# mohammadasim98/mv-ldm

Hardware: AMD Instinct MI355X
Metric: denoised views/sec @ 256x256, 4 views, 50 DDIM steps (higher is better)
Workload: dtype bf16

## Files before the change

### include/mvldm.h

```cpp
#ifndef MVLDM_H
#define MVLDM_H

#include <stddef.h>
#include <stdint.h>

#ifdef __cplusplus
extern "C" {
#endif

#define MVLDM_ABI_VERSION 7

typedef void* mvldm_stream_t;

enum { MVLDM_F32 = 0, MVLDM_BF16 = 1, MVLDM_F16 = 2 };
enum { MVLDM_OK = 0, MVLDM_ERR_ARG = -1, MVLDM_ERR_HIP = -2, MVLDM_ERR_UNSUPPORTED = -3 };

enum { MVLDM_EPI_NONE = 0, MVLDM_EPI_SILU = 1, MVLDM_EPI_GEGLU = 2, MVLDM_EPI_GELU = 3  };
enum { MVLDM_ELT_COPY = 0, MVLDM_ELT_SILU = 1, MVLDM_ELT_GELU = 2 };

int mvldm_abi_version(void);
int mvldm_build_flags(void);
const char* mvldm_last_error(void);
int mvldm_device_info(int* cu_count, size_t* hbm_bytes, char* arch, int arch_len);

typedef struct mvldm_igemm_desc {
    const void* src0;
    const void* src1;
    const void* weight;
    const float* bias;
    const float* row_bias;
    const void* residual;
    void* dst;
    float* workspace;
    int32_t c0, c1;
    int32_t n_img, h_in, w_in, h_out, w_out;
    int32_t ksize, stride, pad, upsample;
    int32_t n_out, n_pad, k_pad;
    int32_t row_bias_ld;
    int32_t epilogue;
    int32_t act_dtype;
    int32_t dst_dtype;
    int32_t splitk;
    int32_t tile;
    int32_t k_order;
    int32_t dst_ld;
    float out_scale;
    size_t workspace_bytes;
} mvldm_igemm_desc;
int mvldm_igemm_fwd(const mvldm_igemm_desc* d, mvldm_stream_t stream);
size_t mvldm_igemm_workspace_bytes(const mvldm_igemm_desc* d);

int mvldm_pack_weight(const float* src, void* dst, int n_out, int c_in, int ksize, int c_pad, int n_pad,
                      int k_pad, int geglu, int k_order, int dst_dtype, int transpose, int c_off, int n_rows,
                      mvldm_stream_t stream);

int mvldm_pack_skinny(const void* packed, void* dst, int n_pad, int k_pad, int geglu, int dtype, mvldm_stream_t stream);
int mvldm_igemm_skinny_config(const mvldm_igemm_desc* d);

typedef struct mvldm_pack_job {
    const float* src; void* dst;
    int n_out, c_in, ksize, c_pad, n_pad, k_pad, geglu, k_order, transpose, c_off, n_rows;
    int kind;
    int blocks;
    int block0;
} mvldm_pack_job;
int mvldm_pack_job_prepare(mvldm_pack_job* job , int dst_dtype);
int mvldm_pack_weight_batch(const mvldm_pack_job* jobs , int n_jobs, const int32_t* block_job, int total_blocks,
                            int dst_dtype, mvldm_stream_t stream);

#define MVLDM_GN_MAX_CHUNKS 32
int mvldm_groupnorm_fwd(const void* x0, const void* x1, void* y, const float* gamma, const float* beta, int n_img,
                        int hw, int c0, int c1, int groups, float eps, int silu, int dtype, void* stats_ws,
                        float* stats_out, mvldm_stream_t stream);
int mvldm_groupnorm_passes(int n_img, int hw, int c, int groups, int dtype);

int mvldm_layernorm_fwd(const void* x, void* y, const float* gamma, const float* beta, int rows, int c, float eps,
                        int dtype, mvldm_stream_t stream);

int mvldm_attention_fwd(const void* q, const void* k, const void* v, void* out, int ld_q, int ld_k, int ld_v,
                        int ld_o, int heads, int head_dim, const int32_t* seg, int n_seg, int max_q_len,
                        float scale, int dtype, float* lse, int lse_ld, mvldm_stream_t stream);

int mvldm_timestep_embed_fwd(const int64_t* timesteps, const float* freqs, void* out, int n, int dim,
                             int flip_sin_to_cos, int dst_dtype, mvldm_stream_t stream);

int mvldm_eltwise_fwd(const void* x, void* y, size_t n, int op, int src_dtype, int dst_dtype, mvldm_stream_t stream);

int mvldm_ddim_cfg_step(const float* eps, const float* x_t, float* x_next, const int32_t* cond_img,
                        const int32_t* uncond_img, int n_tgt, int hw, int c, float cfg_scale, const float* coef,
                        const int32_t* step_ptr, void* unet_in, int unet_in_c, int unet_in_dtype, int n_steps,
                        float clip_range, mvldm_stream_t stream);
int mvldm_ddpm_cfg_step(const float* eps_c, const float* eps_u, const float* x_t, const float* noise, float* x_next, size_t n,
                        float cfg_scale, const float* coef, float clip_range, mvldm_stream_t stream);
int mvldm_ddim_advance(int32_t* step_ptr, const int64_t* t_table, int n_steps, int64_t* timesteps,
                       const int32_t* tgt_rows, int n_rows, mvldm_stream_t stream);

int mvldm_nchw_to_nhwc(const float* src, void* dst, int n_img, int c, int hw, int dst_c, int dst_c_off,
                       int dst_dtype, float scale, float shift, const int32_t* img_map, mvldm_stream_t stream);
int mvldm_nhwc_to_nchw(const void* src, float* dst, int n_img, int c, int hw, int src_c, int src_c_off,
                       int src_dtype, float scale, float shift, int clamp01, mvldm_stream_t stream);

enum { MVLDM_RAYS_RAW = 0, MVLDM_RAYS_POSITIONAL = 1, MVLDM_RAYS_SRT = 2 };
int mvldm_ray_channels(int mode, int n_origin_octaves, int n_dir_octaves);
int mvldm_ray_encode(const float* extrinsics, const float* intrinsics, int n_cam, int h, int w, float* out_nchw,
                     void* out_nhwc, int nhwc_c, int nhwc_c_off, int nhwc_dtype, const int32_t* img_map, int mode,
                     int n_origin_octaves, int n_dir_octaves, int plucker, mvldm_stream_t stream);

int mvldm_posterior_sample(const float* moments, const float* noise, float* out, int n, int c, int hw, float scale,
                           mvldm_stream_t stream);


typedef struct mvldm_wgrad_desc {
    const void* src0; const void* src1; const void* dy;
    float* grad;
    float* workspace; size_t workspace_bytes;
    int32_t c0, c1, c_in;
    int32_t n_img, h_in, w_in, h_out, w_out;
    int32_t ksize, stride, pad, upsample;
    int32_t n_out, dy_ld;
    int32_t act_dtype;
    int32_t accumulate;
} mvldm_wgrad_desc;
int mvldm_igemm_wgrad(const mvldm_wgrad_desc* d, mvldm_stream_t stream);

int mvldm_colsum(const void* x, float* dst, float* workspace, size_t workspace_bytes, int n_seg, int rows_per_seg, int n,
                 int ld, int ld_dst, int per_seg, int accumulate, int dtype, mvldm_stream_t stream);

#define MVLDM_NORM_BWD_STORE 0x100
int mvldm_groupnorm_bwd(const void* x0, const void* x1, const void* dy, void* dx0, void* dx1, const float* gamma,
                        const float* beta, const float* stats, float* dgamma, float* dbeta, int n_img, int hw, int c0,
                        int c1, int groups, int silu, int dtype, float* workspace, size_t workspace_bytes,
                        mvldm_stream_t stream);
int mvldm_layernorm_bwd(const void* x, const void* dy, void* dx, const float* gamma, float* dgamma, float* dbeta,
// ... 233 lines not shown
```

### mv_ldm_amd/_lib.py

```python
from __future__ import annotations

import ctypes as C
from pathlib import Path

LIB_PATH = Path(__file__).resolve().parent / "csrc" / "libmvldm_hip.so"

ABI_VERSION = 7
F32, BF16, F16 = 0, 1, 2
EPI_NONE, EPI_SILU, EPI_GEGLU, EPI_GELU = 0, 1, 2, 3
RAYS_RAW, RAYS_POSITIONAL, RAYS_SRT = 0, 1, 2
ELT_COPY, ELT_SILU, ELT_GELU = 0, 1, 2
NORM_BWD_STORE = 0x100
GN_MAX_CHUNKS = 32
JPEG_GRAY, JPEG_444, JPEG_422, JPEG_420 = 0, 1, 2, 3
JPEG_REASONS = ("ok", "not a JPEG", "truncated", "corrupt", "progressive", "frame type", "precision", "components", "sampling", "colour space",
                "scans", "size", "range guard", "restart intervals")
JPEG_RANGE = 12
JPEG_RESTART = 13
JPEG_HUFF_TABLE_BYTES, JPEG_TABLE_BYTES = 1424, 8928

(OP_IGEMM, OP_GROUPNORM, OP_LAYERNORM, OP_ATTENTION, OP_TIMESTEP_EMBED, OP_ELTWISE, OP_DDIM_STEP, OP_DDIM_ADVANCE,
 OP_NCHW_TO_NHWC, OP_NHWC_TO_NCHW, OP_MEMCPY, OP_RAY_ENCODE, OP_POSTERIOR_SAMPLE,
 OP_WGRAD, OP_ATTENTION_BWD, OP_GROUPNORM_BWD, OP_LAYERNORM_BWD, OP_COLSUM, OP_TRAIN_ELTWISE, OP_POOL2X2, OP_ZERO_INSERT,
 OP_ADD_NOISE, OP_MSE_LOSS, OP_FILL_ZERO, OP_PAR_BEGIN, OP_PAR_NEXT, OP_PAR_END, OP_GATHER_ROWS, OP_ATTN_MERGE) = range(1, 30)
TE_SILU_BWD, TE_ADD, TE_GEGLU_FWD, TE_GEGLU_BWD, TE_GELU_BWD = 0, 1, 2, 3, 4

vp, i32, f32, sz = C.c_void_p, C.c_int32, C.c_float, C.c_size_t


class IgemmDesc(C.Structure):
    _fields_ = [("src0", vp), ("src1", vp), ("weight", vp), ("bias", vp), ("row_bias", vp), ("residual", vp),
                ("dst", vp), ("workspace", vp),
                ("c0", i32), ("c1", i32),
                ("n_img", i32), ("h_in", i32), ("w_in", i32), ("h_out", i32), ("w_out", i32),
                ("ksize", i32), ("stride", i32), ("pad", i32), ("upsample", i32),
                ("n_out", i32), ("n_pad", i32), ("k_pad", i32),
                ("row_bias_ld", i32), ("epilogue", i32), ("act_dtype", i32), ("dst_dtype", i32),
                ("splitk", i32), ("tile", i32), ("k_order", i32), ("dst_ld", i32), ("out_scale", f32), ("workspace_bytes", sz)]


class _GroupNorm(C.Structure):
    _fields_ = [("x", vp), ("x1", vp), ("y", vp), ("gamma", vp), ("beta", vp), ("stats_ws", vp),
                ("n_img", i32), ("hw", i32), ("c0", i32), ("c1", i32), ("groups", i32), ("silu", i32), ("dtype", i32),
                ("eps", f32), ("stats_out", vp)]


class _LayerNorm(C.Structure):
    _fields_ = [("x", vp), ("y", vp), ("gamma", vp), ("beta", vp), ("rows", i32), ("c", i32), ("dtype", i32), ("eps", f32)]


class _Attention(C.Structure):
    _fields_ = [("q", vp), ("k", vp), ("v", vp), ("out", vp), ("seg", vp),
                ("ld_q", i32), ("ld_k", i32), ("ld_v", i32), ("ld_o", i32), ("heads", i32), ("head_dim", i32),
                ("n_seg", i32), ("max_q_len", i32), ("dtype", i32), ("scale", f32), ("lse", vp), ("lse_ld", i32)]


class _Temb(C.Structure):
    _fields_ = [("timesteps", vp), ("freqs", vp), ("out", vp), ("n", i32), ("dim", i32), ("flip", i32), ("dst_dtype", i32)]


class _Eltwise(C.Structure):
    _fields_ = [("x", vp), ("y", vp), ("n", sz), ("op", i32), ("src_dtype", i32), ("dst_dtype", i32)]


class _Ddim(C.Structure):
    _fields_ = [("eps", vp), ("x_t", vp), ("x_next", vp), ("cond_img", vp), ("uncond_img", vp), ("coef", vp),
                ("step_ptr", vp), ("unet_in", vp),
                ("n_tgt", i32), ("hw", i32), ("c", i32), ("unet_in_c", i32), ("unet_in_dtype", i32), ("cfg_scale", f32),
                ("n_steps", i32), ("clip_range", f32)]


class _Advance(C.Structure):
    _fields_ = [("step_ptr", vp), ("t_table", vp), ("timesteps", vp), ("tgt_rows", vp), ("n_steps", i32), ("n_rows", i32)]


class _Layout(C.Structure):
    _fields_ = [("src", vp), ("dst", vp), ("n_img", i32), ("c", i32), ("hw", i32), ("other_c", i32),
                ("other_c_off", i32), ("dtype", i32), ("clamp01", i32), ("scale", f32), ("shift", f32), ("img_map", vp)]


class _Rays(C.Structure):
    _fields_ = [("extrinsics", vp), ("intrinsics", vp), ("out_nchw", vp), ("out_nhwc", vp), ("img_map", vp),
                ("n_cam", i32), ("h", i32), ("w", i32), ("nhwc_c", i32), ("nhwc_c_off", i32), ("nhwc_dtype", i32),
                ("mode", i32), ("n_origin_octaves", i32), ("n_dir_octaves", i32), ("plucker", i32)]


class _Posterior(C.Structure):
    _fields_ = [("moments", vp), ("noise", vp), ("out", vp), ("n", i32), ("c", i32), ("hw", i32), ("scale", f32)]


class _Memcpy(C.Structure):
    _fields_ = [("src", vp), ("dst", vp), ("bytes", sz)]


class _AttnMerge(C.Structure):
    _fields_ = [("oa", vp), ("ob", vp), ("out", vp), ("lse_a", vp), ("lse_b", vp), ("a_img", vp), ("b_img", vp), ("out_img", vp),
                ("n_img", i32), ("tokens", i32), ("heads", i32), ("head_dim", i32), ("ld_a", i32), ("ld_b", i32), ("ld_o", i32),
                ("lse_ld_a", i32), ("lse_ld_b", i32), ("dtype", i32)]


class _Gather(C.Structure):
    _fields_ = [("src", vp), ("dst", vp), ("src_index", vp), ("dst_index", vp), ("row_bytes", sz), ("n_rows", i32)]


class PackJob(C.Structure):
    _fields_ = [("src", vp), ("dst", vp), ("n_out", i32), ("c_in", i32), ("ksize", i32), ("c_pad", i32), ("n_pad", i32), ("k_pad", i32),
                ("geglu", i32), ("k_order", i32), ("transpose", i32), ("c_off", i32), ("n_rows", i32), ("kind", i32), ("blocks", i32),
                ("block0", i32)]


class WgradDesc(C.Structure):
    _fields_ = [("src0", vp), ("src1", vp), ("dy", vp), ("grad", vp), ("workspace", vp), ("workspace_bytes", sz),
                ("c0", i32), ("c1", i32), ("c_in", i32),
                ("n_img", i32), ("h_in", i32), ("w_in", i32), ("h_out", i32), ("w_out", i32),
                ("ksize", i32), ("stride", i32), ("pad", i32), ("upsample", i32),
                ("n_out", i32), ("dy_ld", i32), ("act_dtype", i32), ("accumulate", i32)]


class AttnBwdDesc(C.Structure):
    _fields_ = [("q", vp), ("k", vp), ("v", vp), ("out", vp), ("dout", vp), ("dq", vp), ("dk", vp), ("dv", vp),
                ("lse", vp), ("delta", vp), ("seg", vp),
                ("ld_q", i32), ("ld_k", i32), ("ld_v", i32), ("ld_o", i32), ("ld_do", i32), ("ld_dq", i32), ("ld_dk", i32), ("ld_dv", i32),
                ("heads", i32), ("head_dim", i32), ("n_seg", i32), ("max_q_len", i32), ("max_kv_len", i32), ("total_q_rows", i32),
                ("stat_ld", i32), ("dtype", i32), ("scale", f32)]


class _GroupNormBwd(C.Structure):
    _fields_ = [("x0", vp), ("x1", vp), ("dy", vp), ("dx0", vp), ("dx1", vp), ("gamma", vp), ("beta", vp), ("stats", vp),
                ("dgamma", vp), ("dbeta", vp), ("workspace", vp), ("workspace_bytes", sz),
                ("n_img", i32), ("hw", i32), ("c0", i32), ("c1", i32), ("groups", i32), ("silu", i32), ("dtype", i32)]


class _LayerNormBwd(C.Structure):
    _fields_ = [("x", vp), ("dy", vp), ("dx", vp), ("gamma", vp), ("dgamma", vp), ("dbeta", vp), ("workspace", vp),
                ("workspace_bytes", sz), ("rows", i32), ("c", i32), ("dtype", i32), ("eps", f32)]


class _Colsum(C.Structure):
    _fields_ = [("x", vp), ("dst", vp), ("workspace", vp), ("workspace_bytes", sz),
                ("n_seg", i32), ("rows_per_seg", i32), ("n", i32), ("ld", i32), ("ld_dst", i32), ("per_seg", i32),
                ("accumulate", i32), ("dtype", i32)]


class _TrainEltwise(C.Structure):
    _fields_ = [("a", vp), ("b", vp), ("out", vp), ("rows", sz), ("op", i32), ("d", i32), ("a_dtype", i32), ("dtype", i32)]


class _Resample(C.Structure):
    _fields_ = [("src", vp), ("dst", vp), ("n_img", i32), ("h", i32), ("w", i32), ("c", i32), ("dtype", i32)]


class _AddNoise(C.Structure):
    _fields_ = [("x0", vp), ("noise", vp), ("coef", vp), ("dst", vp), ("img_map", vp),
                ("n", i32), ("c", i32), ("hw", i32), ("dst_c", i32), ("dst_c_off", i32), ("dst_dtype", i32)]


class _Mse(C.Structure):
    _fields_ = [("pred", vp), ("noise", vp), ("tgt_img", vp), ("loss", vp), ("dpred", vp), ("workspace", vp),
                ("n_tgt", i32), ("hw", i32), ("c", i32), ("accumulate", i32), ("dpred_c", i32), ("dpred_dtype", i32),
                ("loss_scale", f32), ("grad_scale", f32), ("amp_scale", vp)]


class AmpState(C.Structure):
    _fields_ = [("scale", f32), ("growth_tracker", i32), ("adam_step", i32), ("found_inf", i32), ("skipped", i32), ("reserved", i32 * 3)]


class _Fill(C.Structure):
    _fields_ = [("dst", vp), ("bytes", sz)]


class _OpUnion(C.Union):
    _fields_ = [("igemm", IgemmDesc), ("groupnorm", _GroupNorm), ("layernorm", _LayerNorm), ("attention", _Attention),
                ("temb", _Temb), ("eltwise", _Eltwise), ("ddim", _Ddim), ("advance", _Advance), ("layout", _Layout),
                ("memcpy_", _Memcpy), ("gather", _Gather), ("attn_merge", _AttnMerge), ("rays", _Rays), ("posterior", _Posterior),
                ("wgrad", WgradDesc), ("attention_bwd", AttnBwdDesc), ("groupnorm_bwd", _GroupNormBwd),
                ("layernorm_bwd", _LayerNormBwd), ("colsum", _Colsum), ("train_eltwise", _TrainEltwise), ("resample", _Resample),
                ("add_noise", _AddNoise), ("mse", _Mse), ("fill", _Fill)]


class Op(C.Structure):
    _fields_ = [("kind", i32), ("tag", i32), ("u", _OpUnion)]


SIGNATURES = {
    "mvldm_abi_version": (C.c_int, []),
    "mvldm_build_flags": (C.c_int, []),
    "mvldm_last_error": (C.c_char_p, []),
    "mvldm_device_info": (C.c_int, [C.POINTER(C.c_int), C.POINTER(sz), C.c_char_p, C.c_int]),
    "mvldm_igemm_fwd": (C.c_int, [C.POINTER(IgemmDesc), vp]),
    "mvldm_igemm_workspace_bytes": (sz, [C.POINTER(IgemmDesc)]),
    "mvldm_pack_weight": (C.c_int, [vp, vp] + [C.c_int] * 12 + [vp]),
    "mvldm_pack_skinny": (C.c_int, [vp, vp, C.c_int, C.c_int, C.c_int, C.c_int, vp]),
    "mvldm_igemm_skinny_config": (C.c_int, [C.POINTER(IgemmDesc)]),
    "mvldm_pack_job_prepare": (C.c_int, [C.POINTER(PackJob), C.c_int]),
    "mvldm_pack_weight_batch": (C.c_int, [vp, C.c_int, vp, C.c_int, C.c_int, vp]),
    "mvldm_groupnorm_fwd": (C.c_int, [vp, vp, vp, vp, vp, C.c_int, C.c_int, C.c_int, C.c_int, C.c_int, f32, C.c_int, C.c_int, vp, vp, vp]),
    "mvldm_groupnorm_passes": (C.c_int, [C.c_int] * 5),
    "mvldm_layernorm_fwd": (C.c_int, [vp, vp, vp, vp, C.c_int, C.c_int, f32, C.c_int, vp]),
    "mvldm_attention_fwd": (C.c_int, [vp, vp, vp, vp] + [C.c_int] * 6 + [vp, C.c_int, C.c_int, f32, C.c_int, vp, C.c_int, vp]),
    "mvldm_igemm_wgrad": (C.c_int, [C.POINTER(WgradDesc), vp]),
    "mvldm_colsum": (C.c_int, [vp, vp, vp, sz] + [C.c_int] * 8 + [vp]),
    "mvldm_groupnorm_bwd": (C.c_int, [vp] * 10 + [C.c_int] * 7 + [vp, sz, vp]),
    "mvldm_layernorm_bwd": (C.c_int, [vp] * 6 + [C.c_int, C.c_int, f32, C.c_int, vp, sz, vp]),
    "mvldm_attention_bwd": (C.c_int, [C.POINTER(AttnBwdDesc), vp]),
    "mvldm_train_eltwise": (C.c_int, [C.c_int, vp, vp, vp, sz, C.c_int, C.c_int, C.c_int, vp]),
    "mvldm_pool2x2_sum": (C.c_int, [vp, vp] + [C.c_int] * 5 + [vp]),
    "mvldm_zero_insert2x": (C.c_int, [vp, vp] + [C.c_int] * 5 + [vp]),
    "mvldm_add_noise": (C.c_int, [vp, vp, vp, vp] + [C.c_int] * 6 + [vp, vp]),
    "mvldm_mse_loss": (C.c_int, [vp, vp, vp, C.c_int, C.c_int, C.c_int, vp, C.c_int, f32, vp, C.c_int, C.c_int, f32, vp, vp]),
    "mvldm_grad_norm": (C.c_int, [vp, sz, vp, f32, vp, vp, vp]),
    "mvldm_adamw_step": (C.c_int, [vp, vp, vp, vp, sz, f32, f32, f32, f32, f32, C.c_int, f32, vp, vp]),
    "mvldm_mse_loss_amp": (C.c_int, [vp, vp, vp, C.c_int, C.c_int, C.c_int, vp, C.c_int, f32, vp, C.c_int, C.c_int, f32, vp, vp, vp]),
    "mvldm_grad_norm_amp": (C.c_int, [vp, sz, vp, f32, vp, vp, vp, vp]),
    "mvldm_adamw_step_amp": (C.c_int, [vp, vp, vp, vp, sz, f32, f32, f32, f32, f32, f32, vp, vp, vp]),
    "mvldm_amp_update": (C.c_int, [vp, f32, f32, C.c_int, vp]),
    "mvldm_timestep_embed_fwd": (C.c_int, [vp, vp, vp, C.c_int, C.c_int, C.c_int, C.c_int, vp]),
    "mvldm_eltwise_fwd": (C.c_int, [vp, vp, sz, C.c_int, C.c_int, C.c_int, vp]),
    "mvldm_ddim_cfg_step": (C.c_int, [vp, vp, vp, vp, vp, C.c_int, C.c_int, C.c_int, f32, vp, vp, vp, C.c_int, C.c_int, C.c_int, f32, vp]),
    "mvldm_ddim_advance": (C.c_int, [vp, vp, C.c_int, vp, vp, C.c_int, vp]),
    "mvldm_gather_rows": (C.c_int, [vp, vp, vp, vp, C.c_int, sz, vp]),
    "mvldm_attention_merge": (C.c_int, [vp] * 8 + [C.c_int] * 10 + [vp]),
    "mvldm_ddpm_cfg_step": (C.c_int, [vp, vp, vp, vp, vp, sz, f32, vp, f32, vp]),
    "mvldm_ema_update": (C.c_int, [vp, vp, sz, f32, vp]),
    "mvldm_image_metrics_workspace_bytes": (sz, [C.c_int] * 4),
    "mvldm_image_metrics": (C.c_int, [vp, vp] + [C.c_int] * 5 + [vp, vp, vp, sz, vp]),
    "mvldm_lpips_workspace_bytes": (sz, [C.c_int] * 3),
    "mvldm_lpips_tap_slots": (C.c_int, [C.c_int] * 3),
    "mvldm_lpips_prep": (C.c_int, [vp, vp, vp] + [C.c_int] * 6 + [vp]),
    "mvldm_lpips_relu": (C.c_int, [vp, sz, C.c_int, vp]),
    "mvldm_lpips_tap": (C.c_int, [vp, vp, vp] + [C.c_int] * 5 + [vp, sz, C.c_int, C.c_int, vp]),
    "mvldm_lpips_fold": (C.c_int, [vp, sz, C.c_int, C.c_int, C.c_int, vp, vp]),
    "mvldm_dists_workspace_bytes": (sz, [C.c_int] * 3),
    "mvldm_dists_stat_slots": (C.c_int, [C.c_int] * 3),
    "mvldm_dists_prep": (C.c_int, [vp, vp, vp] + [C.c_int] * 5 + [vp]),
    "mvldm_dists_stats": (C.c_int, [vp, vp] + [C.c_int] * 5 + [vp, sz, C.c_int, C.c_int, vp]),
    "mvldm_dists_l2pool": (C.c_int, [vp, vp] + [C.c_int] * 5 + [vp]),
    "mvldm_dists_fold": (C.c_int, [vp, sz, C.c_int, C.c_int, C.c_int, vp, vp, vp, vp]),
    "mvldm_fid_workspace_bytes": (sz, [C.c_int] * 4),
    "mvldm_fid_pool_slots": (C.c_int, [C.c_int] * 3),
    "mvldm_fid_prep": (C.c_int, [vp, C.c_int, vp] + [C.c_int] * 7 + [vp]),
    "mvldm_fid_pool": (C.c_int, [vp] + [C.c_int] * 5 + [vp, sz, vp]),
    "mvldm_fid_accumulate": (C.c_int, [vp, sz] + [C.c_int] * 4 + [vp, vp, vp]),
    "mvldm_fid_compute": (C.c_int, [vp, vp, C.c_int, vp, vp, vp]),
    "mvldm_inception_workspace_bytes": (sz, [C.c_int] * 3),
    "mvldm_inception_prep": (C.c_int, [vp, C.c_int, vp] + [C.c_int] * 7 + [vp, sz, vp]),
    "mvldm_inception_unfold": (C.c_int, [vp, vp] + [C.c_int] * 9 + [vp]),
    "mvldm_inception_maxpool": (C.c_int, [vp, vp] + [C.c_int] * 9 + [vp]),
    "mvldm_inception_avgpool": (C.c_int, [vp, vp] + [C.c_int] * 7 + [vp]),
    "mvldm_inception_concat": (C.c_int, [vp, vp, sz] + [C.c_int] * 5 + [vp]),
    "mvldm_inception_features": (C.c_int, [vp] + [C.c_int] * 5 + [vp, vp]),
    "mvldm_frechet_accumulate": (C.c_int, [vp, C.c_int, C.c_int, vp, vp]),
    "mvldm_frechet_workspace_bytes": (sz, [C.c_int]),
    "mvldm_frechet_compute": (C.c_int, [vp, vp, C.c_int, vp, sz, vp, vp, vp]),
    "mvldm_kid_workspace_bytes": (sz, [C.c_int, C.c_int]),
    "mvldm_kid_compute": (C.c_int, [vp, C.c_int, vp, C.c_int, C.c_int, vp, vp, C.c_int, C.c_int, vp, sz, vp, vp, vp, vp]),
    "mvldm_crop_shim_workspace_bytes": (sz, [C.c_int] * 5),
    "mvldm_crop_shim": (C.c_int, [vp, C.c_int, vp] + [C.c_int] * 5 + [vp, sz, C.POINTER(C.c_int), vp]),
    "mvldm_crop_shim_flip": (C.c_int, [vp, C.c_int, vp] + [C.c_int] * 5 + [vp, vp, sz, C.POINTER(C.c_int), vp]),
    "mvldm_crop_shim_axis": (C.c_int, [C.c_int] * 4 + [C.POINTER(i32), C.POINTER(i32), C.c_int]),
    "mvldm_jpeg_probe": (C.c_int, [vp, sz, C.POINTER(i32)]),
    "mvldm_jpeg_coef_count": (sz, [C.c_int] * 3),
    "mvldm_jpeg_entropy": (C.c_int, [vp, sz, vp, sz, vp, C.POINTER(i32)]),
    "mvldm_jpeg_workspace_bytes": (sz, [C.c_int] * 4),
    "mvldm_jpeg_decode": (C.c_int, [vp, vp, vp] + [C.c_int] * 4 + [vp, sz, vp]),
    "mvldm_jpeg_idct_host": (C.c_int, [vp, vp, vp, C.c_int, C.c_int, C.c_int]),
    "mvldm_jpeg_scan_room": (sz, [sz]),
    "mvldm_jpeg_scan_prepare": (C.c_int, [vp, sz, vp, sz, sz, vp, vp, vp]),
    "mvldm_jpeg_entropy_chunk_subseqs": (C.c_int, []),
    "mvldm_jpeg_entropy_device": (C.c_int, [vp, sz, vp, vp] + [C.c_int] * 4 + [vp, vp, vp, C.c_int, vp]),
    "mvldm_jpeg_entropy_emul_host": (C.c_int, [vp, sz, vp, vp] + [C.c_int] * 4 + [vp, vp, vp, C.c_int, C.c_int]),
    "mvldm_nchw_to_nhwc": (C.c_int, [vp, vp] + [C.c_int] * 6 + [f32, f32, vp, vp]),
    "mvldm_ray_channels": (C.c_int, [C.c_int, C.c_int, C.c_int]),
    "mvldm_ray_encode": (C.c_int, [vp, vp, C.c_int, C.c_int, C.c_int, vp, vp, C.c_int, C.c_int, C.c_int, vp] + [C.c_int] * 4 + [vp]),
# ... 56 lines not shown
```

### mv_ldm_amd/csrc/igemm.hip

```cpp
#include <algorithm>
#include <cstdio>
#include <cstdlib>

#include "igemm_common.h"

namespace mvldm {

template <typename T> __global__ __launch_bounds__(256) void igemm_splitk_reduce(const IgemmParams p) {
    const bool geglu = p.epilogue == MVLDM_EPI_GEGLU;
    const size_t total = (size_t)p.M * p.n_dst;
    const size_t slab = (size_t)p.M * p.n_pad;
    for (size_t idx = (size_t)blockIdx.x * 256 + threadIdx.x; idx < total; idx += (size_t)gridDim.x * 256) {
        const int m = (int)(idx / p.n_dst), col = (int)(idx - (size_t)m * p.n_dst);
        float v;
        if (geglu) {
            const int nv = (col >> 5) * 64 + (col & 31), ng = nv + 32;
            float a = 0.f, g = 0.f;
            for (int s = 0; s < p.splitk; ++s) {
                a += p.ws[s * slab + (size_t)m * p.n_pad + nv];
                g += p.ws[s * slab + (size_t)m * p.n_pad + ng];
            }
            if (p.bias) { a += p.bias[col]; g += p.bias[p.n_dst + col]; }
            v = a * gelu_erf_fast(g);
        } else {
// ... 65 lines not shown
                const float* rb = p.row_bias + (size_t)(m / p.hw_out) * p.row_bias_ld + col;
#pragma unroll
                for (int e = 0; e < 8; ++e) a[e] += rb[e];
            }
            if (p.epilogue == MVLDM_EPI_SILU) {
#pragma unroll
                for (int e = 0; e < 8; ++e) a[e] = silu_f(a[e]);
            } else if (p.epilogue == MVLDM_EPI_GELU) {
#pragma unroll
                for (int e = 0; e < 8; ++e) a[e] = gelu_erf_fast(a[e]);
            }
        }
#pragma unroll
        for (int e = 0; e < 8; ++e) a[e] *= p.out_scale;
        if (p.residual) {
            const Chunk<T> rc = load_chunk<T>(reinterpret_cast<const T*>(p.residual) + (size_t)m * p.n_dst + col);
#pragma unroll
            for (int e = 0; e < 8; ++e) a[e] += rc.get(e);
        }
        size_t drow = (size_t)m;
        if (p.scatter) {
            const int img = m / p.hw_out, rem = m - img * p.hw_out;
            const int i = rem / p.w_out, j = rem - i * p.w_out;
            drow = ((size_t)img * (2 * p.h_out) + 2 * i + p.ph_y) * (size_t)(2 * p.w_out) + 2 * j + p.ph_x;
        }
        Chunk<T> oc;
#pragma unroll
        for (int e = 0; e < 8; ++e) oc.set(e, a[e]);
        store_chunk<T>(reinterpret_cast<T*>(p.dst) + drow * p.dst_ld + col, oc);
    }
}

static int env_int(const char* name, int dflt) { return knob_int(name, dflt); }
static const int kEnvTarget = env_int("MVLDM_IGEMM_TARGET", 0);
static const int kEnvSync = env_int("MVLDM_IGEMM_SYNC", 0);
static const int kEnvPx = env_int("MVLDM_IGEMM_PX", 0);
static const int kEnvNoStage = env_int("MVLDM_IGEMM_NOSTAGE", 0);
#ifdef MVLDM_EXPERIMENTS
static const int kEnvFake = env_int("MVLDM_IGEMM_FAKE", 0);
#else
static constexpr int kEnvFake = 0;
#endif

static thread_local int t_force_sync = 0;

static int launch_igemm(const IgemmParams& p, int tile, int act_dtype, hipStream_t s) {
    if (tile >= 1 && tile <= 5) return igemm_launch_small(p, tile, act_dtype, s);
    if (tile >= 6 && tile <= 8) return igemm_launch_large(p, tile, act_dtype, s);
    if (tile == 9 || tile == 10 || tile == 18) return igemm_launch_xl(p, tile, act_dtype, s);
    if (tile == 11 || tile == 17) return igemm_launch_halo(p, tile, act_dtype, s);
    return set_error(MVLDM_ERR_ARG, "igemm: bad tile %d", tile);
}


static void choose_config(const mvldm_igemm_desc& d, int M, int k_tiles, int& tile, int& splitk, size_t ws_bytes) {
    const int target = kEnvTarget ? kEnvTarget : 512;
    if (tile == 0) {
        const bool can10 = d.act_dtype != MVLDM_F32 && d.k_order == 1 && d.dst_dtype != MVLDM_F32 && d.n_pad % 320 == 0 &&
                           d.epilogue != MVLDM_EPI_GEGLU && d.upsample != 1 && d.n_out % 8 == 0 && (d.dst_ld <= 0 || d.dst_ld % 8 == 0) &&
                           !(d.ksize == 3 && d.src1);
        const int wgs10 = cdiv(M, 256) * (d.n_pad / 320);
        const double eff10 = (double)wgs10 / (256.0 * cdiv(wgs10, 256));
        if (can10 && (wgs10 >= 1024 || (wgs10 >= 512 && (eff10 >= 0.9 || d.ksize == 1)))) tile = 10;
        else if (M <= 32) tile = 5;
        else if (M <= 64) tile = 4;
        else if (d.ksize >= 2) tile = cdiv(M, 256) * cdiv(d.n_pad, 128) >= 300 ? 7 : 2;
        else if (d.n_pad >= 768 && d.act_dtype != MVLDM_F32 && d.k_order == 1 && d.dst_dtype != MVLDM_F32 &&
                 cdiv(M, 256) * cdiv(d.n_pad, 256) >= 1024)
            tile = 9;
        else if (d.k_pad >= 1024 && d.n_pad >= 1024 && cdiv(M, 128) * cdiv(d.n_pad, 256) >= 300) tile = 8;
        else tile = d.n_pad < 640 ? 2 : 3;
    }
    const int tm = cdiv(M, kTiles[tile].bm), tn = cdiv(d.n_pad, kTiles[tile].bn);
    if (splitk == 0) {
        splitk = 1;
        const int wgs = tm * tn;
        if (wgs < target) splitk = std::min(std::max(k_tiles / 4, 1), cdiv(target, wgs));
        if (d.workspace == nullptr) splitk = 1;
        while (splitk > 1 && (size_t)splitk * M * d.n_pad * sizeof(float) > ws_bytes) --splitk;
    }
    splitk = std::max(1, std::min(splitk, k_tiles));
}

static int fill_params(const mvldm_igemm_desc& d, IgemmParams& p, int& tile) {
    const int epc = d.act_dtype == MVLDM_F32 ? 4 : 8;
    const int bk = d.act_dtype == MVLDM_F32 ? 32 : 64;
    MVLDM_REQUIRE(d.src0 && d.weight && d.dst, "igemm: null pointer");
    const bool phase = d.upsample >= 2;
    MVLDM_REQUIRE(d.upsample >= 0 && d.upsample <= 5, "igemm: upsample %d", d.upsample);
    MVLDM_REQUIRE(phase ? (d.ksize == 2 && d.stride == 1 && d.h_out == d.h_in && d.w_out == d.w_in && !d.src1 && !d.residual &&
                           !d.row_bias && d.act_dtype != MVLDM_F32 && d.dst_dtype == d.act_dtype && d.k_order == 1)
                        : (d.ksize == 1 || d.ksize == 3),
                  "igemm: ksize %d / upsample %d", d.ksize, d.upsample);
    MVLDM_REQUIRE(d.stride == 1 || d.stride == 2, "igemm: stride %d", d.stride);
    MVLDM_REQUIRE(d.c0 % epc == 0 && d.c1 % epc == 0 && d.c0 > 0, "igemm: channels (%d,%d) must be multiples of %d", d.c0, d.c1, epc);
    MVLDM_REQUIRE((d.c1 == 0) == (d.src1 == nullptr), "igemm: src1/c1 mismatch");
    MVLDM_REQUIRE(d.k_pad % bk == 0 && d.k_pad >= d.ksize * d.ksize * (d.c0 + d.c1), "igemm: k_pad %d", d.k_pad);
    MVLDM_REQUIRE(d.n_pad % 64 == 0 && d.n_pad >= d.n_out, "igemm: n_pad %d (n_out %d)", d.n_pad, d.n_out);
    MVLDM_REQUIRE(d.dst_dtype == d.act_dtype || d.dst_dtype == MVLDM_F32, "igemm: dst dtype");
    if (d.epilogue == MVLDM_EPI_GEGLU)
        MVLDM_REQUIRE(d.n_out % 64 == 0 && !d.row_bias, "igemm: GEGLU needs n_out %% 64 == 0");
    p.src0 = d.src0; p.src1 = d.src1; p.weight = d.weight; p.bias = d.bias; p.row_bias = d.row_bias;
    p.residual = d.residual; p.dst = d.dst; p.ws = d.workspace;
    p.c0 = d.c0; p.c1 = d.c1; p.ctot = d.c0 + d.c1;
    p.n_img = d.n_img; p.h_in = d.h_in; p.w_in = d.w_in; p.h_out = d.h_out; p.w_out = d.w_out;
    p.hw_out = d.h_out * d.w_out;
    p.ksize = d.ksize; p.stride = d.stride; p.pad = d.pad; p.upsample = phase ? 0 : d.upsample; p.taps = d.ksize * d.ksize;
    p.scatter = phase; p.ph_y = phase ? (d.upsample - 2) >> 1 : 0; p.ph_x = phase ? (d.upsample - 2) & 1 : 0;
    p.ty0 = phase ? p.ph_y - 1 : -d.pad; p.tx0 = phase ? p.ph_x - 1 : -d.pad;
    p.cy = phase ? 1 - p.ph_y : d.ksize / 2; p.cx = phase ? 1 - p.ph_x : d.ksize / 2;
    p.M = d.n_img * p.hw_out; p.n_out = d.n_out; p.n_pad = d.n_pad; p.k_pad = d.k_pad;
    p.n_dst = d.epilogue == MVLDM_EPI_GEGLU ? d.n_out / 2 : d.n_out;
    p.rb_vec = d.row_bias && ((uintptr_t)d.row_bias % 16 == 0) && d.row_bias_ld % 4 == 0;
    p.bias_vec = d.bias && ((uintptr_t)d.bias % 16 == 0);
    p.row_bias_ld = d.row_bias_ld; p.epilogue = d.epilogue; p.dst_f32 = d.dst_dtype == MVLDM_F32;
    p.out_scale = d.out_scale;
    p.dst_ld = d.dst_ld > 0 ? d.dst_ld : p.n_dst;
    MVLDM_REQUIRE(p.dst_ld >= p.n_dst, "igemm: dst_ld %d < n_dst %d", p.dst_ld, p.n_dst);
    p.k_tiles = d.k_pad / bk;
    tile = d.tile & 63;
    t_force_sync = (d.tile >> 12) & 1;
    const int force_px = (d.tile >> 8) & 15;
    int splitk = d.splitk;
    MVLDM_REQUIRE(((tile >= 0 && tile <= kNumTiles) || tile == 17 || deep_tile(tile)) && splitk >= 0, "igemm: tile/splitk");
    choose_config(d, p.M, p.k_tiles, tile, splitk, d.workspace_bytes);
    if (splitk > 1)
        MVLDM_REQUIRE(d.workspace && (size_t)splitk * p.M * d.n_pad * sizeof(float) <= d.workspace_bytes,
                      "igemm: split-K workspace too small");
    const double es = 2.0;
    const double b0 = (double)d.n_img * d.h_in * d.w_in * d.c0 * es, b1 = (double)d.n_img * d.h_in * d.w_in * d.c1 * es;
    const double bw = (double)d.n_pad * d.k_pad * es;
    p.use_bl = d.act_dtype != MVLDM_F32 && d.k_order == 1 && !t_force_sync && !kEnvSync &&
               b0 < 4.0e9 && b1 < 4.0e9 && bw < 4.0e9;
    if (d.act_dtype != MVLDM_F32 && d.k_order == 1 && !t_force_sync && !kEnvSync && !p.use_bl) {
        static bool warned = false;
        if (!warned) {
            warned = true;
            fprintf(stderr, "[mvldm] igemm: operand of %.2f GB exceeds the 4 GB range of the fast 16-bit loop; using the slower "
                            "64-bit-address loop (split the batch to avoid this)\n", std::max(std::max(b0, b1), bw) / 1e9);
        }
    }
    p.src0_bytes = (unsigned)b0; p.src1_bytes = (unsigned)b1; p.w_bytes = (unsigned)bw;
    p.fake = kEnvFake;
    p.nt_store = stream_stores((size_t)p.M * (size_t)p.n_dst * (p.dst_f32 || d.act_dtype == MVLDM_F32 ? 4 : 2));
    if (kEnvFake & 1) p.src0_bytes = p.src1_bytes = 0;
    if (kEnvFake & 2) p.w_bytes = 0;
    if (tile >= 6 && !p.use_bl) tile = 2;
    if (deep_tile(tile) && d.upsample) tile = 2;
    p.splitk = splitk;
    if (p.use_bl) {
        const int cbs = p.k_tiles / p.taps;
        const int per = cdiv(cbs, std::min(splitk, cbs));
        p.k_tiles_per_split = per * p.taps;
        p.splitk = cdiv(cbs, per);
    } else {
        p.k_tiles_per_split = cdiv(p.k_tiles, splitk);
        p.splitk = cdiv(p.k_tiles, p.k_tiles_per_split);
    }
    p.stage_epi = d.act_dtype != MVLDM_F32 && !kEnvNoStage && (p.splitk > 1 || (!p.dst_f32 && p.n_dst % 8 == 0 && p.dst_ld % 8 == 0));
    if (tile >= 9 && tile <= 10 && (!p.stage_epi || (tile == 10 && d.epilogue == MVLDM_EPI_GEGLU))) tile = 7;
    if (tile == 11 && !(p.use_bl && p.stage_epi && p.splitk == 1 && d.ksize == 3 && d.stride == 1 && d.pad == 1 && !d.upsample &&
                        d.h_out == d.h_in && d.w_out == d.w_in && halo_rows_for(d.w_in) <= 384 && halo_smem(d.w_in) <= 160 * 1024))
        tile = 7;
    if (tile == 17 && !(p.use_bl && p.stage_epi && p.splitk == 1 && d.ksize == 3 && d.stride == 1 && d.pad == 1 && !d.upsample && d.c1 == 0 &&
                        d.h_out == d.h_in && d.w_out == d.w_in && d.epilogue != MVLDM_EPI_GEGLU && halow_smem(d.w_in) <= 160 * 1024))
        tile = 7;
    if (phase) {
        MVLDM_REQUIRE(p.use_bl && p.stage_epi, "igemm: 2x2 phase conv needs the lean 16-bit loop and an 8-aligned 16-bit output");
        if (tile != 7 && tile != 10) tile = 2;
    }
    if (p.use_bl && d.upsample == 1 && tile != 7) tile = 2;
    if (p.use_bl && d.upsample != 1) {
        const int hc = (d.h_out - 1) * d.stride + p.ty0 + p.cy, wc = (d.w_out - 1) * d.stride + p.tx0 + p.cx;
        MVLDM_REQUIRE(p.ty0 + p.cy >= 0 && p.tx0 + p.cx >= 0 && hc < d.h_in && wc < d.w_in,
                      "igemm: conv geometry (pad %d, stride %d) not supported", d.pad, d.stride);
    }
    p.tiles_m = cdiv(p.M, kTiles[tile].bm);
    p.tiles_n = cdiv(d.n_pad, kTiles[tile].bn);
    p.korder = d.k_order;
    if (d.k_order)
        MVLDM_REQUIRE(d.k_order == 1 && p.ctot % bk == 0 && d.c0 % bk == 0 && d.k_pad == p.taps * p.ctot,
                      "igemm: k_order 1 needs channel counts (%d,%d) multiples of %d", d.c0, d.c1, bk);
    {
        const double a_bytes = (double)d.n_img * d.h_in * d.w_in * p.ctot, w_bytes = (double)d.n_pad * d.k_pad;
        double best = 1e300;
        for (int px = 1; px <= 8; px *= 2) {
            const int py = 8 / px;
            const int sm = cdiv(p.tiles_m, px), sn = cdiv(p.tiles_n, py);
            const double waste = (double)(8 * sm * sn) / ((double)p.tiles_m * p.tiles_n);
            const double cost = (py * a_bytes + px * w_bytes) * waste * waste;
            if (cost < best) { best = cost; p.px = px; p.sub_m = sm; p.sub_n = sn; }
        }
        p.m_fast = w_bytes >= a_bytes;
        const int fpx = force_px ? force_px : kEnvPx;
        if (fpx > 0 && fpx <= 8 && (8 % fpx) == 0) {
            p.px = fpx; p.sub_m = cdiv(p.tiles_m, p.px); p.sub_n = cdiv(p.tiles_n, 8 / p.px);
        }
        p.grp_m = p.grp_n = 1;
        static const int kGroup = knob_int("MVLDM_IGEMM_GROUP", -1);
        if (kGroup != 0 && ((tile >= 7 && tile <= 10) || tile == 17) && p.sub_m * p.sub_n > 32) {
            const double ax = a_bytes / p.px, wx = w_bytes / (8 / p.px);
            double bestc = 1e300;
            for (int gm = 1; gm <= 32; gm *= 2) {
                if (kGroup > 0 && gm != kGroup) continue;
                const int gme = std::min(gm, p.sub_m), gne = std::min(32 / gm, p.sub_n);
                const double c = ax * cdiv(p.sub_n, gne) + wx * cdiv(p.sub_m, gme);
                if (c < bestc) { bestc = c; p.grp_m = gme; p.grp_n = gne; }
            }
        }
    }
    return MVLDM_OK;
}

int linear_pp_run(const mvldm_igemm_desc& d, hipStream_t s);
int linear_pw_run(const mvldm_igemm_desc& d, hipStream_t s);
int linear_ws_run(const mvldm_igemm_desc& d, hipStream_t s);
int skinny_run(const mvldm_igemm_desc& d, hipStream_t s);
int linear_rs_run(const mvldm_igemm_desc& d, hipStream_t s);

int igemm_run(const mvldm_igemm_desc& d, hipStream_t s) {
    IgemmParams p;
    int tile = 0;
    if (d.n_img == 0 || d.h_out == 0 || d.w_out == 0) return MVLDM_OK;
    const int req = d.tile & 63;
    if (req == 15) return skinny_run(d, s);
    if (req == 12 || req == 13 || req == 14 || req == 19) {
        MVLDM_REQUIRE(d.src0 && d.weight && d.dst, "igemm: null pointer");
        return req == 12 ? linear_pp_run(d, s) : req == 13 ? linear_pw_run(d, s) : req == 14 ? linear_ws_run(d, s) : linear_rs_run(d, s);
    }
    MVLDM_REQUIRE(d.k_order != 2, "igemm: the fragment-order pack (k_order 2) is read by tile 15 only");
    int rc = fill_params(d, p, tile);
    if (rc) return rc;
    if (p.M == 0) return MVLDM_OK;
    rc = dispatch_dtype(d.act_dtype, [&](auto t) {
        using T = decltype(t);
        int r = launch_igemm(p, tile, Elt<T>::DT, s);
        if (r) return r;
        if (p.splitk > 1) {
            if constexpr (sizeof(T) == 2) {
                if (!p.dst_f32 && p.n_dst % 8 == 0 && p.dst_ld % 8 == 0 && ((uintptr_t)p.ws % 16) == 0 &&
                    (!p.residual || ((uintptr_t)p.residual % 16) == 0) && ((uintptr_t)p.dst % 16) == 0) {
                    const size_t chunks = (size_t)p.M * (p.n_dst / 8);
                    hipLaunchKernelGGL(igemm_splitk_reduce_vec<T>, dim3((unsigned)std::min<size_t>((chunks + 255) / 256, 4096)), dim3(256), 0, s, p);
                    return check_launch();
                }
            }
            const size_t total = (size_t)p.M * p.n_dst;
            const int blocks = (int)std::min<size_t>((total + 255) / 256, 4096);
            hipLaunchKernelGGL(igemm_splitk_reduce<T>, dim3(blocks), dim3(256), 0, s, p);
            return check_launch();
        }
        return (int)MVLDM_OK;
    });
    return rc;
}

}

using namespace mvldm;

extern "C" int mvldm_igemm_fwd(const mvldm_igemm_desc* d, mvldm_stream_t stream) {
    MVLDM_REQUIRE(d != nullptr, "igemm: null desc");
    return igemm_run(*d, (hipStream_t)stream);
}

extern "C" size_t mvldm_igemm_workspace_bytes(const mvldm_igemm_desc* d) {
    if (!d) return 0;
    const size_t M = (size_t)d->n_img * d->h_out * d->w_out;
    return (size_t)16 * M * d->n_pad * sizeof(float);
}
```

### mv_ldm_amd/csrc/igemm_bl.h

```cpp
#pragma once
#include "igemm_common.h"

namespace mvldm {

template <typename T, int BM, int BN, int WM, int WN>
__global__ __launch_bounds__(WM* WN * 64) void igemm_kernel(const IgemmParams p) {
    using M_ = Mma<T>;
    constexpr int NT = WM * WN * 64;
    constexpr int EPC = Elt<T>::EPC;
    constexpr int BK = M_::BK;
    constexpr int TM = BM / WM / 32, TN = BN / WN / 32;
    constexpr int A_BYTES = BM * M_::PITCH, B_BYTES = BN * M_::PITCH;
    constexpr int A_IT = BM * 8 / NT, B_IT = BN * 8 / NT;
    static_assert(A_IT >= 1 && B_IT >= 1 && TM >= 1 && TN >= 1, "bad tile");
    extern __shared__ __attribute__((aligned(16))) char smem[];

    const int tid = threadIdx.x, lane = tid & 63, wave = tid >> 6;
    const int wm = wave / WN, wn = wave % WN;
    const int hi = lane >> 5, l31 = lane & 31;

    int split, tm, tn;
    if (!map_block(p, split, tm, tn)) return;
    const int kt0 = split * p.k_tiles_per_split;
    const int kt1 = min(kt0 + p.k_tiles_per_split, p.k_tiles);
// ... 36 lines not shown
        const int cs = from0 ? p.c0 : p.c1;
#pragma unroll
        for (int it = 0; it < A_IT; ++it) {
            int iy = a_y[it] + ky, ix = a_x[it] + kx;
            const bool ok = tap_ok && a_img[it] >= 0 && iy >= 0 && iy < hs && ix >= 0 && ix < wsz;
            if (p.upsample) { iy >>= 1; ix >>= 1; }
            if (ok) {
                const size_t off = ((size_t)(a_img[it] * p.h_in + iy) * p.w_in + ix) * cs;
                areg[it] = *reinterpret_cast<const u32x4*>(sbase + off);
            } else {
                areg[it] = u32x4{0u, 0u, 0u, 0u};
            }
        }
#pragma unroll
        for (int it = 0; it < B_IT; ++it) {
            const int n = tn * BN + r0 + it * (NT / 8);
            if (n < p.n_pad)
                breg[it] = *reinterpret_cast<const u32x4*>(wbase + (size_t)it * (NT / 8) * p.k_pad + (size_t)kt * BK);
            else
                breg[it] = u32x4{0u, 0u, 0u, 0u};
        }
    };
    auto store_tile = [&](int stage) {
        char* at = smem + stage * (A_BYTES + B_BYTES);
        char* bt = at + A_BYTES;
#pragma unroll
        for (int it = 0; it < A_IT; ++it) M_::store(at, r0 + it * (NT / 8), kc, areg[it]);
#pragma unroll
        for (int it = 0; it < B_IT; ++it) M_::store(bt, r0 + it * (NT / 8), kc, breg[it]);
    };

    f32x16 acc[TM][TN];
#pragma unroll
    for (int i = 0; i < TM; ++i)
#pragma unroll
        for (int j = 0; j < TN; ++j)
#pragma unroll
            for (int r = 0; r < 16; ++r) acc[i][j][r] = 0.f;

    if (kt0 < kt1) {
        load_tile(kt0);
        store_tile(0);
    }
    __syncthreads();
    int cur = 0;
    for (int kt = kt0; kt < kt1; ++kt) {
        const bool more = kt + 1 < kt1;
        if (more) load_tile(kt + 1);
        const char* at = smem + cur * (A_BYTES + B_BYTES);
        const char* bt = at + A_BYTES;
#pragma unroll
        for (int kk = 0; kk < BK / M_::KI; ++kk) {
            typename M_::Frag a[TM], b[TN];
#pragma unroll
            for (int i = 0; i < TM; ++i) a[i] = M_::load(at, wm * (BM / WM) + i * 32 + l31, kk, hi);
#pragma unroll
            for (int j = 0; j < TN; ++j) b[j] = M_::load(bt, wn * (BN / WN) + j * 32 + l31, kk, hi);
#pragma unroll
            for (int i = 0; i < TM; ++i)
#pragma unroll
                for (int j = 0; j < TN; ++j) acc[i][j] = M_::mma(a[i], b[j], acc[i][j]);
        }
        if (more) store_tile(cur ^ 1);
        __syncthreads();
        cur ^= 1;
    }

    if constexpr (sizeof(T) == 2) {
        if (p.stage_epi) {
            igemm_epilogue_staged<T, BM, BN, WM, WN>(p, acc, tm, tn, split, wm, wn, wave, lane, smem);
            return;
        }
    }
    igemm_epilogue<T, BM, BN, WM, WN>(p, acc, tm, tn, split, wm, wn, hi, l31);
}


template <int TAPS, int A_IT, bool DUAL, bool UPS> struct BlAddr {
    unsigned a0[UPS ? TAPS : 1][A_IT];
    unsigned a1[DUAL ? (UPS ? TAPS : 1) : 1][DUAL ? A_IT : 1];
    unsigned mask[UPS ? 1 : A_IT];
};

template <typename T, int BM, int BN, int NW, int KS, bool DUAL, int A_IT, int B_IT, int STAGES, bool UPS, int t, int LO = 0, int HI = 1 << 20>
__device__ __forceinline__ void bl_issue(const IgemmParams& p, char* stage_base, int wave, int cb,
                                         const BlAddr<KS * KS, A_IT, DUAL, UPS>& ad, const unsigned (&vb)[B_IT]) {
    constexpr int BK = 64, TAPS = KS * KS;
    const int lead = (!UPS && KS > 1) ? p.w_in + 1 : 0;
    const int disp = UPS ? 0 : (t / KS - p.cy) * p.w_in + (t % KS - p.cx) + lead;
    const unsigned lead0 = (unsigned)lead * (unsigned)p.c0 * 2u, lead1 = (unsigned)lead * (unsigned)p.c1 * 2u;
    const __amdgpu_buffer_rsrc_t r0 = __builtin_amdgcn_make_buffer_rsrc(
        const_cast<char*>(reinterpret_cast<const char*>(p.src0)) - lead0, 0, p.src0_bytes + lead0, 0x00020000);
    const __amdgpu_buffer_rsrc_t r1 = __builtin_amdgcn_make_buffer_rsrc(
        const_cast<char*>(reinterpret_cast<const char*>(DUAL ? p.src1 : p.src0)) - (DUAL ? lead1 : lead0), 0,
        DUAL ? p.src1_bytes + lead1 : p.src0_bytes + lead0, 0x00020000);
    const __amdgpu_buffer_rsrc_t rw = __builtin_amdgcn_make_buffer_rsrc(const_cast<void*>(p.weight), 0, p.w_bytes, 0x00020000);
    char* at = stage_base;
    char* bt = at + BM * 128;
    const int c = cb * BK;
    const bool from0 = !DUAL || c < p.c0;
    const int soff = ((from0 ? c : c - p.c0) + disp * (from0 ? p.c0 : p.c1)) * 2;
#pragma unroll
    for (int it = (LO > 0 ? LO : 0); it < (HI < A_IT ? HI : A_IT); ++it) {
        __attribute__((address_space(3))) void* dst = (__attribute__((address_space(3))) void*)(at + (wave + NW * it) * 1024);
        unsigned v0, v1;
        if constexpr (UPS) {
            v0 = ad.a0[t][it];
            v1 = ad.a1[DUAL ? t : 0][DUAL ? it : 0];
        } else {
            const bool ok = (ad.mask[it] >> t) & 1u;
            v0 = ok ? ad.a0[0][it] : kBufOob;
            v1 = ok ? ad.a1[0][DUAL ? it : 0] : kBufOob;
        }
        if (from0) __builtin_amdgcn_raw_ptr_buffer_load_lds(r0, dst, 16, v0, soff, 0, 0);
        else __builtin_amdgcn_raw_ptr_buffer_load_lds(r1, dst, 16, v1, soff, 0, 0);
    }
    const int koff = (cb * TAPS + t) * (BK * 2);
#pragma unroll
    for (int it = (LO > A_IT ? LO - A_IT : 0); it < (HI - A_IT < B_IT ? HI - A_IT : B_IT); ++it)
        __builtin_amdgcn_raw_ptr_buffer_load_lds(rw, (__attribute__((address_space(3))) void*)(bt + (wave + NW * it) * 1024), 16,
                                                 vb[it], koff, 0, 0);
}

template <typename T, int BM, int BN, int WM, int WN>
__device__ __forceinline__ void bl_compute(const char* stage_base, f32x16 (&acc)[BM / WM / 32][BN / WN / 32], int wm, int wn,
                                           int hi, int l31) {
    constexpr int TM = BM / WM / 32, TN = BN / WN / 32;
#pragma unroll
    for (int kk = 0; kk < 64 / Mma<T>::KI; ++kk) {
        BlFrags<T, TM, TN> f;
        bl_load<T, BM, BN, WM, WN>(stage_base, f, kk, wm, wn, hi, l31);
        bl_mma<T, TM, TN>(f, acc);
    }
}

template <int LPT, int MAXY>
__device__ __forceinline__ void bl_wait_young(int young) {
    if constexpr (MAXY >= 1) {
        if (young >= MAXY) {
            asm volatile("s_waitcnt vmcnt(%0) lgkmcnt(0)" ::"n"(MAXY * LPT) : "memory");
            return;
        }
        bl_wait_young<LPT, MAXY - 1>(young);
    } else {
        asm volatile("s_waitcnt vmcnt(0) lgkmcnt(0)" ::: "memory");
    }
}

template <typename T, int BM, int BN, int WM, int WN, int KS, bool DUAL, int STAGES, bool UPS>
__global__ __launch_bounds__(WM* WN * 64) void igemm_bl_kernel(const IgemmParams p) {
    using M_ = Mma<T>;
    static_assert(sizeof(T) == 2, "16-bit activation types only");
    constexpr int NW = WM * WN, TAPS = KS * KS;
    constexpr int BK = 64, EPC = 8;
    constexpr int TM = BM / WM / 32, TN = BN / WN / 32;
    constexpr int A_BYTES = BM * 128, B_BYTES = BN * 128, STAGE_BYTES = A_BYTES + B_BYTES;
    constexpr int A_IT = BM / 8 / NW, B_IT = BN / 8 / NW, LPT = A_IT + B_IT;
    static_assert(A_IT >= 1 && B_IT >= 1 && (BM / 8) % NW == 0 && (BN / 8) % NW == 0, "bad tile");
    static_assert(STAGES >= 2 && STAGES <= 8, "ring depth");
    extern __shared__ __attribute__((aligned(16))) char smem[];

    const auto [lane, wave, wm, wn, hi, l31] = wave_lane<WN>();
    int split, tm, tn;
    if (!map_block(p, split, tm, tn)) return;
    const int cb0 = split * (p.k_tiles_per_split / TAPS);
    const int cb1 = min(cb0 + p.k_tiles_per_split / TAPS, p.k_tiles / TAPS);

    const int slot = lane & 7, rsub = lane >> 3;
    BlAddr<TAPS, A_IT, DUAL, UPS> ad;
#pragma unroll
    for (int it = 0; it < A_IT; ++it) {
        const int row = (wave + NW * it) * 8 + rsub;
        const int m = tm * BM + row;
        const unsigned chunk = (unsigned)((slot ^ ((row >> 1) & 7)) * EPC);
        const bool live = m < p.M;
        const int img = live ? m / p.hw_out : 0, rem = live ? m - img * p.hw_out : 0;
        const int oy = rem / p.w_out, ox = rem - oy * p.w_out;
        if constexpr (UPS) {
            const unsigned hs = 2 * p.h_in, wsz = 2 * p.w_in;
            const int y0 = live ? oy * p.stride - p.pad : -(1 << 20), x0 = ox * p.stride - p.pad;
#pragma unroll
            for (int t = 0; t < TAPS; ++t) {
                const int iy = y0 + t / KS, ix = x0 + t % KS;
                const bool ok = (unsigned)iy < hs && (unsigned)ix < wsz;
                const unsigned pix = (unsigned)(img * p.h_in + (iy >> 1)) * (unsigned)p.w_in + (unsigned)(ix >> 1);
                ad.a0[t][it] = ok ? (pix * (unsigned)p.c0 + chunk) * 2u : kBufOob;
                if constexpr (DUAL) ad.a1[t][it] = ok ? (pix * (unsigned)p.c1 + chunk) * 2u : kBufOob;
            }
        } else {
            const int yc = oy * p.stride + p.ty0 + p.cy, xc = ox * p.stride + p.tx0 + p.cx;
            const unsigned pix = (unsigned)(img * p.h_in + yc) * (unsigned)p.w_in + (unsigned)xc;
            unsigned msk = 0;
#pragma unroll
            for (int t = 0; t < TAPS; ++t) {
                const int iy = yc + t / KS - p.cy, ix = xc + t % KS - p.cx;
                msk |= (live && (unsigned)iy < (unsigned)p.h_in && (unsigned)ix < (unsigned)p.w_in) ? (1u << t) : 0u;
            }
            ad.a0[0][it] = (pix * (unsigned)p.c0 + chunk) * 2u;
            if constexpr (DUAL) ad.a1[0][it] = (pix * (unsigned)p.c1 + chunk) * 2u;
            ad.mask[it] = msk;
        }
    }
    unsigned vb[B_IT];
#pragma unroll
    for (int it = 0; it < B_IT; ++it) {
        const int row = (wave + NW * it) * 8 + rsub;
        const int n = tn * BN + row;
        const unsigned chunk = (unsigned)((slot ^ ((row >> 1) & 7)) * EPC);
        vb[it] = n < p.n_pad ? ((unsigned)n * (unsigned)p.k_pad + chunk) * 2u : kBufOob;
    }

    f32x16 acc[TM][TN];
#pragma unroll
    for (int i = 0; i < TM; ++i)
#pragma unroll
        for (int j = 0; j < TN; ++j)
#pragma unroll
            for (int r = 0; r < 16; ++r) acc[i][j][r] = 0.f;

#define MVLDM_BL_ISSUE(stage_, cb_, t_) \
    bl_issue<T, BM, BN, NW, KS, DUAL, A_IT, B_IT, STAGES, UPS, t_>(p, smem + (stage_) * STAGE_BYTES, wave, cb_, ad, vb)
#define MVLDM_BL_ISSUE_R(stage_, cb_, t_, lo_, hi_) \
    bl_issue<T, BM, BN, NW, KS, DUAL, A_IT, B_IT, STAGES, UPS, t_, lo_, hi_>(p, smem + (stage_) * STAGE_BYTES, wave, cb_, ad, vb)
#define MVLDM_BL_NEXT(t_, d_) (((t_) + (d_)) % TAPS)
#define MVLDM_BL_LOAD(f_, slot_, kk_) bl_load<T, BM, BN, WM, WN>(smem + (slot_) * STAGE_BYTES, f_, kk_, wm, wn, hi, l31)
#define MVLDM_BL_MMA(f_)                  \
    __builtin_amdgcn_sched_barrier(0);    \
    bl_mma<T, TM, TN>(f_, acc);           \
    __builtin_amdgcn_sched_barrier(0);
#define MVLDM_BL_STEP(t_)                                                                                         \
    {                                                                                                             \
        static_assert(64 / M_::KI == 4, "four k-sub-steps per K-tile");                                          \
        MVLDM_BL_LOAD(f1, slot_c, 1);                                                                             \
        MVLDM_BL_MMA(f0)                                                                                          \
        MVLDM_BL_LOAD(f0, slot_c, 2);                                                                             \
        MVLDM_BL_MMA(f1)                                                                                          \
        MVLDM_BL_LOAD(f1, slot_c, 3);                                                                             \
        MVLDM_BL_MMA(f0)                                                                                          \
            \
                             \
        if (STAGES == 3 && cb + ((t_) + 2) / TAPS < cb1) asm volatile("s_waitcnt vmcnt(%0) lgkmcnt(0)" ::"n"(LPT) : "memory"); \
        else asm volatile("s_waitcnt vmcnt(0) lgkmcnt(0)" ::: "memory");                                          \
        __builtin_amdgcn_s_barrier();                                                                             \
        {                                                                                                         \
                   \
            const int cbn_ = cb + ((t_) + STAGES) / TAPS;                                                         \
            if (cbn_ < cb1) { MVLDM_BL_ISSUE(slot_c, cbn_, MVLDM_BL_NEXT(t_, STAGES)); }                          \
        }                                                                                                         \
        slot_c = slot_c + 1 == STAGES ? 0 : slot_c + 1;                                                           \
        MVLDM_BL_LOAD(f0, slot_c, 0);                                                                             \
        MVLDM_BL_MMA(f1)                                                                                          \
    }
#ifdef MVLDM_BL_BURST
    constexpr bool SPREAD_S = false;
#elif defined(MVLDM_BL_SPREAD_ALL)
    constexpr bool SPREAD_S = true;
#else
    constexpr bool SPREAD_S = NW == 8;
#endif
#define MVLDM_BL_STEP_SIMPLE(t_)                                                                                  \
    {                                                                                                             \
        asm volatile("s_waitcnt vmcnt(0) lgkmcnt(0)" ::: "memory");                                               \
        __builtin_amdgcn_s_barrier();                                                                             \
        if constexpr (!SPREAD_S) {                                                                                \
            const int cbn_ = cb + ((t_) + 1) / TAPS;                                                              \
            if (cbn_ < cb1) { MVLDM_BL_ISSUE(slot_c ^ 1, cbn_, MVLDM_BL_NEXT(t_, 1)); }                           \
            bl_compute<T, BM, BN, WM, WN>(smem + slot_c * STAGE_BYTES, acc, wm, wn, hi, l31);                     \
        } else {                                                                                                  \
            constexpr int Q0_ = (4 * LPT + 8) / 9, Q1_ = Q0_ + (LPT - Q0_ + 1) / 2;                              \
            const int cbn_ = cb + ((t_) + 1) / TAPS;                                                              \
            const bool more_ = cbn_ < cb1;                                                                        \
            if (more_) { MVLDM_BL_ISSUE_R(slot_c ^ 1, cbn_, MVLDM_BL_NEXT(t_, 1), 0, Q0_); }                      \
            {                                                                                                     \
                BlFrags<T, TM, TN> fs_;                                                                           \
                MVLDM_BL_LOAD(fs_, slot_c, 0);                                                                    \
                bl_mma<T, TM, TN>(fs_, acc);                                                                      \
            }                                                                                                     \
            if (more_) { MVLDM_BL_ISSUE_R(slot_c ^ 1, cbn_, MVLDM_BL_NEXT(t_, 1), Q0_, Q1_); }                    \
            {                                                                                                     \
                BlFrags<T, TM, TN> fs_;                                                                           \
                MVLDM_BL_LOAD(fs_, slot_c, 1);                                                                    \
                bl_mma<T, TM, TN>(fs_, acc);                                                                      \
            }                                                                                                     \
            if (more_) { MVLDM_BL_ISSUE_R(slot_c ^ 1, cbn_, MVLDM_BL_NEXT(t_, 1), Q1_, LPT); }                    \
            {                                                                                                     \
                BlFrags<T, TM, TN> fs_;                                                                           \
                MVLDM_BL_LOAD(fs_, slot_c, 2);                                                                    \
                bl_mma<T, TM, TN>(fs_, acc);                                                                      \
                MVLDM_BL_LOAD(fs_, slot_c, 3);                                                                    \
                bl_mma<T, TM, TN>(fs_, acc);                                                                      \
            }                                                                                                     \
        }                                                                                                         \
        slot_c ^= 1;                                                                                              \
    }
#define MVLDM_BL_STEP_DEEP(t_)                                                                                    \
    {                                                                                                             \
        bl_wait_young<LPT, STAGES - 2>((cb1 - cb) * TAPS - (t_) - 1);       \
        __builtin_amdgcn_s_barrier();                                       \
        {                                                                                                         \
            const int cbn_ = cb + ((t_) + STAGES - 1) / TAPS;                                                     \
            if (cbn_ < cb1) { MVLDM_BL_ISSUE(slot_c == 0 ? STAGES - 1 : slot_c - 1, cbn_, MVLDM_BL_NEXT(t_, STAGES - 1)); } \
        }                                                                                                         \
        bl_compute<T, BM, BN, WM, WN>(smem + slot_c * STAGE_BYTES, acc, wm, wn, hi, l31);                         \
        slot_c = slot_c + 1 == STAGES ? 0 : slot_c + 1;                                                           \
    }
#define MVLDM_BL_PRO(j_)                                                                                          \
    if constexpr (STAGES - 1 > (j_)) {                                                                            \
        if (cb0 + (j_) / TAPS < cb1) { MVLDM_BL_ISSUE((j_), cb0 + (j_) / TAPS, ((j_) % TAPS)); }                  \
    }
    constexpr bool PIPE = NW == 8 && TM * TN <= 8 && STAGES <= 3;
    if constexpr (STAGES > 3) {
        static_assert((STAGES - 2) * LPT <= 63, "vmcnt is a 6-bit counter");
        if (cb0 < cb1) {
            MVLDM_BL_ISSUE(0, cb0, 0);
            MVLDM_BL_PRO(1) MVLDM_BL_PRO(2) MVLDM_BL_PRO(3) MVLDM_BL_PRO(4) MVLDM_BL_PRO(5) MVLDM_BL_PRO(6)
            int slot_c = 0;
            for (int cb = cb0; cb < cb1; ++cb) {
                MVLDM_BL_STEP_DEEP(0)
                if constexpr (TAPS == 4) { MVLDM_BL_STEP_DEEP(1) MVLDM_BL_STEP_DEEP(2) MVLDM_BL_STEP_DEEP(3) }
                if constexpr (TAPS == 9) {
                    MVLDM_BL_STEP_DEEP(1) MVLDM_BL_STEP_DEEP(2) MVLDM_BL_STEP_DEEP(3) MVLDM_BL_STEP_DEEP(4)
                    MVLDM_BL_STEP_DEEP(5) MVLDM_BL_STEP_DEEP(6) MVLDM_BL_STEP_DEEP(7) MVLDM_BL_STEP_DEEP(8)
                }
            }
        }
    } else if constexpr (!PIPE) {
        static_assert(STAGES == 2, "the plain loop uses the 2-slot ring");
        if (cb0 < cb1) {
            MVLDM_BL_ISSUE(0, cb0, 0);
            int slot_c = 0;
            for (int cb = cb0; cb < cb1; ++cb) {
                MVLDM_BL_STEP_SIMPLE(0)
                if constexpr (TAPS == 4) { MVLDM_BL_STEP_SIMPLE(1) MVLDM_BL_STEP_SIMPLE(2) MVLDM_BL_STEP_SIMPLE(3) }
                if constexpr (TAPS == 9) {
                    MVLDM_BL_STEP_SIMPLE(1) MVLDM_BL_STEP_SIMPLE(2) MVLDM_BL_STEP_SIMPLE(3) MVLDM_BL_STEP_SIMPLE(4)
                    MVLDM_BL_STEP_SIMPLE(5) MVLDM_BL_STEP_SIMPLE(6) MVLDM_BL_STEP_SIMPLE(7) MVLDM_BL_STEP_SIMPLE(8)
                }
            }
        }
    } else if (cb0 < cb1) {
        MVLDM_BL_ISSUE(0, cb0, 0);
        const bool has1 = cb0 + 1 / TAPS < cb1, has2 = STAGES == 3 && cb0 + 2 / TAPS < cb1;
        if (has1) { MVLDM_BL_ISSUE(1, cb0 + 1 / TAPS, (1 % TAPS)); }
        if constexpr (STAGES == 3) {
            if (has2) { MVLDM_BL_ISSUE(2, cb0 + 2 / TAPS, (2 % TAPS)); }
        }
        if (has2) asm volatile("s_waitcnt vmcnt(%0)" ::"n"(2 * LPT) : "memory");
        else if (has1) asm volatile("s_waitcnt vmcnt(%0)" ::"n"(LPT) : "memory");
        else asm volatile("s_waitcnt vmcnt(0)" ::: "memory");
        __builtin_amdgcn_s_barrier();
        int slot_c = 0;
        BlFrags<T, TM, TN> f0, f1;
        MVLDM_BL_LOAD(f0, 0, 0);
        for (int cb = cb0; cb < cb1; ++cb) {
            MVLDM_BL_STEP(0)
            if constexpr (TAPS == 4) { MVLDM_BL_STEP(1) MVLDM_BL_STEP(2) MVLDM_BL_STEP(3) }
            if constexpr (TAPS == 9) {
                MVLDM_BL_STEP(1) MVLDM_BL_STEP(2) MVLDM_BL_STEP(3) MVLDM_BL_STEP(4)
                MVLDM_BL_STEP(5) MVLDM_BL_STEP(6) MVLDM_BL_STEP(7) MVLDM_BL_STEP(8)
            }
        }
    }
#undef MVLDM_BL_STEP_SIMPLE
#undef MVLDM_BL_STEP_DEEP
#undef MVLDM_BL_PRO
#undef MVLDM_BL_LOAD
#undef MVLDM_BL_MMA
#undef MVLDM_BL_NEXT
#undef MVLDM_BL_STEP
#undef MVLDM_BL_ISSUE
#undef MVLDM_BL_ISSUE_R
    asm volatile("s_waitcnt vmcnt(0)" ::: "memory");
    if constexpr (TM * TN > 4) {
        igemm_epilogue_staged<T, BM, BN, WM, WN>(p, acc, tm, tn, split, wm, wn, wave, lane, smem);
    } else {
        if (p.stage_epi) igemm_epilogue_staged<T, BM, BN, WM, WN>(p, acc, tm, tn, split, wm, wn, wave, lane, smem);
        else igemm_epilogue<T, BM, BN, WM, WN>(p, acc, tm, tn, split, wm, wn, hi, l31);
    }
}

template <typename T, int BM, int BN, int WM, int WN> static int launch_sync(const IgemmParams& p, hipStream_t s) {
    static std::atomic<uint64_t> done{0};
    constexpr int ring = 2 * (BM + BN) * Mma<T>::PITCH, park = WM * WN * 32 * (park_blocks(BN / WN / 32) * 32 + 4) * 4;
    return launch_kernel(igemm_kernel<T, BM, BN, WM, WN>, done, (sizeof(T) == 2 && park > ring) ? park : ring,
                         8 * p.sub_m * p.sub_n * p.splitk, WM * WN * 64, p, s);
}

template <typename T, int BM, int BN, int WM, int WN, int KS, bool DUAL, int STAGES, bool UPS>
static int launch_bl_s(const IgemmParams& p, hipStream_t s) {
    static std::atomic<uint64_t> done{0};
    constexpr int ring = STAGES * (BM + BN) * 128, park = WM * WN * 32 * (park_blocks(BN / WN / 32) * 32 + 4) * 4;
    return launch_kernel(igemm_bl_kernel<T, BM, BN, WM, WN, KS, DUAL, STAGES, UPS>, done, ring > park ? ring : park,
                         8 * p.sub_m * p.sub_n * p.splitk, WM * WN * 64, p, s);
}
template <typename T, int BM, int BN, int WM, int WN, int KS, bool DUAL, int DEPTH = 0>
static int launch_bl(const IgemmParams& p, hipStream_t s) {
    constexpr int STAGES = DEPTH ? DEPTH : ((WM * WN == 8 && 3 * (BM + BN) * 128 <= 160 * 1024) ? 3 : 2);
    if (p.upsample) {
        if constexpr (KS == 3 && !DUAL && ((BM == 128 && BN == 64) || (BM == 256 && BN == 128)))
            return launch_bl_s<T, BM, BN, WM, WN, KS, DUAL, STAGES, true>(p, s);
        else
            return set_error(MVLDM_ERR_ARG, "igemm: upsampling 3x3 conv needs tile 2 or 7 on the 16-bit path");
    }
    return launch_bl_s<T, BM, BN, WM, WN, KS, DUAL, STAGES, false>(p, s);
}
template <typename T, int BM, int BN, int WM, int WN, int DEPTH> static int launch_bl_deep(const IgemmParams& p, hipStream_t s) {
    const bool dual = p.c1 > 0;
    if (p.ksize == 3) return dual ? launch_bl<T, BM, BN, WM, WN, 3, true, DEPTH>(p, s) : launch_bl<T, BM, BN, WM, WN, 3, false, DEPTH>(p, s);
    if (p.ksize == 1) return dual ? launch_bl<T, BM, BN, WM, WN, 1, true, DEPTH>(p, s) : launch_bl<T, BM, BN, WM, WN, 1, false, DEPTH>(p, s);
    return set_error(MVLDM_ERR_ARG, "igemm: the deep-ring tiles take 1x1 and 3x3 convs");
}

template <typename T, int BM, int BN, int WM, int WN> static int launch_bl_any(const IgemmParams& p, hipStream_t s) {
    const bool dual = p.c1 > 0;
    if (p.ksize == 2) {
        if constexpr ((BM == 128 && BN == 64) || (BM == 256 && BN == 128) || (BM == 256 && BN == 320))
            return launch_bl<T, BM, BN, WM, WN, 2, false>(p, s);
        else
            return set_error(MVLDM_ERR_ARG, "igemm: 2x2 phase conv needs tile 2, 7 or 10");
    }
    if (p.ksize == 3) {
        if (!dual) return launch_bl<T, BM, BN, WM, WN, 3, false>(p, s);
        if constexpr (BM == 256 && BN >= 256)
            return set_error(MVLDM_ERR_UNSUPPORTED, "igemm: tiles 9 / 10 do not take a two-source 3x3 conv (use tile 7 or 11)");
        else
            return launch_bl<T, BM, BN, WM, WN, 3, true>(p, s);
    }
    return dual ? launch_bl<T, BM, BN, WM, WN, 1, true>(p, s) : launch_bl<T, BM, BN, WM, WN, 1, false>(p, s);
}

template <typename T, int BM, int BN, int WM, int WN> static int launch_tile(const IgemmParams& p, hipStream_t s) {
    if constexpr (sizeof(T) == 2) {
        if (p.use_bl) return launch_bl_any<T, BM, BN, WM, WN>(p, s);
    }
    return launch_sync<T, BM, BN, WM, WN>(p, s);
}

}
```

### mv_ldm_amd/csrc/igemm_common.h

```cpp
#pragma once
#include <algorithm>

#include "common.h"

namespace mvldm {

struct IgemmParams {
    const void* src0; const void* src1; const void* weight;
    const float* bias; const float* row_bias; const void* residual; void* dst; float* ws;
    int c0, c1, ctot;
    int n_img, h_in, w_in, h_out, w_out, hw_out;
    int ksize, stride, pad, upsample;
    int M, n_out, n_pad, n_dst, k_pad, taps;
    int row_bias_ld, epilogue, dst_f32, dst_ld;
    float out_scale;
    int splitk, k_tiles, k_tiles_per_split;
    int tiles_m, tiles_n;
    int korder;
    int px, sub_m, sub_n, m_fast;
    int grp_m, grp_n;
    int rb_vec;
    int bias_vec;
    int ty0, tx0, cy, cx;
    int scatter, ph_y, ph_x;
    int fake;
    unsigned src0_bytes, src1_bytes, w_bytes;
    int use_bl, stage_epi;
    int nt_store;
};

template <typename T> struct Mma;

template <typename T16> struct Mma16 : Mfma16<T16> {
    static constexpr int KI = 16;
    static constexpr int BK = 64;
    static constexpr int PITCH = 128;
    using Frag = typename Mfma16<T16>::Frag;
    static __device__ __forceinline__ void store(char* tile, int r, int kc, u32x4 v) {
        *reinterpret_cast<u32x4*>(tile + r * PITCH + ((kc ^ ((r >> 1) & 7)) << 4)) = v;
    }
    static __device__ __forceinline__ Frag load(const char* tile, int r, int kk, int hi) {
        const int kc = kk * 2 + hi;
        return *reinterpret_cast<const Frag*>(tile + r * PITCH + ((kc ^ ((r >> 1) & 7)) << 4));
    }
};
template <> struct Mma<bf16_t> : Mma16<bf16_t> {};
template <> struct Mma<f16_t> : Mma16<f16_t> {};
template <> struct Mma<float> {
    static constexpr int KI = 2;
    static constexpr int BK = 32;
    static constexpr int PITCH = 33 * 4;
    using Frag = float;
    static __device__ __forceinline__ void store(char* tile, int r, int kc, u32x4 v) {
        uint32_t* p = reinterpret_cast<uint32_t*>(tile + r * PITCH + kc * 16);
        p[0] = v[0]; p[1] = v[1]; p[2] = v[2]; p[3] = v[3];
    }
    static __device__ __forceinline__ Frag load(const char* tile, int r, int kk, int hi) {
        return *reinterpret_cast<const float*>(tile + r * PITCH + (kk * 2 + hi) * 4);
    }
    static __device__ __forceinline__ f32x16 mma(Frag a, Frag b, f32x16 c) {
        return __builtin_amdgcn_mfma_f32_32x32x2f32(a, b, c, 0, 0, 0);
    }
};

__device__ __forceinline__ int orig_col(int n_packed, int n_out, bool geglu) {
    if (!geglu) return n_packed;
    const int blk = n_packed >> 5, w = n_packed & 31;
    return (blk & 1) ? (n_out >> 1) + (blk >> 1) * 32 + w : (blk >> 1) * 32 + w;
}

template <typename T, bool SCATTER = false>
__device__ __forceinline__ void epilogue_store(const IgemmParams& p, int m, int n_dst_col, float v) {
    v *= p.out_scale;
    if (p.residual) v += to_f32<T>(reinterpret_cast<const T*>(p.residual)[(size_t)m * p.n_dst + n_dst_col]);
    size_t drow = (size_t)m;
    if (SCATTER && p.scatter) {
        const int img = m / p.hw_out, rem = m - img * p.hw_out;
        const int i = rem / p.w_out, j = rem - i * p.w_out;
        drow = ((size_t)img * (2 * p.h_out) + 2 * i + p.ph_y) * (size_t)(2 * p.w_out) + 2 * j + p.ph_x;
    }
    const size_t o = drow * p.dst_ld + n_dst_col;
    if (p.dst_f32) reinterpret_cast<float*>(p.dst)[o] = v;
    else reinterpret_cast<T*>(p.dst)[o] = from_f32<T>(v);
}

__device__ __forceinline__ bool map_block(const IgemmParams& p, int& split, int& tm, int& tn) {
    const int b = blockIdx.x, xcd = b & 7, idx = b >> 3;
    const int xm = xcd % p.px, xn = xcd / p.px;
    const int per = p.sub_m * p.sub_n;
    split = idx / per;
    const int r = idx - split * per;
    int tml, tnl;
    if (p.grp_m * p.grp_n > 1) {
        const int gm = p.grp_m, gn = p.grp_n;
        const int nfull = p.sub_m / gm, per_super = gm * p.sub_n;
        int mg, gm_eff, rr;
        if (r < nfull * per_super) { mg = r / per_super; rr = r - mg * per_super; gm_eff = gm; }
        else { mg = nfull; rr = r - nfull * per_super; gm_eff = p.sub_m - nfull * gm; }
        const int ng = rr / (gm_eff * gn), r2 = rr - ng * gm_eff * gn;
        tnl = ng * gn + r2 / gm_eff;
        tml = mg * gm + r2 % gm_eff;
    } else if (p.m_fast) { tnl = r / p.sub_m; tml = r - tnl * p.sub_m; }
    else { tml = r / p.sub_n; tnl = r - tml * p.sub_n; }
    tm = xm * p.sub_m + tml;
    tn = xn * p.sub_n + tnl;
    return tm < p.tiles_m && tn < p.tiles_n;
}

template <typename T, int BM, int BN, int WM, int WN>
__device__ __forceinline__ void igemm_epilogue(const IgemmParams& p, f32x16 (&acc)[BM / WM / 32][BN / WN / 32], int tm, int tn,
                                               int split, int wm, int wn, int hi, int l31) {
// ... 312 lines not shown
```

### mv_ldm_amd/csrc/skinny.hip

```cpp
#include <algorithm>
#include <cstdio>
#include <cstdlib>
#include <cstring>

#include "common.h"

namespace mvldm {

struct SkParams {
    const void* src0; const void* src1; const void* w;
    const float* bias; const float* row_bias; const void* residual; void* dst;
    int c0, c1;
    int n_img, h_in, w_in, hw_in, h_out, w_out, hw_out;
    int stride, ty0, tx0, ksize;
    int M, n_out, n_dst, dst_ld, row_bias_ld, rb_hw;
    int epilogue, dst_f32;
    float out_scale;
    int n_tiles;
    int n_groups, m_groups, G;
    int n_cbs, cb0;
    int n_stages;
    int ksteps;
    int scatter, ph_y, ph_x;
    int hw_sh, w_sh, rb_sh;
// ... 712 lines not shown
    for (int c : pref)
        if (c > 0 && c < kNumSkCfgs && sk_cfg_fits(kSkCfgs[c], d)) return c;
    for (int c = 1; c < kNumSkCfgs; ++c)
        if (sk_cfg_fits(kSkCfgs[c], d)) return c;
    return 0;
}

int skinny_run(const mvldm_igemm_desc& d, hipStream_t s) {
    MVLDM_REQUIRE(d.src0 && d.weight && d.dst, "igemm: null pointer");
    MVLDM_REQUIRE(skinny_applicable(d), "igemm: tile 15 (skinny weight-streaming GEMM) does not apply to this problem (needs the fragment-order "
                                        "pack, k_order 2, 16-bit activations, channels in multiples of 64, ksize 1 / 3 or a 2x2 phase conv)");
    int cfg = (d.tile >> 8) & 63;
    if (cfg == 0) cfg = sk_choose(d);
    MVLDM_REQUIRE(cfg > 0 && cfg < kNumSkCfgs && sk_cfg_fits(kSkCfgs[cfg], d), "igemm: tile 15: configuration %d does not compute this problem", cfg);
    const SkinnyCfgInfo& k = kSkCfgs[cfg];
    SkParams p;
    const bool phase = d.upsample >= 2;
    p.src0 = d.src0; p.src1 = d.src1; p.w = d.weight; p.bias = d.bias; p.row_bias = d.row_bias; p.residual = d.residual; p.dst = d.dst;
    p.c0 = d.c0; p.c1 = d.c1;
    const SkGeom g = sk_geom(d);
    p.n_img = g.n_img; p.h_in = g.h_in; p.w_in = g.w_in; p.hw_in = g.h_in * g.w_in; p.h_out = g.h_out; p.w_out = g.w_out; p.hw_out = g.h_out * g.w_out;
    p.rb_hw = d.h_out * d.w_out;
    auto lg2 = [](int v) { int sh = 0; while ((1 << sh) < v) ++sh; return (1 << sh) == v ? sh : -1; };
    p.hw_sh = lg2(p.hw_out); p.w_sh = lg2(p.w_out); p.rb_sh = lg2(p.rb_hw);
    p.stride = d.stride; p.ksize = d.ksize;
    p.scatter = phase; p.ph_y = phase ? (d.upsample - 2) >> 1 : 0; p.ph_x = phase ? (d.upsample - 2) & 1 : 0;
    p.ty0 = phase ? p.ph_y - 1 : -d.pad; p.tx0 = phase ? p.ph_x - 1 : -d.pad;
    p.M = p.n_img * p.hw_out; p.n_out = d.n_out;
    p.n_dst = d.epilogue == MVLDM_EPI_GEGLU ? d.n_out / 2 : d.n_out;
    p.dst_ld = d.dst_ld > 0 ? d.dst_ld : p.n_dst;
    p.row_bias_ld = d.row_bias_ld; p.epilogue = d.epilogue; p.dst_f32 = d.dst_dtype == MVLDM_F32; p.out_scale = d.out_scale;
    p.n_tiles = d.n_pad / 16;
    p.n_groups = (p.n_tiles + k.nt - 1) / k.nt;
    p.G = k.mt * 16 / p.hw_out;
    p.m_groups = (p.n_img + p.G - 1) / p.G;
    p.n_cbs = (d.c0 + d.c1) / 64; p.cb0 = d.c0 / 64;
    p.n_stages = k.sc ? (p.n_cbs + k.sc - 1) / k.sc : p.n_cbs;
    p.ksteps = p.n_cbs * k.taps * 2;
    const double px = (double)d.n_img * d.h_in * d.w_in;
    p.src0_bytes = (unsigned)(px * d.c0 * 2.0); p.src1_bytes = (unsigned)(px * d.c1 * 2.0);
    p.w_bytes = (unsigned)((double)d.n_pad * d.k_pad * 2.0);
    p.fake = kSkFake;
    p.trace = nullptr;
#ifdef MVLDM_SK_TRACE
    static unsigned long long* trace = nullptr;
    if (getenv("MVLDM_SK_TRACE")) {
        if (!trace) hipHostMalloc((void**)&trace, 16 * 40 * 8 * 8, hipHostMallocMapped);
        memset(trace, 0, 16 * 40 * 8 * 8);
        p.trace = trace;
    }
#endif
    if (kSkFake & 1) p.w_bytes = 0;
    if (kSkFake & 2) p.src0_bytes = p.src1_bytes = 0;
    if (kSkFake & 4) p.n_stages = 0;
    if (p.M == 0) return MVLDM_OK;
    const int grid = 8 * ((p.n_groups + 7) / 8) * p.m_groups;
    const int rc = dispatch_dtype(d.act_dtype, [&](auto t) -> int {
        using T = decltype(t);
        if constexpr (sizeof(T) == 2) return sk_dispatch<T>(cfg, p, grid, s);
        else return set_error(MVLDM_ERR_ARG, "igemm: tile 15 needs a 16-bit activation type");
    });
#ifdef MVLDM_SK_TRACE
    if (p.trace && getenv("MVLDM_SK_TRACE_DUMP")) {
        hipDeviceSynchronize();
        const unsigned long long t0 = p.trace[0];
        for (int w = 0; w < k.nw; ++w) {
            fprintf(stderr, "wave %d:", w);
            for (int st = 0; st < std::min(p.n_stages, 24); ++st) {
                const unsigned long long* e = p.trace + (w * 40 + st) * 8;
                fprintf(stderr, " [s%d +%llu w%llu b%llu c%llu i%llu]", st, e[0] - t0, e[1] - e[0], e[2] - e[1], e[3] - e[2], e[4] - e[3]);
            }
            fprintf(stderr, "\n");
        }
    }
#endif
    return rc;
}

}

using namespace mvldm;

extern "C" int mvldm_igemm_skinny_config(const mvldm_igemm_desc* d) {
    if (!d) return 0;
    mvldm_igemm_desc t = *d;
    t.k_order = 2;
    if (!t.weight) t.weight = t.src0;
    if (!skinny_applicable(t)) return 0;
    return sk_choose(t);
}

extern "C" int mvldm_pack_skinny(const void* packed, void* dst, int n_pad, int k_pad, int geglu, int dtype, mvldm_stream_t stream) {
    MVLDM_REQUIRE(packed && dst, "pack_skinny: null pointer");
    MVLDM_REQUIRE(dtype == MVLDM_BF16 || dtype == MVLDM_F16, "pack_skinny: 16-bit types only");
    MVLDM_REQUIRE(n_pad > 0 && n_pad % 64 == 0 && k_pad > 0 && k_pad % 64 == 0, "pack_skinny: n_pad %d / k_pad %d must be multiples of 64", n_pad, k_pad);
    const int n_tiles = n_pad / 16, ksteps = k_pad / 32;
    const size_t total = (size_t)n_tiles * ksteps * 64;
    const int blocks = (int)std::min<size_t>((total + 255) / 256, 8192);
    hipLaunchKernelGGL(pack_skinny_kernel, dim3(blocks), dim3(256), 0, (hipStream_t)stream, reinterpret_cast<const u32x4*>(packed),
                       reinterpret_cast<u32x4*>(dst), n_tiles, ksteps, geglu);
    return check_launch();
}
```

### mv_ldm_amd/modules.py

```python
from __future__ import annotations

import math
import os
from types import SimpleNamespace
from typing import List, Optional, Sequence

import torch
from torch import nn

from . import _lib as L
from . import ops
from .ops import PackedWeight
from .plan import Builder
from .runtime import from_nhwc, get_compute_dtype, require_gpu, to_nhwc


_EPOCH_COUNTER = [0]


def bump_weights_epoch(module=None) -> int:
    _EPOCH_COUNTER[0] += 1
    e = _EPOCH_COUNTER[0]
    if module is None:
        _GLOBAL_FLOOR[0] = e
# ... 57 lines not shown
        return b.conv(x, self.packed(b.dtype, c_tot, None if x2 is None else x.shape[-1]), self._f32("bias"), x2=x2,
                      stride=self.stride[0], pad=self.padding[0], **kw)

    def forward(self, x):
        b = eager_builder(x)
        return from_nhwc(self.emit(b, to_nhwc(x, b.dtype, ops.epc(b.dtype))))


class Linear(nn.Linear, _PackMixin):
    def packed(self, dtype, geglu=False) -> PackedWeight:
        require_gpu(self.weight)
        return self._cache(("w", dtype, geglu), [self.weight], lambda: ops.pack_weight(self.weight, dtype, geglu=geglu))

    def emit(self, b: Builder, x, **kw):
        return b.linear(x, self.packed(b.dtype), self._f32("bias"), **kw)

    def forward(self, x):
        b = eager_builder(x)
        lead = x.shape[:-1]
        x2 = x.reshape(-1, x.shape[-1])
        x2 = x2 if x2.dtype == b.dtype and x2.is_contiguous() else ops.convert(x2.contiguous(), b.dtype)
        return self.emit(b, x2).reshape(*lead, -1)


class GroupNorm(nn.GroupNorm, _PackMixin):
    def emit(self, b: Builder, x, silu=False, x2=None, name="groupnorm"):
        return b.groupnorm(x, self._f32("weight"), self._f32("bias"), self.num_groups, self.eps, silu, x2=x2, name=name)

    def forward(self, x):
        b = eager_builder(x)
        return from_nhwc(self.emit(b, to_nhwc(x, b.dtype)))


class LayerNorm(nn.LayerNorm, _PackMixin):
    def emit(self, b: Builder, x, name="layernorm"):
        return b.layernorm(x, self._f32("weight"), self._f32("bias"), self.eps, name=name)


class SiLU(nn.Module):
    def forward(self, x):
        require_gpu(x)
        if x.ndim == 4:
            return from_nhwc(ops.silu(to_nhwc(x, x.dtype if x.dtype != torch.float64 else torch.float32)))
        return ops.silu(x.contiguous())


class Timesteps(nn.Module):

    def __init__(self, num_channels: int, flip_sin_to_cos: bool = True, downscale_freq_shift: float = 0.0):
        super().__init__()
        self.num_channels, self.flip_sin_to_cos, self.downscale_freq_shift = num_channels, flip_sin_to_cos, downscale_freq_shift
        half = num_channels // 2
        exponent = -math.log(10000) * torch.arange(0, half, dtype=torch.float32) / (half - downscale_freq_shift)
        self.register_buffer("freqs", torch.exp(exponent), persistent=False)

    def emit(self, b: Builder, timesteps, dtype=torch.float32):
        return b.timestep_embed(timesteps, self.freqs, self.num_channels, self.flip_sin_to_cos, dtype)

    def forward(self, timesteps):
        require_gpu(timesteps)
        return ops.timestep_embed(timesteps.to(torch.int64).contiguous(), self.freqs, self.num_channels,
                                  self.flip_sin_to_cos, torch.float32)


class TimestepEmbedding(nn.Module):
    def __init__(self, in_channels: int, time_embed_dim: int):
        super().__init__()
        self.linear_1 = Linear(in_channels, time_embed_dim)
        self.act = nn.SiLU()
        self.linear_2 = Linear(time_embed_dim, time_embed_dim)

    def emit(self, b: Builder, t_emb, silu_out=False):
        h = self.linear_1.emit(b, t_emb, epilogue=L.EPI_SILU, name="time_embedding.linear_1")
        out = self.linear_2.emit(b, h, epilogue=L.EPI_SILU if silu_out else L.EPI_NONE, name="time_embedding.linear_2")
        b.free(h)
        return out

    def forward(self, sample):
        b = eager_builder(sample)
        x = sample if sample.dtype == b.dtype else ops.convert(sample.contiguous(), b.dtype)
        return self.emit(b, x)


class ResnetBlock2D(nn.Module):

    def __init__(self, in_channels, out_channels=None, temb_channels=512, groups=32, eps=1e-6):
        super().__init__()
        out_channels = in_channels if out_channels is None else out_channels
        self.in_channels, self.out_channels = in_channels, out_channels
        self.norm1 = GroupNorm(groups, in_channels, eps=eps)
        self.conv1 = Conv2d(in_channels, out_channels, 3, padding=1)
        self.time_emb_proj = Linear(temb_channels, out_channels) if temb_channels is not None else None
        self.norm2 = GroupNorm(groups, out_channels, eps=eps)
        self.dropout = nn.Dropout(0.0)
        self.conv2 = Conv2d(out_channels, out_channels, 3, padding=1)
        self.nonlinearity = nn.SiLU()
        self.conv_shortcut = Conv2d(in_channels, out_channels, 1) if in_channels != out_channels else None

    def emit(self, b: Builder, x, temb=None, x2=None, temb_proj=None, out=None):
        if self.time_emb_proj is not None and temb_proj is None:
            ta = b.eltwise(temb, L.ELT_SILU, name="temb_silu")
            temb_proj = self.time_emb_proj.emit(b, ta, out_dtype=torch.float32, name="time_emb_proj")
            b.free(ta)
        def main_chain():
            g1 = self.norm1.emit(b, x, silu=True, x2=x2, name="norm1+silu")
            h = self.conv1.emit(b, g1, row_bias=temb_proj, name="conv1")
            b.free(g1)
            g2 = self.norm2.emit(b, h, silu=True, name="norm2+silu")
            b.free(h)
            return g2

        if self.conv_shortcut is None:
            assert x2 is None
            g2, sc = main_chain(), x
        elif b.small_launch(x.shape[0] * x.shape[1] * x.shape[2], self.conv_shortcut.out_channels):
            with b.parallel() as par:
                par.lane()
                g2 = main_chain()
                par.lane()
                sc = self.conv_shortcut.emit(b, x, x2=x2, name="conv_shortcut")
        else:
            g2 = main_chain()
            sc = self.conv_shortcut.emit(b, x, x2=x2, name="conv_shortcut")
        out = self.conv2.emit(b, g2, residual=sc, name="conv2", **({} if out is None else {"out": out}))
        b.free(g2)
        if sc is not x:
            b.free(sc)
        return out

    def forward(self, input_tensor, temb=None):
        b = eager_builder(input_tensor)
        x = to_nhwc(input_tensor, b.dtype)
        if temb is not None and (temb.dtype != b.dtype or not temb.is_contiguous()):
            temb = ops.convert(temb.contiguous(), b.dtype)
        return from_nhwc(self.emit(b, x, temb))


class Attention(nn.Module, _PackMixin):

    def __init__(self, query_dim, cross_attention_dim=None, heads=8, dim_head=64, bias=False, out_bias=True):
        super().__init__()
        inner = heads * dim_head
        self.heads, self.dim_head, self.inner = heads, dim_head, inner
        kv = query_dim if cross_attention_dim is None else cross_attention_dim
        self.to_q = Linear(query_dim, inner, bias=bias)
        self.to_k = Linear(kv, inner, bias=bias)
        self.to_v = Linear(kv, inner, bias=bias)
        self.to_out = nn.ModuleList([Linear(inner, query_dim, bias=out_bias), nn.Dropout(0.0)])

    def _packed_cat(self, dtype, mods: Sequence[Linear]):
        ws = [m.weight for m in mods]
        return self._cache(("cat", dtype, len(mods)), ws, lambda: ops.pack_weight(torch.cat([w.detach() for w in ws], 0), dtype))

    def _bias_cat(self, mods: Sequence[Linear]):
        if mods[0].bias is None:
            return None
        bs = [m.bias for m in mods]
        return self._cache(("bcat", len(mods)), bs, lambda: torch.cat([x.detach().float() for x in bs], 0).contiguous())

    def out_bias(self, extra: Optional[torch.Tensor] = None):
        bo = self.to_out[0].bias
        if extra is None:
            return self.to_out[0]._f32("bias")
        return self._cache(("bsum",), [bo, extra], lambda: (bo.detach().float() + extra.detach().float()).contiguous())

    def emit_self(self, b: Builder, xn, residual, seg, lens, extra_bias=None, name="attn", kv_lens=None):
        C = self.inner
        qkv = b.linear(xn, self._packed_cat(b.dtype, [self.to_q, self.to_k, self.to_v]),
                       self._bias_cat([self.to_q, self.to_k, self.to_v]), name=name + ".to_qkv")
        a = b.attention(qkv[:, :C], qkv[:, C:2 * C], qkv[:, 2 * C:], self.heads, self.dim_head, seg, lens, lens if kv_lens is None else kv_lens,
                        name=name + ".sdpa")
        b.free(qkv)
        out = b.linear(a, self.to_out[0].packed(b.dtype), self.out_bias(extra_bias), residual=residual, name=name + ".to_out")
        b.free(a)
        return out

    def emit_cross(self, b: Builder, xn, ctx, residual, seg, q_lens, kv_lens, name="attn"):
        C = self.inner
        q = self.to_q.emit(b, xn, name=name + ".to_q")
        kv = b.linear(ctx, self._packed_cat(b.dtype, [self.to_k, self.to_v]), self._bias_cat([self.to_k, self.to_v]), name=name + ".to_kv")
        a = b.attention(q, kv[:, :C], kv[:, C:], self.heads, self.dim_head, seg, q_lens, kv_lens, name=name + ".sdpa")
        b.free(q)
        b.free(kv)
        out = b.linear(a, self.to_out[0].packed(b.dtype), self.out_bias(), residual=residual, name=name + ".to_out")
        b.free(a)
        return out


class GEGLU(nn.Module):
    def __init__(self, dim_in, dim_out):
        super().__init__()
        self.proj = Linear(dim_in, dim_out * 2)


class FeedForward(nn.Module):

    def __init__(self, dim, mult=4):
        super().__init__()
        self.net = nn.ModuleList([GEGLU(dim, dim * mult), nn.Dropout(0.0), Linear(dim * mult, dim)])

    def emit(self, b: Builder, xn, residual, name="ff"):
        p = self.net[0].proj
        g = b.linear(xn, p.packed(b.dtype, geglu=True), p._f32("bias"), epilogue=L.EPI_GEGLU, name=name + ".geglu")
        out = self.net[2].emit(b, g, residual=residual, name=name + ".out")
        b.free(g)
# ... 330 lines not shown
```

### mv_ldm_amd/ops.py

```python
from __future__ import annotations

import ctypes as C
import os
from dataclasses import dataclass
from typing import NamedTuple, Optional, Sequence

import math

import numpy as np
import torch

from . import _lib as L

_DT = {torch.float32: L.F32, torch.bfloat16: L.BF16, torch.float16: L.F16}


def dt(t) -> int:
    return _DT[t if isinstance(t, torch.dtype) else t.dtype]


def epc(dtype: torch.dtype) -> int:
    return 4 if dtype == torch.float32 else 8


def stream() -> int:
    return torch.cuda.current_stream().cuda_stream


def ptr(t: Optional[torch.Tensor]) -> Optional[int]:
    return None if t is None else t.data_ptr()


def _roundup(a: int, b: int) -> int:
    return (a + b - 1) // b * b


_WS: dict = {}


def workspace(nbytes: int, device, key: str = "splitk") -> torch.Tensor:
    k = (str(device), key)
    cur = _WS.get(k)
    if cur is None or cur.numel() < nbytes:
        cur = torch.empty(max(nbytes, 1 << 20), dtype=torch.uint8, device=device)
        _WS[k] = cur
    return cur


@dataclass
class PackedWeight:
    data: torch.Tensor
    n_out: int
    n_pad: int
    k_pad: int
    c_pad: int
    ksize: int
    geglu: bool = False
    k_order: int = 0
    _skinny: Optional[torch.Tensor] = None
    _skinny_pinned: bool = False

    def can_skinny(self) -> bool:
        return self.k_order == 1 and self.data.dtype != torch.float32 and self.c_pad % 64 == 0 and self.k_pad == self.ksize * self.ksize * self.c_pad \
            and self.ksize in (1, 2, 3) and self.n_out % 4 == 0

    def skinny(self) -> torch.Tensor:
        if self._skinny is None:
            assert self.can_skinny(), "tile 15 needs a 16-bit block-major pack with channels in multiples of 64"
            out = torch.empty_like(self.data)
            L.check(L.load().mvldm_pack_skinny(self.data.data_ptr(), out.data_ptr(), self.n_pad, self.k_pad, int(self.geglu), dt(self.data), stream()))
            self._skinny = out
        return self._skinny

    def drop_skinny(self):
        if not self._skinny_pinned:
            self._skinny = None


def block_k(dtype: torch.dtype) -> int:
    return 32 if dtype == torch.float32 else 64


def pack_weight_t(w: torch.Tensor, dtype: torch.dtype, c_off: int = 0, n_rows: Optional[int] = None,
                  out: Optional[torch.Tensor] = None) -> PackedWeight:
    assert w.is_cuda and w.dtype == torch.float32 and w.is_contiguous()
    n_out, c_in = w.shape[0], w.shape[1]
    ksize = w.shape[2] if w.ndim == 4 else 1
    n_rows = c_in - c_off if n_rows is None else n_rows
    c_pad = _roundup(n_out, epc(dtype))
    bk = block_k(dtype)
    k_pad = _roundup(ksize * ksize * c_pad, bk)
    n_pad = _roundup(n_rows, 64)
    k_order = int(c_pad % bk == 0)
    data = torch.zeros(n_pad, k_pad, dtype=dtype, device=w.device) if out is None else out
    L.check(L.load().mvldm_pack_weight(w.data_ptr(), data.data_ptr(), n_out, c_in, ksize, c_pad, n_pad, k_pad, 0, k_order, dt(dtype),
                                       1, c_off, n_rows, stream()))
    return PackedWeight(data, n_rows, n_pad, k_pad, c_pad, ksize, False, k_order)


def pack_weight(w: torch.Tensor, dtype: torch.dtype, c_pad: Optional[int] = None, geglu: bool = False,
                c_split: Optional[int] = None, out: Optional[torch.Tensor] = None) -> PackedWeight:
    assert w.is_cuda, "pack_weight needs a device tensor (no CPU path)"
    w = w.detach().to(torch.float32).contiguous()
    n_out, c_in = w.shape[0], w.shape[1]
    ksize = w.shape[2] if w.ndim == 4 else 1
    e = epc(dtype)
    c_pad = _roundup(c_in, e) if c_pad is None else c_pad
    bk = block_k(dtype)
    k_pad = _roundup(ksize * ksize * c_pad, bk)
    n_pad = _roundup(n_out, 64)
    k_order = int(c_pad % bk == 0 and (c_split is None or c_split % bk == 0))
    out = torch.empty(n_pad, k_pad, dtype=dtype, device=w.device) if out is None else out
    L.check(L.load().mvldm_pack_weight(w.data_ptr(), out.data_ptr(), n_out, c_in, ksize, c_pad, n_pad, k_pad,
                                       int(geglu), k_order, dt(dtype), 0, 0, n_out, stream()))
    return PackedWeight(out, n_out, n_pad, k_pad, c_pad, ksize, geglu, k_order)


def pack_job(w: torch.Tensor, pw: PackedWeight, *, transpose: bool = False, c_off: int = 0) -> "L.PackJob":
    assert w.is_cuda and w.dtype == torch.float32 and w.is_contiguous()
    j = L.PackJob()
    j.src, j.dst = w.data_ptr(), pw.data.data_ptr()
    j.n_out, j.c_in, j.ksize = w.shape[0], w.shape[1], pw.ksize
    j.c_pad, j.n_pad, j.k_pad, j.geglu, j.k_order = pw.c_pad, pw.n_pad, pw.k_pad, int(pw.geglu), pw.k_order
    j.transpose, j.c_off, j.n_rows = int(transpose), c_off, (pw.n_out if transpose else w.shape[0])
    L.check(L.load().mvldm_pack_job_prepare(C.byref(j), dt(pw.data.dtype)))
    return j


class PackBatch:

    def __init__(self, jobs: Sequence["L.PackJob"], dtype: torch.dtype, device):
        self.n, self.dtype = len(jobs), dtype
        arr = (L.PackJob * max(len(jobs), 1))()
        b0 = 0
        for i, j in enumerate(jobs):
            C.memmove(C.byref(arr[i]), C.byref(j), C.sizeof(L.PackJob))
            arr[i].block0 = b0
            b0 += j.blocks
        self.total_blocks = b0
        raw = torch.frombuffer(bytearray(bytes(arr)), dtype=torch.uint8).clone()
        self.table = raw.to(device)
        self.block_job = None
        if jobs:
            self.block_job = torch.repeat_interleave(torch.arange(len(jobs), dtype=torch.int32), torch.tensor([j.blocks for j in jobs])).to(device)
            assert self.block_job.numel() == b0

    def run(self):
        L.check(L.load().mvldm_pack_weight_batch(self.table.data_ptr(), self.n, None if self.block_job is None else self.block_job.data_ptr(),
                                                 self.total_blocks, dt(self.dtype), stream()))


def conv_out_hw(h: int, w: int, ksize: int, stride: int, pad: int, upsample) -> tuple:
    if int(upsample) >= 2:
        return h, w
    hs, ws = (2 * h, 2 * w) if upsample else (h, w)
    if ksize == 3 and stride == 2 and pad == 0:
        return (hs + 1 - 3) // 2 + 1, (ws + 1 - 3) // 2 + 1
    return (hs + 2 * pad - ksize) // stride + 1, (ws + 2 * pad - ksize) // stride + 1


def use_skinny(d, pw: PackedWeight) -> torch.Tensor:
    t = pw.skinny()
    d.weight, d.k_order = ptr(t), 2
    return t


def igemm_desc(src0, src1, pw: PackedWeight, dst, *, n_img, h_in, w_in, h_out, w_out, stride=1, pad=None, upsample=False,
               bias=None, row_bias=None, residual=None, epilogue=L.EPI_NONE, out_scale=1.0, ws=None, splitk=0,
               tile=0, into=None) -> L.IgemmDesc:
    d = L.IgemmDesc() if into is None else into
    c0 = src0.shape[-1]
    c1 = 0 if src1 is None else src1.shape[-1]
    assert c0 + c1 == pw.c_pad, f"weight packed for {pw.c_pad} channels, sources give {c0}+{c1}"
    assert not pw.k_order or c0 % block_k(src0.dtype) == 0, "weight packed block-major but the source split is unaligned"
    d.src0, d.src1, d.weight = ptr(src0), ptr(src1), ptr(pw.data)
    d.bias, d.row_bias, d.residual, d.dst = ptr(bias), ptr(row_bias), ptr(residual), ptr(dst)
    d.c0, d.c1 = c0, c1
    d.n_img, d.h_in, d.w_in, d.h_out, d.w_out = n_img, h_in, w_in, h_out, w_out
    d.ksize, d.stride, d.upsample = pw.ksize, stride, int(upsample)
    d.pad = (pw.ksize // 2) if pad is None else pad
    d.n_out, d.n_pad, d.k_pad = pw.n_out, pw.n_pad, pw.k_pad
    d.row_bias_ld = 0 if row_bias is None else row_bias.stride(0)
    d.epilogue, d.act_dtype, d.dst_dtype = epilogue, dt(src0), dt(dst)
    d.splitk, d.tile, d.out_scale = splitk, tile, out_scale
    n_dst = pw.n_out // 2 if epilogue == L.EPI_GEGLU else pw.n_out
    d.dst_ld = 0 if dst.shape[-1] == n_dst else dst.shape[-1]
    d.k_order = pw.k_order
    if (tile & 63) == 15:
        use_skinny(d, pw)
    if ws is not None:
        d.workspace, d.workspace_bytes = ws.data_ptr(), ws.numel() * ws.element_size()
    else:
        d.workspace, d.workspace_bytes = None, 0
        if splitk == 0:
            d.splitk = 1
    return d


def conv2d(x: torch.Tensor, pw: PackedWeight, bias=None, *, x2=None, stride=1, pad=None, upsample=False, row_bias=None,
           residual=None, epilogue=L.EPI_NONE, out_dtype=None, out_scale=1.0, splitk=0, tile=0, out=None, dst=None) -> torch.Tensor:
    assert x.is_cuda and x.is_contiguous() and (x2 is None or x2.is_contiguous())
    n, h, w, _ = x.shape
    pad = (pw.ksize // 2) if pad is None else pad
    ho, wo = conv_out_hw(h, w, pw.ksize, stride, pad, upsample)
    n_dst = pw.n_out // 2 if epilogue == L.EPI_GEGLU else pw.n_out
    if dst is not None:
        up = 2 if int(upsample) >= 2 else 1
        assert out is None and dst.is_contiguous() and dst.dtype == (out_dtype or x.dtype) and dst.shape[-1] > n_dst
        assert dst.numel() == n * up * ho * up * wo * dst.shape[-1]
        out = dst
    elif out is None:
        out = torch.empty(n, ho, wo, n_dst, dtype=out_dtype or x.dtype, device=x.device)
    else:
        assert out.is_contiguous() and out.numel() == n * ho * wo * n_dst and out.dtype == (out_dtype or x.dtype)
        out = out.view(n, ho, wo, n_dst)
    scratch = None
    if splitk != 1:
        scratch = workspace(min(16 * n * ho * wo * pw.n_pad * 4, 256 << 20), x.device)
    d = igemm_desc(x, x2, pw, out, n_img=n, h_in=h, w_in=w, h_out=ho, w_out=wo, stride=stride, pad=pad,
                   upsample=upsample, bias=bias, row_bias=row_bias, residual=residual, epilogue=epilogue,
                   out_scale=out_scale, ws=scratch, splitk=splitk, tile=tile)
    L.check(L.load().mvldm_igemm_fwd(C.byref(d), stream()))
    return out


def upsample_phase_weights(w: torch.Tensor) -> list:
    assert w.ndim == 4 and w.shape[2:] == (3, 3)
    w = w.detach().to(torch.float32)
    rows = {0: (w[:, :, 0], w[:, :, 1] + w[:, :, 2]), 1: (w[:, :, 0] + w[:, :, 1], w[:, :, 2])}
    out = []
    for py in (0, 1):
        for px in (0, 1):
            taps = []
            for r in rows[py]:
                cols = (r[:, :, 0], r[:, :, 1] + r[:, :, 2]) if px == 0 else (r[:, :, 0] + r[:, :, 1], r[:, :, 2])
                taps.append(torch.stack(cols, dim=-1))
            out.append(torch.stack(taps, dim=-2).contiguous())
    return out


def conv2d_upsample_phases(x: torch.Tensor, pws, bias=None, tile=0, splitk=0) -> torch.Tensor:
    n, h, w, _ = x.shape
    out = torch.empty(n, 2 * h, 2 * w, pws[0].n_out, dtype=x.dtype, device=x.device)
    scratch = workspace(min(16 * n * h * w * pws[0].n_pad * 4, 256 << 20), x.device)
    for phase, pw in enumerate(pws):
        d = igemm_desc(x, None, pw, out, n_img=n, h_in=h, w_in=w, h_out=h, w_out=w, stride=1, pad=0, upsample=2 + phase,
                       bias=bias, splitk=splitk, tile=tile, ws=scratch)
        L.check(L.load().mvldm_igemm_fwd(C.byref(d), stream()))
    return out


def linear(x: torch.Tensor, pw: PackedWeight, bias=None, *, residual=None, epilogue=L.EPI_NONE, out_dtype=None,
           splitk=0, tile=0, out=None, dst=None) -> torch.Tensor:
    rows, c = x.shape
    y = conv2d(x.view(rows, 1, 1, c), pw, bias, residual=None if residual is None else residual.view(rows, 1, 1, -1),
               epilogue=epilogue, out_dtype=out_dtype, splitk=splitk, tile=tile, out=out, dst=None if dst is None else dst.view(rows, 1, 1, -1))
    return y.view(rows, -1)


def groupnorm(x: torch.Tensor, gamma, beta, groups: int, eps: float, silu: bool, x2=None, stats_out=None, out=None) -> torch.Tensor:
    assert x.is_cuda and x.is_contiguous() and (x2 is None or x2.is_contiguous())
    n, c0 = x.shape[0], x.shape[-1]
    c1 = 0 if x2 is None else x2.shape[-1]
    hw = math.prod(x.shape[1:-1])
    if out is None:
        y = torch.empty(*x.shape[:-1], c0 + c1, dtype=x.dtype, device=x.device)
    else:
        assert out.is_contiguous() and out.dtype == x.dtype and out.numel() == n * hw * (c0 + c1)
        y = out.view(*x.shape[:-1], c0 + c1)
    ws = workspace(max(n, 1) * L.GN_MAX_CHUNKS * groups * 2 * 8, x.device, "gn")
    L.check(L.load().mvldm_groupnorm_fwd(x.data_ptr(), ptr(x2), y.data_ptr(), gamma.data_ptr(), beta.data_ptr(), n, hw, c0, c1,
                                         groups, eps, int(silu), dt(x), ws.data_ptr(), ptr(stats_out), stream()))
    return y


def layernorm(x: torch.Tensor, gamma, beta, eps: float = 1e-5, out=None) -> torch.Tensor:
    assert x.is_cuda and x.is_contiguous()
    c = x.shape[-1]
    rows = x.numel() // c
    if out is None:
        y = torch.empty_like(x)
    else:
        assert out.is_contiguous() and out.dtype == x.dtype and out.numel() == x.numel()
        y = out.view(x.shape)
    L.check(L.load().mvldm_layernorm_fwd(x.data_ptr(), y.data_ptr(), gamma.data_ptr(), beta.data_ptr(), rows, c, eps,
                                         dt(x), stream()))
    return y


def make_segments(q_lens, kv_lens=None, device="cuda") -> torch.Tensor:
    kv_lens = q_lens if kv_lens is None else kv_lens
    rows, q0, k0 = [], 0, 0
    for ql, kl in zip(q_lens, kv_lens):
        rows.append([q0, ql, k0, kl])
        q0, k0 = q0 + ql, k0 + kl
    return torch.tensor(rows, dtype=torch.int32, device=device)


def attention(q: torch.Tensor, k: torch.Tensor, v: torch.Tensor, heads: int, head_dim: int, seg: torch.Tensor,
              max_q_len: int, scale: Optional[float] = None, lse: Optional[torch.Tensor] = None, out=None) -> torch.Tensor:
    assert q.is_cuda and q.stride(1) == 1 and k.stride(1) == 1 and v.stride(1) == 1
    if out is None:
        out = torch.empty(q.shape[0], heads * head_dim, dtype=q.dtype, device=q.device)
    assert out.stride(1) == 1 and out.dtype == q.dtype and out.shape[1] == heads * head_dim
# ... 892 lines not shown
```

### mv_ldm_amd/plan.py

```python
from __future__ import annotations

import ctypes as C
import json
import os
import sys
from dataclasses import dataclass
from typing import List, Optional

import torch

from . import _lib as L
from .ops import PackedWeight, conv_out_hw, dt, igemm_desc, ptr, use_skinny


def _PIN_TILE() -> int:
    v = os.environ.get("MVLDM_IGEMM_TILE")
    return int(v) if v else 0


@dataclass
class OpMeta:
    name: str
    kind: int
    flops: float = 0.0
    bytes: float = 0.0


class Builder:
    def __init__(self, device, dtype: torch.dtype, record: bool = False, splitk_ws_bytes: int = 256 << 20):
        self.device, self.dtype, self.record = torch.device(device), dtype, record
        self.ops: List[L.Op] = []
        self.meta: List[OpMeta] = []
        self.keep: list = []
        self._pool: dict = {}
        self._ws = None
        self._ws_bytes = splitk_ws_bytes
        self._gn_ws = None
        self._scope: List[str] = []
        self._lane = 0
        self._lane_ws: dict = {}
        self._deferred: Optional[list] = None
        self.skinny = True
        self._skinny_pw: dict = {}

    def empty(self, *shape, dtype=None) -> torch.Tensor:
        dtype = dtype or self.dtype
        if self.record:
            nbytes = int(torch.Size(shape).numel()) * torch.empty(0, dtype=dtype).element_size()
            free = self._pool.get(nbytes)
            if free:
                base = free.pop()
                return base.view(dtype).view(*shape)
        t = torch.empty(*shape, dtype=dtype, device=self.device)
        if self.record:
            self.keep.append(t)
            self.__dict__.setdefault("_own_ptrs", set()).add(t.data_ptr())
        return t

    def free(self, t: Optional[torch.Tensor]):
        if t is None or not self.record:
            return
        base = t.reshape(-1).view(torch.uint8)
        if self._deferred is not None:
            self._deferred.append(base)
            return
        self._pool.setdefault(base.numel(), []).append(base)

    class _Parallel:

        def __init__(self, b):
            self.b, self.n = b, 0

        def __enter__(self):
            assert self.b._deferred is None, "parallel groups do not nest"
            self.b._marker(L.OP_PAR_BEGIN, "par_begin")
            self.b._deferred = []
            return self

        def lane(self):
            if self.n:
                self.b._marker(L.OP_PAR_NEXT, "par_next")
            self.b._lane = self.n
            self.n += 1

        def __exit__(self, *a):
            b = self.b
            b._marker(L.OP_PAR_END, "par_end")
            b._lane = 0
            deferred, b._deferred = b._deferred, None
            for base in deferred:
                b._pool.setdefault(base.numel(), []).append(base)

    def parallel(self):
        return Builder._Parallel(self)

    def _marker(self, kind: int, name: str):
        op = L.Op()
        op.kind = kind
        self._emit(op, name)

    def splitk_ws(self) -> torch.Tensor:
        if self._lane:
            ws = self._lane_ws.get(("splitk", self._lane))
            if ws is None:
                ws = torch.empty(min(self._ws_bytes, 64 << 20), dtype=torch.uint8, device=self.device)
                self._lane_ws[("splitk", self._lane)] = ws
                self.keep.append(ws)
            return ws
        if self._ws is None:
            self._ws = torch.empty(self._ws_bytes, dtype=torch.uint8, device=self.device)
            self.keep.append(self._ws)
        return self._ws

    def gn_ws(self, n_img: int, groups: int) -> torch.Tensor:
        need = n_img * L.GN_MAX_CHUNKS * groups * 16
        if self._lane:
            ws = self._lane_ws.get(("gn", self._lane))
            if ws is None or ws.numel() < need:
                ws = torch.empty(max(need, 1 << 16), dtype=torch.uint8, device=self.device)
                self._lane_ws[("gn", self._lane)] = ws
                self.keep.append(ws)
            return ws
        if self._gn_ws is None or self._gn_ws.numel() < need:
            self._gn_ws = torch.empty(max(need, 1 << 16), dtype=torch.uint8, device=self.device)
            self.keep.append(self._gn_ws)
        return self._gn_ws

    class _Scope:
        def __init__(self, b, name):
            self.b, self.name = b, name

        def __enter__(self):
            self.b._scope.append(self.name)

        def __exit__(self, *a):
            self.b._scope.pop()

    def scope(self, name: str):
        return Builder._Scope(self, name)

    def _emit(self, op: L.Op, name: str, flops=0.0, nbytes=0.0, refs=()):
        if self.record:
            op.tag = len(self.ops)
            self.ops.append(op)
            self.meta.append(OpMeta("/".join(self._scope + [name]), op.kind, flops, nbytes))
            self.keep.extend(r for r in refs if r is not None)
        else:
            L.check(L.load().mvldm_op_run(C.byref(op), torch.cuda.current_stream().cuda_stream))

    def conv(self, x, pw: PackedWeight, bias=None, *, x2=None, stride=1, pad=None, upsample=False, row_bias=None,
             residual=None, epilogue=L.EPI_NONE, out_dtype=None, out_scale=1.0, out=None, name="conv", splitk=0, tile=0):
        n, h, w, c0 = x.shape
        c1 = 0 if x2 is None else x2.shape[-1]
        pad = (pw.ksize // 2) if pad is None else pad
        ho, wo = conv_out_hw(h, w, pw.ksize, stride, pad, upsample)
        n_dst = pw.n_out // 2 if epilogue == L.EPI_GEGLU else pw.n_out
        if out is None:
            out = self.empty(n, ho, wo, n_dst, dtype=out_dtype or x.dtype)
        ws = self.splitk_ws() if splitk != 1 else None
        if tile == 0 and _PIN_TILE() and x.dtype != torch.float32 and pw.k_order == 1:
            tile, splitk = _PIN_TILE(), 1
        m = n * ho * wo
        k_real = pw.ksize * pw.ksize * (c0 + c1)
        es = x.element_size()
        nbytes = (pw.n_out * k_real + n * h * w * (c0 + c1)) * es + m * n_dst * out.element_size() \
            + (m * n_dst * es if residual is not None else 0)
        self._igemm(x, x2, pw, bias, row_bias, residual, out, ws, name, 2.0 * m * pw.n_out * k_real, nbytes, h_out=ho, w_out=wo,
                    stride=stride, pad=pad, upsample=upsample, epilogue=epilogue, out_scale=out_scale, splitk=splitk, tile=tile)
        return out

    def _igemm(self, x, x2, pw, bias, row_bias, residual, out, ws, name, flops, nbytes, *, h_out, w_out, tile=0, **desc):
        n, h, w, c0 = x.shape
        c1 = 0 if x2 is None else x2.shape[-1]
        op = L.Op()
        op.kind = L.OP_IGEMM
        d = igemm_desc(x, x2, pw, out, n_img=n, h_in=h, w_in=w, h_out=h_out, w_out=w_out, bias=bias, row_bias=row_bias,
                       residual=residual, ws=ws, tile=tile, into=op.u.igemm, **desc)
        m = n * h_out * w_out
        can_sk = tile == 0 and self.skinny and skinny_candidate(pw, m, c0, c1, d.upsample, x.dtype) \
            and x.is_cuda and L.load().mvldm_igemm_skinny_config(C.byref(d)) > 0
        if can_sk and skinny_rule(m, pw.n_pad):
            tile = d.tile = 15
            use_skinny(d, pw)
        elif can_sk and self.record:
            self._skinny_pw[len(self.ops)] = pw
        if self.record:
            own = self.__dict__.get("_own_ptrs", ())
            self.__dict__.setdefault("_tune_srcs", {})[len(self.ops)] = tuple(t if (t is not None and t.data_ptr() in own) else None
                                                                              for t in (x, x2))
        self._emit(op, name, flops, nbytes, (x, x2, pw.data, pw._skinny if (tile & 63) == 15 else None, bias, row_bias, residual, out))

    def small_launch(self, rows: int, n_out: int) -> bool:
        limit = int(os.environ.get("MVLDM_PAR_ROWS", "0"))
        return self.record and rows * max(n_out, 1) <= limit * 640 and limit > 0

    def conv_upsample_phases(self, x, pws, bias=None, name="upsample"):
        n, h, w, c0 = x.shape
        out = self.empty(n, 2 * h, 2 * w, pws[0].n_out, dtype=x.dtype)
        lanes = self.parallel() if self.small_launch(n * h * w, pws[0].n_out) else None
        if lanes is not None:
            lanes.__enter__()
        for phase, pw in enumerate(pws):
            if lanes is not None:
                lanes.lane()
            self._phase_conv(x, pw, bias, out, phase, name)
        if lanes is not None:
            lanes.__exit__(None, None, None)
        return out

    def _phase_conv(self, x, pw, bias, out, phase, name, tile=0, splitk=0):
        n, h, w, c0 = x.shape
        ws = self.splitk_ws()
        assert pw.ksize == 2 and pw.k_order == 1 and c0 == pw.c_pad
        m = n * h * w
        es = x.element_size()
        nbytes = (pw.n_out * 4 * c0 + (m * c0 if phase == 0 else 0)) * es + m * pw.n_out * es
        self._igemm(x, None, pw, bias, None, None, out, ws, f"{name}.p{phase}", 2.0 * m * pw.n_out * 4 * c0, nbytes, h_out=h, w_out=w,
                    stride=1, pad=0, upsample=2 + phase, splitk=splitk, tile=tile)

    def linear(self, x, pw: PackedWeight, bias=None, *, residual=None, epilogue=L.EPI_NONE, out_dtype=None, out=None,
               name="linear", row_bias=None):
        rows, c = x.shape
        y = self.conv(x.view(rows, 1, 1, c), pw, bias, residual=None if residual is None else residual.view(rows, 1, 1, -1),
                      epilogue=epilogue, out_dtype=out_dtype, out=None if out is None else out.view(rows, 1, 1, -1),
                      name=name, row_bias=row_bias)
        return y.view(rows, -1)

    def groupnorm(self, x, gamma, beta, groups, eps, silu, x2=None, name="groupnorm", stats_out=None):
        n, c0 = x.shape[0], x.shape[-1]
        c1 = 0 if x2 is None else x2.shape[-1]
        hw = x.numel() // (n * c0)
        y = self.empty(*x.shape[:-1], c0 + c1, dtype=x.dtype)
        op = L.Op()
        op.kind = L.OP_GROUPNORM
        g = op.u.groupnorm
        g.x, g.x1, g.y, g.gamma, g.beta = ptr(x), ptr(x2), ptr(y), ptr(gamma), ptr(beta)
        g.stats_ws = self.gn_ws(n, groups).data_ptr()
        g.n_img, g.hw, g.c0, g.c1, g.groups, g.silu, g.dtype, g.eps = n, hw, c0, c1, groups, int(silu), dt(x), eps
        g.stats_out = ptr(stats_out)
        passes = L.load().mvldm_groupnorm_passes(n, hw, c0 + c1, groups, dt(x))
        self._emit(op, name, 0.0, float(passes) * y.numel() * y.element_size(), (x, x2, y, gamma, beta, stats_out))
        return y

    def layernorm(self, x, gamma, beta, eps=1e-5, name="layernorm"):
        c = x.shape[-1]
        rows = x.numel() // c
        y = self.empty(*x.shape, dtype=x.dtype)
        op = L.Op()
        op.kind = L.OP_LAYERNORM
        l = op.u.layernorm
        l.x, l.y, l.gamma, l.beta, l.rows, l.c, l.dtype, l.eps = ptr(x), ptr(y), ptr(gamma), ptr(beta), rows, c, dt(x), eps
        self._emit(op, name, 0.0, 2.0 * y.numel() * y.element_size(), (x, y, gamma, beta))
        return y

    def attention(self, q, k, v, heads, head_dim, seg, q_lens, kv_lens, scale=None, name="attention", lse=None, out=None):
        assert q.stride(1) == 1 and k.stride(1) == 1 and v.stride(1) == 1
        if out is None:
            out = self.empty(q.shape[0], heads * head_dim, dtype=q.dtype)
        op = L.Op()
        op.kind = L.OP_ATTENTION
        a = op.u.attention
        a.q, a.k, a.v, a.out, a.seg = ptr(q), ptr(k), ptr(v), ptr(out), ptr(seg)
        a.ld_q, a.ld_k, a.ld_v, a.ld_o = q.stride(0), k.stride(0), v.stride(0), out.stride(0)
        a.heads, a.head_dim, a.n_seg, a.max_q_len, a.dtype = heads, head_dim, seg.shape[0], max(q_lens), dt(q)
        a.scale = head_dim ** -0.5 if scale is None else scale
        a.lse, a.lse_ld = ptr(lse), (0 if lse is None else lse.stride(0))
        pairs = sum(ql * kl for ql, kl in zip(q_lens, kv_lens))
        es = q.element_size()
        nbytes = (sum(q_lens) * 2 + sum(kv_lens) * 2) * heads * head_dim * es
        self._emit(op, name, 4.0 * pairs * heads * head_dim, nbytes, (q, k, v, out, seg, lse))
        return out

    def attention_merge(self, oa, lse_a, ob, lse_b, out, a_img, b_img, out_img, tokens, heads, head_dim, name="attention_merge"):
# ... 43 lines not shown

    def ddim_advance(self, step_ptr, t_table, timesteps, tgt_rows, name="ddim_advance"):
        op = L.Op()
        op.kind = L.OP_DDIM_ADVANCE
        a = op.u.advance
        a.step_ptr, a.t_table, a.timesteps, a.tgt_rows = ptr(step_ptr), ptr(t_table), ptr(timesteps), ptr(tgt_rows)
        a.n_steps, a.n_rows = t_table.numel(), 0 if tgt_rows is None else tgt_rows.numel()
        self._emit(op, name, 0.0, 0.0, (step_ptr, t_table, timesteps, tgt_rows))

    def memcpy(self, dst, src, name="memcpy"):
        assert dst.is_contiguous() and src.is_contiguous() and dst.numel() * dst.element_size() == src.numel() * src.element_size()
        op = L.Op()
        op.kind = L.OP_MEMCPY
        op.u.memcpy_.src, op.u.memcpy_.dst, op.u.memcpy_.bytes = ptr(src), ptr(dst), src.numel() * src.element_size()
        self._emit(op, name, 0.0, 2.0 * src.numel() * src.element_size(), (dst, src))

    def gather_rows(self, src, dst, src_index=None, dst_index=None, n_rows=None, name="gather_rows"):
        idx = src_index if src_index is not None else dst_index
        n = int(n_rows if n_rows is not None else (idx.numel() if idx is not None else dst.shape[0]))
        row_bytes = dst[0].numel() * dst.element_size()
        assert src[0].numel() * src.element_size() == row_bytes and row_bytes % 16 == 0 and dst.is_contiguous() and src.is_contiguous()
        assert all(i is None or (i.dtype == torch.int32 and i.numel() == n) for i in (src_index, dst_index))
        assert (src_index is not None or src.shape[0] >= n) and (dst_index is not None or dst.shape[0] >= n)
        op = L.Op()
        op.kind = L.OP_GATHER_ROWS
        g = op.u.gather
        g.src, g.dst, g.src_index, g.dst_index, g.row_bytes, g.n_rows = ptr(src), ptr(dst), ptr(src_index), ptr(dst_index), row_bytes, n
        self._emit(op, name, 0.0, 2.0 * n * row_bytes, (src, dst, src_index, dst_index))

    def nhwc_to_nchw(self, src, dst, c=None, c_off=0, scale=1.0, shift=0.0, clamp01=False, name="nhwc_to_nchw"):
        n, h, w, sc = src.shape
        op = L.Op()
        op.kind = L.OP_NHWC_TO_NCHW
        l = op.u.layout
        l.src, l.dst, l.n_img, l.c, l.hw, l.other_c, l.other_c_off, l.dtype = ptr(src), ptr(dst), n, c or sc, h * w, sc, c_off, dt(src)
        l.clamp01, l.scale, l.shift = int(clamp01), scale, shift
        self._emit(op, name, 0.0, src.numel() * src.element_size() + dst.numel() * 4, (src, dst))
        return dst

    def nchw_to_nhwc(self, src, dst, c_off=0, scale=1.0, shift=0.0, img_map=None, name="nchw_to_nhwc"):
        n, c, h, w = src.shape
        op = L.Op()
        op.kind = L.OP_NCHW_TO_NHWC
        l = op.u.layout
        l.src, l.dst, l.n_img, l.c, l.hw, l.other_c, l.other_c_off, l.dtype = ptr(src), ptr(dst), n, c, h * w, dst.shape[-1], c_off, dt(dst)
        l.scale, l.shift, l.img_map = scale, shift, ptr(img_map)
        self._emit(op, name, 0.0, src.numel() * 4 + src.numel() * dst.element_size(), (src, dst, img_map))
        return dst

    def ray_encode(self, extr, intr, h, w, out_nhwc, c_off, img_map=None, out_nchw=None, name="ray_encode", mode=0, n_origin_octaves=0,
                   n_dir_octaves=0, plucker=False):
        op = L.Op()
        op.kind = L.OP_RAY_ENCODE
        r = op.u.rays
        r.extrinsics, r.intrinsics, r.out_nchw, r.out_nhwc, r.img_map = ptr(extr), ptr(intr), ptr(out_nchw), ptr(out_nhwc), ptr(img_map)
        r.n_cam, r.h, r.w = extr.shape[0], h, w
        r.nhwc_c, r.nhwc_c_off, r.nhwc_dtype = (0, 0, L.F32) if out_nhwc is None else (out_nhwc.shape[-1], c_off, dt(out_nhwc))
        r.mode, r.n_origin_octaves, r.n_dir_octaves, r.plucker = mode, n_origin_octaves, n_dir_octaves, int(plucker)
        self._emit(op, name, 0.0, extr.shape[0] * h * w * 6 * 4.0, (extr, intr, out_nhwc, out_nchw, img_map))

    def posterior_sample(self, moments, noise, out, scale=1.0, name="posterior_sample"):
        n, c2, h, w = moments.shape
        op = L.Op()
        op.kind = L.OP_POSTERIOR_SAMPLE
        q = op.u.posterior
        q.moments, q.noise, q.out, q.n, q.c, q.hw, q.scale = ptr(moments), ptr(noise), ptr(out), n, c2 // 2, h * w, scale
        self._emit(op, name, 0.0, moments.numel() * 4 * 2.0, (moments, noise, out))
        return out

    def finalize(self, autotune: Optional[bool] = None) -> "Plan":
        assert self.record
        if autotune is None:
            autotune = os.environ.get("MVLDM_AUTOTUNE", "1") != "0"
        if autotune and torch.device(self.device).type == "cuda":
            autotune_igemm(self.ops, srcs=self.__dict__.get("_tune_srcs"), skinny=self._skinny_pw, keep=self.keep)
            autotune_wgrad(self.ops)
            if type(self) is Builder and _BATCH_SPLIT:
                self.ops, self.meta = autosplit_igemm(self.ops, self.meta, skinny=self._skinny_pw, keep=self.keep)
        return Plan(self.ops, self.meta, self.keep, self.device)


_TUNE_CACHE = {}
_WGRAD_CACHE = {}
_SPLIT_CACHE = {}
_VALIDATED = set()
_TUNE_TILES = tuple(int(t) for t in os.environ["MVLDM_TUNE_TILES"].split(",")) if os.environ.get("MVLDM_TUNE_TILES") else (0, 1, 2, 3, 4, 5, 6, 7, 8, 9, 10, 11, 12, 13, 14)


def tune_cache_state() -> dict:
    return {"version": 2, "igemm": {json.dumps(list(k)): (int(v) if isinstance(v, int) else list(v)) for k, v in _TUNE_CACHE.items()},
            "wgrad": {json.dumps(list(k)): int(v) for k, v in _WGRAD_CACHE.items()},
            "split": {json.dumps(list(k)): int(v) for k, v in _SPLIT_CACHE.items()}}


def set_tune_cache_state(state: dict, replace: bool = False) -> None:
    if replace:
        _TUNE_CACHE.clear()
        _WGRAD_CACHE.clear()
        _SPLIT_CACHE.clear()
    for name, cache in (("igemm", _TUNE_CACHE), ("wgrad", _WGRAD_CACHE), ("split", _SPLIT_CACHE)):
        for k, v in (state.get(name) or {}).items():
            cache[tuple(json.loads(k))] = int(v) if isinstance(v, int) else list(v)


def save_tune_cache(path: Optional[str] = None) -> Optional[str]:
    path = path or os.environ.get("MVLDM_TUNE_CACHE")
    if not path:
        return None
    tmp = f"{path}.{os.getpid()}.tmp"
    with open(tmp, "w") as f:
        json.dump(tune_cache_state(), f, indent=0, sort_keys=True)
    os.replace(tmp, path)
    return path


def load_tune_cache(path: Optional[str] = None) -> int:
    path = path or os.environ.get("MVLDM_TUNE_CACHE")
    if not path or not os.path.exists(path):
        return 0
    with open(path) as f:
        set_tune_cache_state(json.load(f))
    return len(_TUNE_CACHE) + len(_WGRAD_CACHE) + len(_SPLIT_CACHE)


def broadcast_tune_cache(dist, src: int = 0, device=None) -> None:
    box = [tune_cache_state() if dist.get_rank() == src else None]
    dist.broadcast_object_list(box, src=src, device=device)
    set_tune_cache_state(box[0], replace=True)


load_tune_cache()


def _igemm_signature(d) -> tuple:
    return (d.n_img, d.h_in, d.w_in, d.h_out, d.w_out, d.c0, d.c1, d.ksize, d.stride, d.pad, d.upsample, d.n_out, d.n_pad,
            d.k_pad, d.epilogue, d.act_dtype, d.dst_dtype, d.k_order, d.dst_ld, bool(d.residual), bool(d.row_bias),
            bool(d.bias), d.splitk, d.workspace_bytes)


_SMALL_ROWS = int(os.environ.get("MVLDM_TUNE_SMALL_ROWS", "64"))
_SPLITS = (0, 1, 2, 4, 8, 16, 32)
_MID_ROWS = int(os.environ.get("MVLDM_TUNE_MID_ROWS", "40000"))
_MID_SPLITS = (0, 1, 2, 3, 4, 6, 8)
_SMALL_TILES = tuple(int(t) for t in os.environ.get("MVLDM_TUNE_SMALL_TILES", "0,1,2,3,4,5").split(","))


_SKINNY = os.environ.get("MVLDM_SKINNY", "1") != "0"
_SKINNY_ROWS = int(os.environ.get("MVLDM_SKINNY_ROWS", "2304"))
_SKINNY_CFGS = tuple(int(c) for c in os.environ.get("MVLDM_SKINNY_CFGS", "0,1,2,5,6,7,8,9,10,12,13,18,19,20,38,39,40,41,42,43,44,46").split(","))


def skinny_rule(rows: int, n_pad: int) -> bool:
    if os.environ.get("MVLDM_AUTOTUNE", "1") != "0" or os.environ.get("MVLDM_SKINNY_RULE", "1") == "0":
        return False
    return rows <= 160 or (rows <= 1152 and n_pad <= 1280)


def skinny_candidate(pw: PackedWeight, rows: int, c0: int, c1: int, upsample, dtype) -> bool:
    return (_SKINNY and dtype != torch.float32 and rows <= _SKINNY_ROWS and not (upsample is True or upsample == 1) and pw.can_skinny()
            and c0 % 64 == 0 and c1 % 64 == 0)


def _unpack_choice(v):
    return (int(v), None) if isinstance(v, int) else (int(v[0]), None if v[1] is None else int(v[1]))


_TUNE_COLD = int(os.environ.get("MVLDM_TUNE_COLD", "9216"))
_THRASH = []
_THRASH_FILLS = [0]


def _thrash(device=None):
    if not _THRASH or (device is not None and _THRASH[0].device != torch.device(device)):
        _THRASH[:] = [torch.empty(640 << 20, dtype=torch.uint8, device=torch.cuda.current_device() if device is None else device)]
    return _THRASH[0]


def autotune_igemm(ops, min_rows: int = 2048, iters: int = 4, srcs=None, skinny=None, keep=None) -> int:
    lib = L.load()
    stream = torch.cuda.current_stream().cuda_stream
    e0, e1 = torch.cuda.Event(enable_timing=True), torch.cuda.Event(enable_timing=True)
    timed = 0
    tune_dev = next((t.device for pair in (srcs or {}).values() for t in pair if t is not None), None)
    if srcs:
        seen, gen = set(), None
        for pair in srcs.values():
            for t in pair:
                if t is not None and t.is_floating_point() and t.data_ptr() not in seen:
                    seen.add(t.data_ptr())
                    if gen is None:
                        gen = torch.Generator(device=t.device)
                        gen.manual_seed(0x5EED)
                    t.normal_(generator=gen)
    for idx, op in enumerate(ops):
        if op.kind != L.OP_IGEMM:
            continue
        d = op.u.igemm
        rows = d.n_img * d.h_out * d.w_out
        sk_pw = (skinny or {}).get(idx)
        if d.tile != 0 or d.act_dtype == L.F32 or d.k_order != 1 or (rows < min(min_rows, _SMALL_ROWS) and sk_pw is None):
            continue
        small = rows < min_rows
        key = _igemm_signature(d) + (("sk",) if sk_pw is not None else ())
        best = _TUNE_CACHE.get(key)
        if best is not None and (_unpack_choice(best)[0] & 63) not in (set(_TUNE_TILES) | set(_SMALL_TILES) | {17, 19} | ({15} if sk_pw is not None else set())):
            best = None
        if best is None:
            trial = L.Op()
            C.memmove(C.byref(trial), C.byref(op), C.sizeof(L.Op))
            can_split = small and bool(d.workspace) and d.splitk == 0
            mid = (not small) and rows < _MID_ROWS and bool(d.workspace) and d.splitk == 0
            cands = [(t, sk) for t in _TUNE_TILES for sk in _MID_SPLITS] if mid else [(t, None) for t in _TUNE_TILES] if not small else \
                    [(t, sk) for t in _SMALL_TILES if t in _TUNE_TILES or not os.environ.get("MVLDM_TUNE_TILES") for sk in (_SPLITS if can_split else (None,))]
            n_it = iters if not small else 3 * iters
            cold = _TUNE_COLD > 0 and rows <= _TUNE_COLD
            if not small and 17 not in _TUNE_TILES and not os.environ.get("MVLDM_TUNE_TILES") and d.ksize == 3 and d.stride == 1 \
                    and d.src1 is None and not d.upsample and d.w_in <= 24:
                cands = cands + [(17, None)]
            if not small and d.ksize == 1 and not os.environ.get("MVLDM_TUNE_TILES"):
                cands = cands + [(19, None), (13 | (1 << 13), None)]
# ... 23 lines not shown
                e0.record()
                for _ in range(n_it):
                    lib.mvldm_op_run(C.byref(trial), stream)
                e1.record()
                e1.synchronize()
                results.append((e0.elapsed_time(e1), tile, sk))
            t_rule = next(t for t, tile, sk in results if tile == 0 and sk in (None, 0))
            t_best, tile_best, sk_best = min(results, key=lambda r: r[0])
            best = [tile_best, sk_best] if t_best < 0.97 * t_rule else [0, None]
            _TUNE_CACHE[key] = best
            _VALIDATED.add(key)
            timed += 1
        tile, sk = _unpack_choice(best)
        if tile != 0 and key not in _VALIDATED:
            trial = L.Op()
            C.memmove(C.byref(trial), C.byref(op), C.sizeof(L.Op))
            trial.u.igemm.tile = tile
            if sk is not None:
                trial.u.igemm.splitk = sk
            if (tile & 63) == 15:
                if sk_pw is None:
                    tile, sk = 0, None
                else:
                    use_skinny(trial.u.igemm, sk_pw)
            if tile != 0 and lib.mvldm_op_run(C.byref(trial), stream) != 0:
                tile, sk = 0, None
                _TUNE_CACHE[key] = [0, None]
            _VALIDATED.add(key)
        d.tile = tile
        if sk is not None:
            d.splitk = sk
        if (tile & 63) == 15:
            t = use_skinny(d, sk_pw)
            sk_pw._skinny_pinned = True
            if keep is not None:
                keep.append(t)
        elif sk_pw is not None:
            sk_pw.drop_skinny()
    if timed:
        save_tune_cache()
        _THRASH.clear()
    return timed


_BATCH_SPLIT = os.environ.get("MVLDM_BATCH_SPLIT", "1") != "0"
_SPLIT_MIN_ROWS = int(os.environ.get("MVLDM_BATCH_SPLIT_MIN_ROWS", "16384"))


def _split_candidates(d) -> list:
    rpi = d.h_out * d.w_out
    rows = d.n_img * rpi
    out = []
    for bn in (320, 256):
        n_tiles = -(-d.n_pad // bn)
        m_tiles = -(-rows // 256)
        if m_tiles * n_tiles <= 256 or (m_tiles * n_tiles) % 256 == 0 or (m_tiles * n_tiles) % 256 > 216:
            continue
        for m1 in range(m_tiles - 1, 0, -1):
            if (m1 * n_tiles) % 256 == 0 and (m1 * 256) % rpi == 0:
                n1 = m1 * 256 // rpi
                frac = 1.0 - n1 / d.n_img
                if 0.03 <= frac <= 0.45 and n1 not in out:
                    out.append(n1)
                break
    return out


def _image_range(op, i0: int, n: int):
    q = L.Op()
    C.memmove(C.byref(q), C.byref(op), C.sizeof(L.Op))
    d = q.u.igemm
    es = 4 if d.act_dtype == L.F32 else 2
    ds = 4 if d.dst_dtype == L.F32 else 2
    n_dst = d.n_out // 2 if d.epilogue == L.EPI_GEGLU else d.n_out
    px_in, px_out = d.h_in * d.w_in, d.h_out * d.w_out

    def off(p, nbytes):
        return (p + nbytes) if p else p
    d.src0 = off(d.src0, i0 * px_in * d.c0 * es)
    d.src1 = off(d.src1, i0 * px_in * d.c1 * es)
    d.dst = off(d.dst, i0 * px_out * (d.dst_ld or n_dst) * ds)
    d.residual = off(d.residual, i0 * px_out * n_dst * es)
    d.row_bias = off(d.row_bias, i0 * d.row_bias_ld * 4)
    d.n_img = n
    d.tile, d.splitk = 0, 0
    return q


def _time_ops(ops, iters: int) -> float:
    lib = L.load()
    stream = torch.cuda.current_stream().cuda_stream
    e0, e1 = torch.cuda.Event(enable_timing=True), torch.cuda.Event(enable_timing=True)
    for o in ops:
        L.check(lib.mvldm_op_run(C.byref(o), stream))
    e0.record()
    for _ in range(iters):
        for o in ops:
            lib.mvldm_op_run(C.byref(o), stream)
    e1.record()
    e1.synchronize()
    return e0.elapsed_time(e1) / iters


def autosplit_igemm(ops, meta, skinny=None, keep=None, iters: int = 6):
    new_ops, new_meta, decided = [], [], 0
    for idx, (op, m) in enumerate(zip(ops, meta)):
        d = op.u.igemm if op.kind == L.OP_IGEMM else None
        rows = d.n_img * d.h_out * d.w_out if d is not None else 0
        ok = (d is not None and rows >= _SPLIT_MIN_ROWS and d.act_dtype != L.F32 and d.k_order == 1 and d.stride == 1 and not d.upsample
              and (d.tile & 63) != 15 and not _PIN_TILE() and bool(d.workspace) and idx not in (skinny or {}))
        n1 = 0
        if ok:
            key = _igemm_signature(d)[:-2] + (d.workspace_bytes,)
            if key in _SPLIT_CACHE:
                n1 = _SPLIT_CACHE[key]
            else:
                best_t, t_whole = None, None
                for cand in _split_candidates(d):
                    parts = [_image_range(op, 0, cand), _image_range(op, cand, d.n_img - cand)]
                    try:
                        autotune_igemm(parts, iters=4)
                        if t_whole is None:
                            t_whole = _time_ops([op], iters)
                        t = _time_ops(parts, iters)
                    except L.MvldmError:
                        continue
                    if os.environ.get("MVLDM_BATCH_SPLIT_LOG"):
                        print(f"[batch split] {m.name}: {d.n_img} images x {d.h_out}x{d.w_out}, N {d.n_out}, K {d.k_pad}: whole {t_whole * 1e3:.1f} us (tile {d.tile & 63}, "
                              f"splitk {d.splitk}); {cand} + {d.n_img - cand}: {t * 1e3:.1f} us (tiles {parts[0].u.igemm.tile & 63} / {parts[1].u.igemm.tile & 63}, "
                              f"splitk {parts[1].u.igemm.splitk})", file=sys.stderr, flush=True)
                    if t < 0.97 * t_whole and (best_t is None or t < best_t):
                        best_t, n1 = t, cand
                _SPLIT_CACHE[key] = n1
                decided += 1
        if n1:
            parts = [_image_range(op, 0, n1), _image_range(op, n1, d.n_img - n1)]
            autotune_igemm(parts, iters=4)
            for k, (q, i0, cnt) in enumerate(zip(parts, (0, n1), (n1, d.n_img - n1))):
                q.tag = len(new_ops)
                new_ops.append(q)
                share = cnt / d.n_img
                new_meta.append(OpMeta(m.name if k == 0 else m.name + "[rest]", m.kind, m.flops * share, m.bytes * share))
        else:
            op.tag = len(new_ops)
            new_ops.append(op)
            new_meta.append(m)
    if decided:
        save_tune_cache()
    return new_ops, new_meta


_WGRAD_TARGETS = tuple(int(t) for t in os.environ.get("MVLDM_TUNE_WGRAD_TARGETS", "0,1,2,3,4,5").split(","))


def autotune_wgrad(ops, iters: int = 3) -> int:
    lib = L.load()
    stream = torch.cuda.current_stream().cuda_stream
    e0, e1 = torch.cuda.Event(enable_timing=True), torch.cuda.Event(enable_timing=True)
    timed = 0
    scratch = None
    for op in ops:
        if op.kind != L.OP_WGRAD:
            continue
        d = op.u.wgrad
        if d.act_dtype == L.F32 or (d.accumulate >> 8) & 3:
            continue
        key = (d.c0, d.c1, d.n_img, d.h_in, d.w_in, d.h_out, d.w_out, d.ksize, d.stride, d.pad, d.upsample, d.n_out, d.dy_ld, d.act_dtype,
               int(d.workspace_bytes), d.accumulate & 1)
        best = _WGRAD_CACHE.get(key)
        if best is None:
            trial = L.Op()
            C.memmove(C.byref(trial), C.byref(op), C.sizeof(L.Op))
            need = d.n_out * d.c_in * d.ksize * d.ksize
            if scratch is None or scratch.numel() < need:
                scratch = torch.zeros(need, dtype=torch.float32, device=torch.cuda.current_device())
            else:
                scratch[:need].zero_()
            trial.u.wgrad.grad = scratch.data_ptr()
            results = []
            for form in (1, 2):
                for tcode in _WGRAD_TARGETS:
                    v = form + 4 * tcode
                    trial.u.wgrad.accumulate = (d.accumulate & 1) | (v << 8)
                    if lib.mvldm_op_run(C.byref(trial), stream) != 0:
                        break
                    e0.record()
                    for _ in range(iters):
                        lib.mvldm_op_run(C.byref(trial), stream)
                    e1.record()
                    e1.synchronize()
                    results.append((e0.elapsed_time(e1), v))
            best = min(results)[1] if results else 0
            _WGRAD_CACHE[key] = best
            timed += 1
        d.accumulate = (d.accumulate & 1) | (best << 8)
    if timed:
# ... 52 lines not shown
```

Baseline: 50.54.

## Fold 1x1 shortcut conv into 3x3 conv2 as extra K tail

Adds a K-tail path to the LDS-DMA implicit-GEMM kernel so a ResNet block's second 3x3 conv can also consume the block input channels as extra K tiles. This folds the 1x1 shortcut conv and the residual add into one GEMM. It removes one GEMM launch and the write-then-reread of the shortcut output. In exchange, the folded kernel is restricted to tiles 7/9/10 with no split-K, and the plan chooses fold or pair per shape by autotuned timing.

```diff
diff --git a/include/mvldm.h b/include/mvldm.h
--- a/include/mvldm.h
+++ b/include/mvldm.h
@@ -46,9 +46,15 @@
     int32_t dst_ld;
     float out_scale;
     size_t workspace_bytes;
+    const void* tail0;
+    const void* tail1;
+    int32_t tail_c0, tail_c1;
+    int32_t tail_k;
+    int32_t tail_reserved;
 } mvldm_igemm_desc;
 int mvldm_igemm_fwd(const mvldm_igemm_desc* d, mvldm_stream_t stream);
 size_t mvldm_igemm_workspace_bytes(const mvldm_igemm_desc* d);
+int mvldm_igemm_tail_tiles(void);
 
 int mvldm_pack_weight(const float* src, void* dst, int n_out, int c_in, int ksize, int c_pad, int n_pad,
                       int k_pad, int geglu, int k_order, int dst_dtype, int transpose, int c_off, int n_rows,
diff --git a/mv_ldm_amd/_lib.py b/mv_ldm_amd/_lib.py
--- a/mv_ldm_amd/_lib.py
+++ b/mv_ldm_amd/_lib.py
@@ -36,7 +36,8 @@
                 ("ksize", i32), ("stride", i32), ("pad", i32), ("upsample", i32),
                 ("n_out", i32), ("n_pad", i32), ("k_pad", i32),
                 ("row_bias_ld", i32), ("epilogue", i32), ("act_dtype", i32), ("dst_dtype", i32),
-                ("splitk", i32), ("tile", i32), ("k_order", i32), ("dst_ld", i32), ("out_scale", f32), ("workspace_bytes", sz)]
+                ("splitk", i32), ("tile", i32), ("k_order", i32), ("dst_ld", i32), ("out_scale", f32), ("workspace_bytes", sz),
+                ("tail0", vp), ("tail1", vp), ("tail_c0", i32), ("tail_c1", i32), ("tail_k", i32), ("tail_reserved", i32)]
 
 
 class _GroupNorm(C.Structure):
@@ -189,6 +190,7 @@
     "mvldm_device_info": (C.c_int, [C.POINTER(C.c_int), C.POINTER(sz), C.c_char_p, C.c_int]),
     "mvldm_igemm_fwd": (C.c_int, [C.POINTER(IgemmDesc), vp]),
     "mvldm_igemm_workspace_bytes": (sz, [C.POINTER(IgemmDesc)]),
+    "mvldm_igemm_tail_tiles": (C.c_int, []),
     "mvldm_pack_weight": (C.c_int, [vp, vp] + [C.c_int] * 12 + [vp]),
     "mvldm_pack_skinny": (C.c_int, [vp, vp, C.c_int, C.c_int, C.c_int, C.c_int, vp]),
     "mvldm_igemm_skinny_config": (C.c_int, [C.POINTER(IgemmDesc)]),
diff --git a/mv_ldm_amd/csrc/igemm.hip b/mv_ldm_amd/csrc/igemm.hip
--- a/mv_ldm_amd/csrc/igemm.hip
+++ b/mv_ldm_amd/csrc/igemm.hip
@@ -171,10 +171,31 @@
     splitk = std::max(1, std::min(splitk, k_tiles));
 }
 
+static bool igemm_tail_tile(int tile) { return tile == 7 || tile == 9 || tile == 10; }
+static int log2_exact(int v) { int s = 0; while ((1 << s) < v) ++s; return (1 << s) == v ? s : -1; }
+
 static int fill_params(const mvldm_igemm_desc& d, IgemmParams& p, int& tile) {
     const int epc = d.act_dtype == MVLDM_F32 ? 4 : 8;
     const int bk = d.act_dtype == MVLDM_F32 ? 32 : 64;
     MVLDM_REQUIRE(d.src0 && d.weight && d.dst, "igemm: null pointer");
+    const bool tail = d.tail0 != nullptr;
+    const int tail_c = tail ? d.tail_c0 + d.tail_c1 : 0;
+    MVLDM_REQUIRE(tail || (!d.tail1 && !d.tail_c0 && !d.tail_c1 && !d.tail_k), "igemm: tail fields without tail0");
+    if (tail) {
+        MVLDM_REQUIRE(d.act_dtype != MVLDM_F32, "igemm: a K tail needs a 16-bit activation type");
+        MVLDM_REQUIRE(d.k_order == 1, "igemm: a K tail needs the block-major pack (k_order 1), not k_order %d", d.k_order);
+        MVLDM_REQUIRE(d.stride == 1, "igemm: a K tail needs stride 1, not %d", d.stride);
+        MVLDM_REQUIRE(d.ksize == 3 && d.pad == 1 && !d.upsample && !d.src1 && d.h_out == d.h_in && d.w_out == d.w_in,
+                      "igemm: a K tail follows a one-source 3x3 / pad-1 conv without upsampling");
+        MVLDM_REQUIRE((d.tail_c1 == 0) == (d.tail1 == nullptr) && d.tail_c0 > 0 && d.tail_c0 % 64 == 0 && d.tail_c1 % 64 == 0 && d.c0 % 64 == 0,
+                      "igemm: tail channels (%d,%d) must be multiples of 64", d.tail_c0, d.tail_c1);
+        MVLDM_REQUIRE(d.tail_k == 9 * d.c0 && d.k_pad == d.tail_k + tail_c, "igemm: tail_k %d / k_pad %d (3x3 part %d, tail %d)", d.tail_k, d.k_pad,
+                      9 * d.c0, tail_c);
+        MVLDM_REQUIRE(d.splitk <= 1, "igemm: a K tail runs in one K pass (splitk %d)", d.splitk);
+        MVLDM_REQUIRE((d.tile & 63) == 0 || igemm_tail_tile(d.tile & 63), "igemm: tile %d does not take a K tail (tiles 7, 9, 10)", d.tile & 63);
+        MVLDM_REQUIRE(!((d.tile >> 12) & 1), "igemm: a K tail needs the LDS-DMA loop");
+        MVLDM_REQUIRE(d.dst != d.tail0 && d.dst != d.tail1, "igemm: dst aliases a tail source");
+    }
     const bool phase = d.upsample >= 2;
     MVLDM_REQUIRE(d.upsample >= 0 && d.upsample <= 5, "igemm: upsample %d", d.upsample);
     MVLDM_REQUIRE(phase ? (d.ksize == 2 && d.stride == 1 && d.h_out == d.h_in && d.w_out == d.w_in && !d.src1 && !d.residual &&
@@ -184,7 +205,7 @@
     MVLDM_REQUIRE(d.stride == 1 || d.stride == 2, "igemm: stride %d", d.stride);
     MVLDM_REQUIRE(d.c0 % epc == 0 && d.c1 % epc == 0 && d.c0 > 0, "igemm: channels (%d,%d) must be multiples of %d", d.c0, d.c1, epc);
     MVLDM_REQUIRE((d.c1 == 0) == (d.src1 == nullptr), "igemm: src1/c1 mismatch");
-    MVLDM_REQUIRE(d.k_pad % bk == 0 && d.k_pad >= d.ksize * d.ksize * (d.c0 + d.c1), "igemm: k_pad %d", d.k_pad);
+    MVLDM_REQUIRE(d.k_pad % bk == 0 && d.k_pad >= d.ksize * d.ksize * (d.c0 + d.c1) + tail_c, "igemm: k_pad %d", d.k_pad);
     MVLDM_REQUIRE(d.n_pad % 64 == 0 && d.n_pad >= d.n_out, "igemm: n_pad %d (n_out %d)", d.n_pad, d.n_out);
     MVLDM_REQUIRE(d.dst_dtype == d.act_dtype || d.dst_dtype == MVLDM_F32, "igemm: dst dtype");
     if (d.epilogue == MVLDM_EPI_GEGLU)
@@ -206,13 +227,36 @@
     p.out_scale = d.out_scale;
     p.dst_ld = d.dst_ld > 0 ? d.dst_ld : p.n_dst;
     MVLDM_REQUIRE(p.dst_ld >= p.n_dst, "igemm: dst_ld %d < n_dst %d", p.dst_ld, p.n_dst);
-    p.k_tiles = d.k_pad / bk;
+    p.k_tiles = (d.k_pad - tail_c) / bk;
+    p.tail0 = d.tail0; p.tail1 = d.tail1;
+    p.tail_tiles = tail_c / 64; p.tail_t0 = tail ? d.tail_c0 / 64 : 0;
+    p.tail0_bytes = p.tail1_bytes = 0;
+    p.tail_sl0 = p.tail_sr0 = p.tail_sl1 = p.tail_sr1 = 0;
+    if (tail) {
+        const int tc[2] = {d.tail_c0, d.tail_c1};
+        int* sl[2] = {&p.tail_sl0, &p.tail_sl1};
+        int* sr[2] = {&p.tail_sr0, &p.tail_sr1};
+        for (int i = 0; i < 2; ++i) {
+            if (!tc[i]) continue;
+            const int from = i ? d.tail_c0 : d.c0;
+            const int up = tc[i] >= from ? log2_exact(tc[i] / from) : -1, dn = tc[i] < from ? log2_exact(from / tc[i]) : -1;
+            MVLDM_REQUIRE(log2_exact(std::max(tc[i], d.c0) / std::min(tc[i], d.c0)) >= 0 && std::max(tc[i], d.c0) % std::min(tc[i], d.c0) == 0 &&
+                              ((tc[i] >= from && tc[i] % from == 0 && up >= 0) || (tc[i] < from && from % tc[i] == 0 && dn >= 0)),
+                          "igemm: tail channels %d against c0 %d: the ratio must be a power of two", tc[i], d.c0);
+            if (up >= 0) *sl[i] = up; else *sr[i] = dn;
+        }
+        const double t0 = (double)d.n_img * d.h_in * d.w_in * d.tail_c0 * 2.0, t1 = (double)d.n_img * d.h_in * d.w_in * d.tail_c1 * 2.0;
+        MVLDM_REQUIRE(t0 < 4.0e9 && t1 < 4.0e9, "igemm: a tail source of %.2f GB exceeds the 4 GB range of the 16-bit loop", std::max(t0, t1) / 1e9);
+        p.tail0_bytes = (unsigned)t0; p.tail1_bytes = (unsigned)t1;
+    }
     tile = d.tile & 63;
     t_force_sync = (d.tile >> 12) & 1;
     const int force_px = (d.tile >> 8) & 15;
     int splitk = d.splitk;
     MVLDM_REQUIRE(((tile >= 0 && tile <= kNumTiles) || tile == 17 || deep_tile(tile)) && splitk >= 0, "igemm: tile/splitk");
+    if (tail) splitk = 1;
     choose_config(d, p.M, p.k_tiles, tile, splitk, d.workspace_bytes);
+    if (tail && !igemm_tail_tile(tile)) tile = 7;
     if (splitk > 1)
         MVLDM_REQUIRE(d.workspace && (size_t)splitk * p.M * d.n_pad * sizeof(float) <= d.workspace_bytes,
                       "igemm: split-K workspace too small");
@@ -264,11 +308,14 @@
         MVLDM_REQUIRE(p.ty0 + p.cy >= 0 && p.tx0 + p.cx >= 0 && hc < d.h_in && wc < d.w_in,
                       "igemm: conv geometry (pad %d, stride %d) not supported", d.pad, d.stride);
     }
+    if (tail)
+        MVLDM_REQUIRE(p.use_bl && p.stage_epi && p.splitk == 1 && igemm_tail_tile(tile),
+                      "igemm: a K tail needs the lean 16-bit loop, an 8-aligned 16-bit output and tile 7, 9 or 10 (got tile %d)", tile);
     p.tiles_m = cdiv(p.M, kTiles[tile].bm);
     p.tiles_n = cdiv(d.n_pad, kTiles[tile].bn);
     p.korder = d.k_order;
     if (d.k_order)
-        MVLDM_REQUIRE(d.k_order == 1 && p.ctot % bk == 0 && d.c0 % bk == 0 && d.k_pad == p.taps * p.ctot,
+        MVLDM_REQUIRE(d.k_order == 1 && p.ctot % bk == 0 && d.c0 % bk == 0 && d.k_pad == p.taps * p.ctot + tail_c,
                       "igemm: k_order 1 needs channel counts (%d,%d) multiples of %d", d.c0, d.c1, bk);
     {
         const double a_bytes = (double)d.n_img * d.h_in * d.w_in * p.ctot, w_bytes = (double)d.n_pad * d.k_pad;
@@ -312,6 +359,7 @@
     int tile = 0;
     if (d.n_img == 0 || d.h_out == 0 || d.w_out == 0) return MVLDM_OK;
     const int req = d.tile & 63;
+    MVLDM_REQUIRE(!d.tail0 || !(req == 15 || req == 12 || req == 13 || req == 14 || req == 19), "igemm: tile %d does not take a K tail (tiles 7, 9, 10)", req);
     if (req == 15) return skinny_run(d, s);
     if (req == 12 || req == 13 || req == 14 || req == 19) {
         MVLDM_REQUIRE(d.src0 && d.weight && d.dst, "igemm: null pointer");
@@ -353,6 +401,12 @@
     return igemm_run(*d, (hipStream_t)stream);
 }
 
+extern "C" int mvldm_igemm_tail_tiles(void) {
+    int m = 0;
+    for (int t = 1; t < 32; ++t) m |= igemm_tail_tile(t) ? 1 << t : 0;
+    return m;
+}
+
 extern "C" size_t mvldm_igemm_workspace_bytes(const mvldm_igemm_desc* d) {
     if (!d) return 0;
     const size_t M = (size_t)d->n_img * d->h_out * d->w_out;
diff --git a/mv_ldm_amd/csrc/igemm_bl.h b/mv_ldm_amd/csrc/igemm_bl.h
--- a/mv_ldm_amd/csrc/igemm_bl.h
+++ b/mv_ldm_amd/csrc/igemm_bl.h
@@ -142,7 +142,7 @@
     unsigned mask[UPS ? 1 : A_IT];
 };
 
-template <typename T, int BM, int BN, int NW, int KS, bool DUAL, int A_IT, int B_IT, int STAGES, bool UPS, int t, int LO = 0, int HI = 1 << 20>
+template <typename T, int BM, int BN, int NW, int KS, bool DUAL, int A_IT, int B_IT, int STAGES, bool UPS, int t, int LO = 0, int HI = 1 << 20, bool TAILK = false>
 __device__ __forceinline__ void bl_issue(const IgemmParams& p, char* stage_base, int wave, int cb,
                                          const BlAddr<KS * KS, A_IT, DUAL, UPS>& ad, const unsigned (&vb)[B_IT]) {
     constexpr int BK = 64, TAPS = KS * KS;
@@ -182,6 +182,35 @@
                                                  vb[it], koff, 0, 0);
 }
 
+template <typename T, int BM, int BN, int NW, int A_IT, int B_IT, int STAGES, int LO = 0, int HI = 1 << 20>
+__device__ __forceinline__ void bl_issue_tail(const IgemmParams& p, char* stage_base, int wave, int tj,
+                                              BlAddr<9, A_IT, false, false>& ad, const unsigned (&vb)[B_IT]) {
+    const bool second = tj >= p.tail_t0;
+    if (tj == 0 || tj == p.tail_t0) {
+        const int sl = second ? p.tail_sl1 : p.tail_sl0, sr = second ? p.tail_sr1 : p.tail_sr0;
+#pragma unroll
+        for (int it = (LO > 0 ? LO : 0); it < (HI < A_IT ? HI : A_IT); ++it) {
+            const unsigned a = ad.a0[0][it];
+            ad.a0[0][it] = ((ad.mask[it] >> 4) & 1u) ? ((((a & ~127u) << sl) >> sr) | (a & 127u)) : kBufOob;
+        }
+    }
+    const __amdgpu_buffer_rsrc_t rt = __builtin_amdgcn_make_buffer_rsrc(
+        const_cast<void*>(second ? p.tail1 : p.tail0), 0, second ? p.tail1_bytes : p.tail0_bytes, 0x00020000);
+    const __amdgpu_buffer_rsrc_t rw = __builtin_amdgcn_make_buffer_rsrc(const_cast<void*>(p.weight), 0, p.w_bytes, 0x00020000);
+    const int soff = (second ? tj - p.tail_t0 : tj) * 128;
+    char* at = stage_base;
+    char* bt = at + BM * 128;
+#pragma unroll
+    for (int it = (LO > 0 ? LO : 0); it < (HI < A_IT ? HI : A_IT); ++it)
+        __builtin_amdgcn_raw_ptr_buffer_load_lds(rt, (__attribute__((address_space(3))) void*)(at + (wave + NW * it) * 1024), 16,
+                                                 ad.a0[0][it], soff, 0, 0);
+    const int koff = (p.k_tiles + tj) * 128;
+#pragma unroll
+    for (int it = (LO > A_IT ? LO - A_IT : 0); it < (HI - A_IT < B_IT ? HI - A_IT : B_IT); ++it)
+        __builtin_amdgcn_raw_ptr_buffer_load_lds(rw, (__attribute__((address_space(3))) void*)(bt + (wave + NW * it) * 1024), 16,
+                                                 vb[it], koff, 0, 0);
+}
+
 template <typename T, int BM, int BN, int WM, int WN>
 __device__ __forceinline__ void bl_compute(const char* stage_base, f32x16 (&acc)[BM / WM / 32][BN / WN / 32], int wm, int wn,
                                            int hi, int l31) {
@@ -207,10 +236,11 @@
     }
 }
 
-template <typename T, int BM, int BN, int WM, int WN, int KS, bool DUAL, int STAGES, bool UPS>
+template <typename T, int BM, int BN, int WM, int WN, int KS, bool DUAL, int STAGES, bool UPS, bool TAIL = false>
 __global__ __launch_bounds__(WM* WN * 64) void igemm_bl_kernel(const IgemmParams p) {
     using M_ = Mma<T>;
     static_assert(sizeof(T) == 2, "16-bit activation types only");
+    static_assert(!TAIL || (KS == 3 && !DUAL && !UPS && STAGES <= 3), "the K tail follows a one-source 3x3 phase on the 2 / 3-slot loops");
     constexpr int NW = WM * WN, TAPS = KS * KS;
     constexpr int BK = 64, EPC = 8;
     constexpr int TM = BM / WM / 32, TN = BN / WN / 32;
@@ -225,6 +255,7 @@
     if (!map_block(p, split, tm, tn)) return;
     const int cb0 = split * (p.k_tiles_per_split / TAPS);
     const int cb1 = min(cb0 + p.k_tiles_per_split / TAPS, p.k_tiles / TAPS);
+    const int ntail = TAIL ? p.tail_tiles : 0;
 
     const int slot = lane & 7, rsub = lane >> 3;
     BlAddr<TAPS, A_IT, DUAL, UPS> ad;
@@ -279,16 +310,33 @@
             for (int r = 0; r < 16; ++r) acc[i][j][r] = 0.f;
 
 #define MVLDM_BL_ISSUE(stage_, cb_, t_) \
-    bl_issue<T, BM, BN, NW, KS, DUAL, A_IT, B_IT, STAGES, UPS, t_>(p, smem + (stage_) * STAGE_BYTES, wave, cb_, ad, vb)
+    bl_issue<T, BM, BN, NW, KS, DUAL, A_IT, B_IT, STAGES, UPS, t_, 0, 1 << 20, TAIL>(p, smem + (stage_) * STAGE_BYTES, wave, cb_, ad, vb)
 #define MVLDM_BL_ISSUE_R(stage_, cb_, t_, lo_, hi_) \
-    bl_issue<T, BM, BN, NW, KS, DUAL, A_IT, B_IT, STAGES, UPS, t_, lo_, hi_>(p, smem + (stage_) * STAGE_BYTES, wave, cb_, ad, vb)
+    bl_issue<T, BM, BN, NW, KS, DUAL, A_IT, B_IT, STAGES, UPS, t_, lo_, hi_, TAIL>(p, smem + (stage_) * STAGE_BYTES, wave, cb_, ad, vb)
 #define MVLDM_BL_NEXT(t_, d_) (((t_) + (d_)) % TAPS)
+#define MVLDM_BL_ISSUE_TAIL(stage_, tj_, lo_, hi_) \
+    bl_issue_tail<T, BM, BN, NW, A_IT, B_IT, STAGES, lo_, hi_>(p, smem + (stage_) * STAGE_BYTES, wave, tj_, ad, vb)
+#define MVLDM_BL_TIDX(t_, d_) ((cb + ((t_) + (d_)) / TAPS - cb1) * TAPS + MVLDM_BL_NEXT(t_, d_))
+#define MVLDM_BL_HAS_P(t_, d_) (cb + ((t_) + (d_)) / TAPS < cb1 || (TAIL && MVLDM_BL_TIDX(t_, d_) < ntail))
+#define MVLDM_BL_AHEAD_P(stage_, t_, d_, lo_, hi_)                                                                \
+    {                                                                                                             \
+                   \
+        const int cbn_ = cb + ((t_) + (d_)) / TAPS;                                                               \
+        if (cbn_ < cb1) { MVLDM_BL_ISSUE_R(stage_, cbn_, MVLDM_BL_NEXT(t_, d_), lo_, hi_); }                      \
+        else if constexpr (TAIL) {                                                                                \
+            if (MVLDM_BL_TIDX(t_, d_) < ntail) { MVLDM_BL_ISSUE_TAIL(stage_, MVLDM_BL_TIDX(t_, d_), lo_, hi_); }  \
+        }                                                                                                         \
+    }
+#define MVLDM_BL_HAS_T(t_, d_) (tj + (d_) < ntail)
+#define MVLDM_BL_AHEAD_T(stage_, t_, d_, lo_, hi_) \
+    if constexpr (TAIL) { if (tj + (d_) < ntail) { MVLDM_BL_ISSUE_TAIL(stage_, tj + (d_), lo_, hi_); } }
 #define MVLDM_BL_LOAD(f_, slot_, kk_) bl_load<T, BM, BN, WM, WN>(smem + (slot_) * STAGE_BYTES, f_, kk_, wm, wn, hi, l31)
 #define MVLDM_BL_MMA(f_)                  \
     __builtin_amdgcn_sched_barrier(0);    \
     bl_mma<T, TM, TN>(f_, acc);           \
     __builtin_amdgcn_sched_barrier(0);
-#define MVLDM_BL_STEP(t_)                                                                                         \
+#define MVLDM_BL_STEP(t_) MVLDM_BL_STEP_X(t_, MVLDM_BL_HAS_P, MVLDM_BL_AHEAD_P)
+#define MVLDM_BL_STEP_X(t_, HAS_, AHEAD_)                                                                         \
     {                                                                                                             \
         static_assert(64 / M_::KI == 4, "four k-sub-steps per K-tile");                                          \
         MVLDM_BL_LOAD(f1, slot_c, 1);                                                                             \
@@ -299,14 +347,10 @@
         MVLDM_BL_MMA(f0)                                                                                          \
             \
                              \
-        if (STAGES == 3 && cb + ((t_) + 2) / TAPS < cb1) asm volatile("s_waitcnt vmcnt(%0) lgkmcnt(0)" ::"n"(LPT) : "memory"); \
+        if (STAGES == 3 && HAS_(t_, 2)) asm volatile("s_waitcnt vmcnt(%0) lgkmcnt(0)" ::"n"(LPT) : "memory");     \
         else asm volatile("s_waitcnt vmcnt(0) lgkmcnt(0)" ::: "memory");                                          \
         __builtin_amdgcn_s_barrier();                                                                             \
-        {                                                                                                         \
-                   \
-            const int cbn_ = cb + ((t_) + STAGES) / TAPS;                                                         \
-            if (cbn_ < cb1) { MVLDM_BL_ISSUE(slot_c, cbn_, MVLDM_BL_NEXT(t_, STAGES)); }                          \
-        }                                                                                                         \
+        AHEAD_(slot_c, t_, STAGES, 0, 1 << 20)                                                                    \
         slot_c = slot_c + 1 == STAGES ? 0 : slot_c + 1;                                                           \
         MVLDM_BL_LOAD(f0, slot_c, 0);                                                                             \
         MVLDM_BL_MMA(f1)                                                                                          \
@@ -318,31 +362,29 @@
 #else
     constexpr bool SPREAD_S = NW == 8;
 #endif
-#define MVLDM_BL_STEP_SIMPLE(t_)                                                                                  \
+#define MVLDM_BL_STEP_SIMPLE(t_) MVLDM_BL_STEP_SIMPLE_X(t_, MVLDM_BL_HAS_P, MVLDM_BL_AHEAD_P)
+#define MVLDM_BL_STEP_SIMPLE_X(t_, HAS_, AHEAD_)                                                                  \
     {                                                                                                             \
         asm volatile("s_waitcnt vmcnt(0) lgkmcnt(0)" ::: "memory");                                               \
         __builtin_amdgcn_s_barrier();                                                                             \
         if constexpr (!SPREAD_S) {                                                                                \
-            const int cbn_ = cb + ((t_) + 1) / TAPS;                                                              \
-            if (cbn_ < cb1) { MVLDM_BL_ISSUE(slot_c ^ 1, cbn_, MVLDM_BL_NEXT(t_, 1)); }                           \
+            AHEAD_(slot_c ^ 1, t_, 1, 0, 1 << 20)                                                                 \
             bl_compute<T, BM, BN, WM, WN>(smem + slot_c * STAGE_BYTES, acc, wm, wn, hi, l31);                     \
         } else {                                                                                                  \
             constexpr int Q0_ = (4 * LPT + 8) / 9, Q1_ = Q0_ + (LPT - Q0_ + 1) / 2;                              \
-            const int cbn_ = cb + ((t_) + 1) / TAPS;                                                              \
-            const bool more_ = cbn_ < cb1;                                                                        \
-            if (more_) { MVLDM_BL_ISSUE_R(slot_c ^ 1, cbn_, MVLDM_BL_NEXT(t_, 1), 0, Q0_); }                      \
+            AHEAD_(slot_c ^ 1, t_, 1, 0, Q0_)                                                                     \
             {                                                                                                     \
                 BlFrags<T, TM, TN> fs_;                                                                           \
                 MVLDM_BL_LOAD(fs_, slot_c, 0);                                                                    \
                 bl_mma<T, TM, TN>(fs_, acc);                                                                      \
             }                                                                                                     \
-            if (more_) { MVLDM_BL_ISSUE_R(slot_c ^ 1, cbn_, MVLDM_BL_NEXT(t_, 1), Q0_, Q1_); }                    \
+            AHEAD_(slot_c ^ 1, t_, 1, Q0_, Q1_)                                                                   \
             {                                                                                                     \
                 BlFrags<T, TM, TN> fs_;                                                                           \
                 MVLDM_BL_LOAD(fs_, slot_c, 1);                                                                    \
                 bl_mma<T, TM, TN>(fs_, acc);                                                                      \
             }                                                                                                     \
-            if (more_) { MVLDM_BL_ISSUE_R(slot_c ^ 1, cbn_, MVLDM_BL_NEXT(t_, 1), Q1_, LPT); }                    \
+            AHEAD_(slot_c ^ 1, t_, 1, Q1_, LPT)                                                                   \
             {                                                                                                     \
                 BlFrags<T, TM, TN> fs_;                                                                           \
                 MVLDM_BL_LOAD(fs_, slot_c, 2);                                                                    \
@@ -397,6 +439,9 @@
                     MVLDM_BL_STEP_SIMPLE(5) MVLDM_BL_STEP_SIMPLE(6) MVLDM_BL_STEP_SIMPLE(7) MVLDM_BL_STEP_SIMPLE(8)
                 }
             }
+            if constexpr (TAIL) {
+                for (int tj = 0; tj < ntail; ++tj) { MVLDM_BL_STEP_SIMPLE_X(0, MVLDM_BL_HAS_T, MVLDM_BL_AHEAD_T) }
+            }
         }
     } else if (cb0 < cb1) {
         MVLDM_BL_ISSUE(0, cb0, 0);
@@ -420,8 +465,19 @@
                 MVLDM_BL_STEP(5) MVLDM_BL_STEP(6) MVLDM_BL_STEP(7) MVLDM_BL_STEP(8)
             }
         }
+        if constexpr (TAIL) {
+            for (int tj = 0; tj < ntail; ++tj) { MVLDM_BL_STEP_X(0, MVLDM_BL_HAS_T, MVLDM_BL_AHEAD_T) }
+        }
     }
 #undef MVLDM_BL_STEP_SIMPLE
+#undef MVLDM_BL_STEP_SIMPLE_X
+#undef MVLDM_BL_STEP_X
+#undef MVLDM_BL_ISSUE_TAIL
+#undef MVLDM_BL_TIDX
+#undef MVLDM_BL_HAS_P
+#undef MVLDM_BL_AHEAD_P
+#undef MVLDM_BL_HAS_T
+#undef MVLDM_BL_AHEAD_T
 #undef MVLDM_BL_STEP_DEEP
 #undef MVLDM_BL_PRO
 #undef MVLDM_BL_LOAD
@@ -446,16 +502,17 @@
                          8 * p.sub_m * p.sub_n * p.splitk, WM * WN * 64, p, s);
 }
 
-template <typename T, int BM, int BN, int WM, int WN, int KS, bool DUAL, int STAGES, bool UPS>
+template <typename T, int BM, int BN, int WM, int WN, int KS, bool DUAL, int STAGES, bool UPS, bool TAIL = false>
 static int launch_bl_s(const IgemmParams& p, hipStream_t s) {
     static std::atomic<uint64_t> done{0};
     constexpr int ring = STAGES * (BM + BN) * 128, park = WM * WN * 32 * (park_blocks(BN / WN / 32) * 32 + 4) * 4;
-    return launch_kernel(igemm_bl_kernel<T, BM, BN, WM, WN, KS, DUAL, STAGES, UPS>, done, ring > park ? ring : park,
+    return launch_kernel(igemm_bl_kernel<T, BM, BN, WM, WN, KS, DUAL, STAGES, UPS, TAIL>, done, ring > park ? ring : park,
                          8 * p.sub_m * p.sub_n * p.splitk, WM * WN * 64, p, s);
 }
-template <typename T, int BM, int BN, int WM, int WN, int KS, bool DUAL, int DEPTH = 0>
+template <typename T, int BM, int BN, int WM, int WN, int KS, bool DUAL, int DEPTH = 0, bool TAIL = false>
 static int launch_bl(const IgemmParams& p, hipStream_t s) {
     constexpr int STAGES = DEPTH ? DEPTH : ((WM * WN == 8 && 3 * (BM + BN) * 128 <= 160 * 1024) ? 3 : 2);
+    if constexpr (TAIL) return launch_bl_s<T, BM, BN, WM, WN, KS, DUAL, STAGES, false, true>(p, s);
     if (p.upsample) {
         if constexpr (KS == 3 && !DUAL && ((BM == 128 && BN == 64) || (BM == 256 && BN == 128)))
             return launch_bl_s<T, BM, BN, WM, WN, KS, DUAL, STAGES, true>(p, s);
@@ -479,6 +536,12 @@
         else
             return set_error(MVLDM_ERR_ARG, "igemm: 2x2 phase conv needs tile 2, 7 or 10");
     }
+    if (p.tail_tiles) {
+        if constexpr (BM == 256 && BN >= 128 && WM == 4 && WN == 2) {
+            if (p.ksize == 3 && !dual && !p.upsample) return launch_bl<T, BM, BN, WM, WN, 3, false, 0, true>(p, s);
+        }
+        return set_error(MVLDM_ERR_UNSUPPORTED, "igemm: a K tail needs a one-source 3x3 conv on tile 7, 9 or 10");
+    }
     if (p.ksize == 3) {
         if (!dual) return launch_bl<T, BM, BN, WM, WN, 3, false>(p, s);
         if constexpr (BM == 256 && BN >= 256)
diff --git a/mv_ldm_amd/csrc/igemm_common.h b/mv_ldm_amd/csrc/igemm_common.h
--- a/mv_ldm_amd/csrc/igemm_common.h
+++ b/mv_ldm_amd/csrc/igemm_common.h
@@ -27,6 +27,10 @@
     unsigned src0_bytes, src1_bytes, w_bytes;
     int use_bl, stage_epi;
     int nt_store;
+    const void* tail0; const void* tail1;
+    unsigned tail0_bytes, tail1_bytes;
+    int tail_tiles, tail_t0;
+    int tail_sl0, tail_sr0, tail_sl1, tail_sr1;
 };
 
 template <typename T> struct Mma;
diff --git a/mv_ldm_amd/csrc/skinny.hip b/mv_ldm_amd/csrc/skinny.hip
--- a/mv_ldm_amd/csrc/skinny.hip
+++ b/mv_ldm_amd/csrc/skinny.hip
@@ -818,7 +818,7 @@
 using namespace mvldm;
 
 extern "C" int mvldm_igemm_skinny_config(const mvldm_igemm_desc* d) {
-    if (!d) return 0;
+    if (!d || d->tail0) return 0;
     mvldm_igemm_desc t = *d;
     t.k_order = 2;
     if (!t.weight) t.weight = t.src0;
diff --git a/mv_ldm_amd/modules.py b/mv_ldm_amd/modules.py
--- a/mv_ldm_amd/modules.py
+++ b/mv_ldm_amd/modules.py
@@ -163,7 +163,7 @@
         return self.emit(b, x)
 
 
-class ResnetBlock2D(nn.Module):
+class ResnetBlock2D(nn.Module, _PackMixin):
 
     def __init__(self, in_channels, out_channels=None, temb_channels=512, groups=32, eps=1e-6):
         super().__init__()
@@ -177,6 +177,17 @@
         self.conv2 = Conv2d(out_channels, out_channels, 3, padding=1)
         self.nonlinearity = nn.SiLU()
         self.conv_shortcut = Conv2d(in_channels, out_channels, 1) if in_channels != out_channels else None
+
+    def folded(self, dtype):
+        c2, cs = self.conv2, self.conv_shortcut
+        if cs is None or dtype == torch.float32 or c2.in_channels % 64 or cs.in_channels % 64:
+            return None, None
+        pw = self._cache(("fold", dtype), [c2.weight, cs.weight], lambda: ops.pack_weight_fold(c2.weight, cs.weight, dtype))
+        bias = None
+        if c2.bias is not None or cs.bias is not None:
+            bs = [m.bias for m in (c2, cs) if m.bias is not None]
+            bias = self._cache(("fold_bias",), bs, lambda: sum(p.detach().float() for p in bs).contiguous())
+        return pw, bias
 
     def emit(self, b: Builder, x, temb=None, x2=None, temb_proj=None, out=None):
         if self.time_emb_proj is not None and temb_proj is None:
@@ -202,6 +213,14 @@
                 sc = self.conv_shortcut.emit(b, x, x2=x2, name="conv_shortcut")
         else:
             g2 = main_chain()
+            c_tot = x.shape[-1] + (0 if x2 is None else x2.shape[-1])
+            pwf, biasf = self.folded(b.dtype) if hasattr(b, "fold_shortcut") else (None, None)
+            if pwf is not None and b.fold_shortcut(g2, x, x2, out, self.conv2.packed(b.dtype, g2.shape[-1]),
+                                                   self.conv_shortcut.packed(b.dtype, c_tot, None if x2 is None else x.shape[-1]), pwf,
+                                                   self.conv2._f32("bias"), self.conv_shortcut._f32("bias"), biasf):
+                out = b.conv(g2, pwf, biasf, tail=(x, x2), name="conv2+shortcut", **({} if out is None else {"out": out}))
+                b.free(g2)
+                return out
             sc = self.conv_shortcut.emit(b, x, x2=x2, name="conv_shortcut")
         out = self.conv2.emit(b, g2, residual=sc, name="conv2", **({} if out is None else {"out": out}))
         b.free(g2)
diff --git a/mv_ldm_amd/ops.py b/mv_ldm_amd/ops.py
--- a/mv_ldm_amd/ops.py
+++ b/mv_ldm_amd/ops.py
@@ -57,6 +57,7 @@
     ksize: int
     geglu: bool = False
     k_order: int = 0
+    tail_c: int = 0
     _skinny: Optional[torch.Tensor] = None
     _skinny_pinned: bool = False
 
@@ -116,6 +117,22 @@
     return PackedWeight(out, n_out, n_pad, k_pad, c_pad, ksize, geglu, k_order)
 
 
+def fold_offered(dtype: torch.dtype, c_mid: int, tail_cs: Sequence[int]) -> bool:
+    def pow2_ratio(a, b):
+        hi, lo = max(a, b), min(a, b)
+        return lo > 0 and hi % lo == 0 and (hi // lo) & (hi // lo - 1) == 0
+    return dtype != torch.float32 and c_mid % 64 == 0 and 1 <= len(tail_cs) <= 2 and all(c % 64 == 0 and pow2_ratio(c, c_mid) for c in tail_cs)
+
+
+def pack_weight_fold(w3: torch.Tensor, w1: torch.Tensor, dtype: torch.dtype) -> PackedWeight:
+    assert w3.ndim == 4 and w3.shape[2:] == (3, 3) and w1.shape[0] == w3.shape[0] and dtype != torch.float32
+    a = pack_weight(w3, dtype)
+    b = pack_weight(w1.reshape(w1.shape[0], -1), dtype)
+    assert a.k_order == 1 and b.k_pad == b.c_pad and b.c_pad % 64 == 0 and a.n_pad == b.n_pad, "fold needs channel counts in multiples of 64"
+    data = torch.cat([a.data, b.data], dim=1).contiguous()
+    return PackedWeight(data, a.n_out, a.n_pad, a.k_pad + b.k_pad, a.c_pad, 3, False, 1, tail_c=b.k_pad)
+
+
 def pack_job(w: torch.Tensor, pw: PackedWeight, *, transpose: bool = False, c_off: int = 0) -> "L.PackJob":
     assert w.is_cuda and w.dtype == torch.float32 and w.is_contiguous()
     j = L.PackJob()
@@ -167,7 +184,7 @@
 
 def igemm_desc(src0, src1, pw: PackedWeight, dst, *, n_img, h_in, w_in, h_out, w_out, stride=1, pad=None, upsample=False,
                bias=None, row_bias=None, residual=None, epilogue=L.EPI_NONE, out_scale=1.0, ws=None, splitk=0,
-               tile=0, into=None) -> L.IgemmDesc:
+               tile=0, into=None, tail=None) -> L.IgemmDesc:
     d = L.IgemmDesc() if into is None else into
     c0 = src0.shape[-1]
     c1 = 0 if src1 is None else src1.shape[-1]
@@ -186,6 +203,16 @@
     n_dst = pw.n_out // 2 if epilogue == L.EPI_GEGLU else pw.n_out
     d.dst_ld = 0 if dst.shape[-1] == n_dst else dst.shape[-1]
     d.k_order = pw.k_order
+    t0, t1 = tail if tail is not None else (None, None)
+    assert (pw.tail_c > 0) == (t0 is not None), "a folded weight needs its tail sources (and only a folded weight takes them)"
+    d.tail0, d.tail1 = ptr(t0), ptr(t1)
+    d.tail_c0, d.tail_c1 = (0 if t0 is None else t0.shape[-1]), (0 if t1 is None else t1.shape[-1])
+    d.tail_k, d.tail_reserved = (pw.k_pad - pw.tail_c if t0 is not None else 0), 0
+    if t0 is not None:
+        assert d.tail_c0 + d.tail_c1 == pw.tail_c and all(t is None or (t.is_contiguous() and t.dtype == src0.dtype and
+                                                                       t.numel() == n_img * h_out * w_out * t.shape[-1]) for t in (t0, t1))
+        assert all(t is None or t.data_ptr() != dst.data_ptr() for t in (t0, t1)), "dst aliases a tail source: other workgroups still read it"
+        splitk = d.splitk = 1
     if (tile & 63) == 15:
         use_skinny(d, pw)
     if ws is not None:
@@ -198,7 +225,7 @@
 
 
 def conv2d(x: torch.Tensor, pw: PackedWeight, bias=None, *, x2=None, stride=1, pad=None, upsample=False, row_bias=None,
-           residual=None, epilogue=L.EPI_NONE, out_dtype=None, out_scale=1.0, splitk=0, tile=0, out=None, dst=None) -> torch.Tensor:
+           residual=None, epilogue=L.EPI_NONE, out_dtype=None, out_scale=1.0, splitk=0, tile=0, out=None, dst=None, tail=None) -> torch.Tensor:
     assert x.is_cuda and x.is_contiguous() and (x2 is None or x2.is_contiguous())
     n, h, w, _ = x.shape
     pad = (pw.ksize // 2) if pad is None else pad
@@ -219,7 +246,7 @@
         scratch = workspace(min(16 * n * ho * wo * pw.n_pad * 4, 256 << 20), x.device)
     d = igemm_desc(x, x2, pw, out, n_img=n, h_in=h, w_in=w, h_out=ho, w_out=wo, stride=stride, pad=pad,
                    upsample=upsample, bias=bias, row_bias=row_bias, residual=residual, epilogue=epilogue,
-                   out_scale=out_scale, ws=scratch, splitk=splitk, tile=tile)
+                   out_scale=out_scale, ws=scratch, splitk=splitk, tile=tile, tail=tail)
     L.check(L.load().mvldm_igemm_fwd(C.byref(d), stream()))
     return out
 
diff --git a/mv_ldm_amd/plan.py b/mv_ldm_amd/plan.py
--- a/mv_ldm_amd/plan.py
+++ b/mv_ldm_amd/plan.py
@@ -10,7 +10,7 @@
 import torch
 
 from . import _lib as L
-from .ops import PackedWeight, conv_out_hw, dt, igemm_desc, ptr, use_skinny
+from .ops import PackedWeight, conv_out_hw, dt, fold_offered, igemm_desc, ptr, use_skinny
 
 
 def _PIN_TILE() -> int:
@@ -149,7 +149,7 @@
             L.check(L.load().mvldm_op_run(C.byref(op), torch.cuda.current_stream().cuda_stream))
 
     def conv(self, x, pw: PackedWeight, bias=None, *, x2=None, stride=1, pad=None, upsample=False, row_bias=None,
-             residual=None, epilogue=L.EPI_NONE, out_dtype=None, out_scale=1.0, out=None, name="conv", splitk=0, tile=0):
+             residual=None, epilogue=L.EPI_NONE, out_dtype=None, out_scale=1.0, out=None, name="conv", splitk=0, tile=0, tail=None):
         n, h, w, c0 = x.shape
         c1 = 0 if x2 is None else x2.shape[-1]
         pad = (pw.ksize // 2) if pad is None else pad
@@ -165,8 +165,13 @@
         es = x.element_size()
         nbytes = (pw.n_out * k_real + n * h * w * (c0 + c1)) * es + m * n_dst * out.element_size() \
             + (m * n_dst * es if residual is not None else 0)
+        if tail is not None:
+            assert out.data_ptr() not in [t.data_ptr() for t in tail if t is not None], "a folded conv must not write over a tail source"
+            k_real += pw.tail_c
+            nbytes += (pw.n_out + m) * pw.tail_c * es
         self._igemm(x, x2, pw, bias, row_bias, residual, out, ws, name, 2.0 * m * pw.n_out * k_real, nbytes, h_out=ho, w_out=wo,
-                    stride=stride, pad=pad, upsample=upsample, epilogue=epilogue, out_scale=out_scale, splitk=splitk, tile=tile)
+                    stride=stride, pad=pad, upsample=upsample, epilogue=epilogue, out_scale=out_scale, splitk=splitk, tile=tile,
+                    **({} if tail is None else {"tail": tail}))
         return out
 
     def _igemm(self, x, x2, pw, bias, row_bias, residual, out, ws, name, flops, nbytes, *, h_out, w_out, tile=0, **desc):
@@ -188,7 +193,51 @@
             own = self.__dict__.get("_own_ptrs", ())
             self.__dict__.setdefault("_tune_srcs", {})[len(self.ops)] = tuple(t if (t is not None and t.data_ptr() in own) else None
                                                                               for t in (x, x2))
-        self._emit(op, name, flops, nbytes, (x, x2, pw.data, pw._skinny if (tile & 63) == 15 else None, bias, row_bias, residual, out))
+        self._emit(op, name, flops, nbytes, (x, x2, pw.data, pw._skinny if (tile & 63) == 15 else None, bias, row_bias, residual, out,
+                                             *(desc.get("tail") or ())))
+
+    def fold_shortcut(self, g2, x, x2, out, pw2, pws, pwf, bias2, biass, biasf) -> bool:
+        n, h, w, c_mid = g2.shape
+        if type(self) is not Builder:
+            return False
+        if os.environ.get("MVLDM_FOLD_SHORTCUT", "1") == "0":
+            return False
+        if pwf is None or not fold_offered(g2.dtype, c_mid, [t.shape[-1] for t in (x, x2) if t is not None]):
+            return False
+        if out is not None and out.data_ptr() in [t.data_ptr() for t in (x, x2) if t is not None]:
+            return False
+        if _PIN_TILE():
+            return False
+        if os.environ.get("MVLDM_FOLD_SHORTCUT") == "2":
+            return True
+        rule = n * h * w >= 2048
+        if not (self.record and self.device.type == "cuda" and os.environ.get("MVLDM_AUTOTUNE", "1") != "0"):
+            return rule
+        key = (n, h, w, c_mid, x.shape[-1], 0 if x2 is None else x2.shape[-1], pw2.n_out, dt(g2), self._ws_bytes)
+        ent = _FOLD_CACHE.get(key)
+        if ent is None:
+            own = self.__dict__.get("_own_ptrs", ())
+            sc = torch.empty(n, h, w, pw2.n_out, dtype=g2.dtype, device=g2.device)
+            dst = torch.empty_like(sc)
+            ws = self.splitk_ws()
+
+            def mk(src, src2, pw, bias, **kw):
+                op = L.Op()
+                op.kind = L.OP_IGEMM
+                igemm_desc(src, src2, pw, dst if kw else sc, n_img=n, h_in=h, w_in=w, h_out=h, w_out=w, bias=bias, ws=ws, into=op.u.igemm, **kw)
+                return op
+            pair = [mk(x, x2, pws, biass), mk(g2, None, pw2, bias2, residual=sc)]
+            fold = [mk(g2, None, pwf, biasf, tail=(x, x2))]
+            srcs = {i: tuple(t if (t is not None and t.data_ptr() in own) else None for t in pr) for i, pr in enumerate(((x, x2), (g2, None)))}
+            autotune_igemm(pair, srcs=srcs)
+            autotune_igemm(fold)
+            t_pair, t_fold = _time_ops(pair, 6), _time_ops(fold, 6)
+            ent = _FOLD_CACHE[key] = [int(t_fold < t_pair), round(t_pair * 1e3, 1), round(t_fold * 1e3, 1)]
+            if os.environ.get("MVLDM_FOLD_LOG"):
+                print(f"[fold] {n} x {h}x{w}, {c_mid} <- {key[4]}+{key[5]}: shortcut + conv2 {ent[1]} us (tiles {pair[0].u.igemm.tile & 63} / "
+                      f"{pair[1].u.igemm.tile & 63}), folded {ent[2]} us (tile {fold[0].u.igemm.tile & 63})", file=sys.stderr, flush=True)
+            save_tune_cache()
+        return bool(ent[0])
 
     def small_launch(self, rows: int, n_out: int) -> bool:
         limit = int(os.environ.get("MVLDM_PAR_ROWS", "0"))
@@ -398,6 +447,7 @@
 
 _TUNE_CACHE = {}
 _WGRAD_CACHE = {}
+_FOLD_CACHE = {}
 _SPLIT_CACHE = {}
 _VALIDATED = set()
 _TUNE_TILES = tuple(int(t) for t in os.environ["MVLDM_TUNE_TILES"].split(",")) if os.environ.get("MVLDM_TUNE_TILES") else (0, 1, 2, 3, 4, 5, 6, 7, 8, 9, 10, 11, 12, 13, 14)
@@ -406,7 +456,8 @@
 def tune_cache_state() -> dict:
     return {"version": 2, "igemm": {json.dumps(list(k)): (int(v) if isinstance(v, int) else list(v)) for k, v in _TUNE_CACHE.items()},
             "wgrad": {json.dumps(list(k)): int(v) for k, v in _WGRAD_CACHE.items()},
-            "split": {json.dumps(list(k)): int(v) for k, v in _SPLIT_CACHE.items()}}
+            "split": {json.dumps(list(k)): int(v) for k, v in _SPLIT_CACHE.items()},
+            "fold": {json.dumps(list(k)): list(v) for k, v in _FOLD_CACHE.items()}}
 
 
 def set_tune_cache_state(state: dict, replace: bool = False) -> None:
@@ -414,7 +465,8 @@
         _TUNE_CACHE.clear()
         _WGRAD_CACHE.clear()
         _SPLIT_CACHE.clear()
-    for name, cache in (("igemm", _TUNE_CACHE), ("wgrad", _WGRAD_CACHE), ("split", _SPLIT_CACHE)):
+        _FOLD_CACHE.clear()
+    for name, cache in (("igemm", _TUNE_CACHE), ("wgrad", _WGRAD_CACHE), ("split", _SPLIT_CACHE), ("fold", _FOLD_CACHE)):
         for k, v in (state.get(name) or {}).items():
             cache[tuple(json.loads(k))] = int(v) if isinstance(v, int) else list(v)
 
@@ -451,7 +503,7 @@
 def _igemm_signature(d) -> tuple:
     return (d.n_img, d.h_in, d.w_in, d.h_out, d.w_out, d.c0, d.c1, d.ksize, d.stride, d.pad, d.upsample, d.n_out, d.n_pad,
             d.k_pad, d.epilogue, d.act_dtype, d.dst_dtype, d.k_order, d.dst_ld, bool(d.residual), bool(d.row_bias),
-            bool(d.bias), d.splitk, d.workspace_bytes)
+            bool(d.bias), d.splitk, d.workspace_bytes) + (("tail", d.tail_c0, d.tail_c1) if d.tail0 else ())
 
 
 _SMALL_ROWS = int(os.environ.get("MVLDM_TUNE_SMALL_ROWS", "64"))
@@ -641,6 +693,8 @@
     d.dst = off(d.dst, i0 * px_out * (d.dst_ld or n_dst) * ds)
     d.residual = off(d.residual, i0 * px_out * n_dst * es)
     d.row_bias = off(d.row_bias, i0 * d.row_bias_ld * 4)
+    d.tail0 = off(d.tail0, i0 * px_out * d.tail_c0 * es)
+    d.tail1 = off(d.tail1, i0 * px_out * d.tail_c1 * es)
     d.n_img = n
     d.tile, d.splitk = 0, 0
     return q
@@ -670,7 +724,8 @@
               and (d.tile & 63) != 15 and not _PIN_TILE() and bool(d.workspace) and idx not in (skinny or {}))
         n1 = 0
         if ok:
-            key = _igemm_signature(d)[:-2] + (d.workspace_bytes,)
+            sig = _igemm_signature(d)
+            key = sig[:22] + (d.workspace_bytes,) + sig[24:]
             if key in _SPLIT_CACHE:
                 n1 = _SPLIT_CACHE[key]
             else:
```

After: 50.89 (median of 6 runs). About the same (+0.7%).
